# tritonmedia/downloader

Hardware: AMD Instinct MI355X
Metric: MB/s staged end-to-end (download->S3) + p50 job latency (higher is better)
Workload: dtype bytes

## Files before the change

downloader_amd/csrc/gpu_part_api.h:

```cpp
#pragma once

#include <stddef.h>
#include <stdint.h>

#define GPU_PART_API_ABI 2u
#define GPU_PART_COPIED 1
#define GPU_PART_DONE 2

typedef void (*gpu_part_notify_fn)(void* arg, uint64_t ticket, int phase);

struct GpuPartHashApi {
  uint32_t abi;
  void* ctx;
  int (*reg)(void* ctx, void* p, size_t n);
  void (*unreg)(void* ctx, void* p);
  uint64_t (*submit)(void* ctx, const uint8_t* data, int64_t len, int64_t piece_len);
  int (*wait)(void* ctx, uint64_t ticket, int phase, uint8_t* out, size_t out_len, char* err,
              size_t errlen);
  void (*set_notify)(void* ctx, gpu_part_notify_fn fn, void* arg);
};
```

downloader_amd/csrc/gpu_sha1.hip:

```cpp
#include <hip/hip_runtime.h>
#include <pybind11/pybind11.h>
#include <pybind11/stl.h>

#include <algorithm>
#include <atomic>
#include <chrono>
#include <cerrno>
#include <condition_variable>
#include <cstring>
#include <deque>
#include <fcntl.h>
#include <mutex>
#include <exception>
#include <stdexcept>
#include <string>
#include <pthread.h>
#include <thread>
#include <unistd.h>
#include <unordered_map>
#include <vector>

#include "gpu_part_api.h"
#include "part_dispatch.h"

// ... 959 lines not shown
      bool live = false;
    } pend[2];
    auto drain = [&](int s) {
      if (!pend[s].live) return;
      HIP_CHECK(hipStreamSynchronize(stream_[s]));
      uint8_t* hm = h_meta_ + (size_t)s * meta_stride_;
      if (out_digests) memcpy(out_digests + pend[s].first * 20, hm, (size_t)pend[s].cnt * 20);
      if (out_ok) memcpy(out_ok + pend[s].first, hm, (size_t)pend[s].cnt);
      pend[s].live = false;
    };
    int s = 0;
    for (int64_t first = 0; first < np; first += per, s ^= 1) {
      int64_t cnt = std::min(per, np - first);
      drain(s);
      fill(first, cnt, h_buf_[s]);
      int64_t off = first * piece_len;
      int64_t bytes = std::min(cnt * piece_len, total - off);
      int64_t last_len = bytes - (cnt - 1) * piece_len;
      uint8_t* dm = d_meta_ + (size_t)s * meta_stride_;
      uint8_t* hm = h_meta_ + (size_t)s * meta_stride_;
      HIP_CHECK(hipMemcpyAsync(d_buf_[s], h_buf_[s], (size_t)bytes, hipMemcpyHostToDevice, stream_[s]));
      const uint8_t* d_exp = nullptr;
      if (expected) {
        uint8_t* de = dm + per;
        HIP_CHECK(hipMemcpyAsync(de, expected + first * 20, (size_t)cnt * 20, hipMemcpyHostToDevice,
                                 stream_[s]));
        d_exp = de;
        launch(stream_[s], d_buf_[s], piece_len, last_len, (int)cnt, d_exp, dm, nullptr);
        HIP_CHECK(hipMemcpyAsync(hm, dm, (size_t)cnt, hipMemcpyDeviceToHost, stream_[s]));
      } else {
        launch(stream_[s], d_buf_[s], piece_len, last_len, (int)cnt, nullptr, nullptr, dm);
        HIP_CHECK(hipMemcpyAsync(hm, dm, (size_t)cnt * 20, hipMemcpyDeviceToHost, stream_[s]));
      }
      pend[s] = {first, cnt, true};
    }
    drain(0);
    drain(1);
  }

  void grow(int64_t bytes) {
    batch_bytes_ = 0;
    for (int s = 0; s < 2; ++s) {
      HIP_CHECK(hipStreamSynchronize(stream_[s]));
      HIP_CHECK(hipHostFree(h_buf_[s]));
      h_buf_[s] = nullptr;
      HIP_CHECK(hipFree(d_buf_[s]));
      d_buf_[s] = nullptr;
      HIP_CHECK(hipHostMalloc((void**)&h_buf_[s], (size_t)bytes, hipHostMallocDefault));
      HIP_CHECK(hipMalloc((void**)&d_buf_[s], (size_t)bytes));
    }
    batch_bytes_ = bytes;
  }

  void ensure_meta(int64_t per) {
    size_t need = (size_t)per * 21;
    if (need <= meta_stride_) return;
    if (d_meta_) HIP_CHECK(hipFree(d_meta_));
    d_meta_ = nullptr;
    if (h_meta_) HIP_CHECK(hipHostFree(h_meta_));
    h_meta_ = nullptr;
    meta_stride_ = 0;
    HIP_CHECK(hipMalloc((void**)&d_meta_, need * 2));
    HIP_CHECK(hipHostMalloc((void**)&h_meta_, need * 2, hipHostMallocDefault));
    meta_stride_ = need;
  }

  int device_;
  int64_t batch_bytes_;
  int readers_;
  hipStream_t stream_[2] = {nullptr, nullptr};
  hipEvent_t done_[2] = {nullptr, nullptr};
  uint8_t* h_buf_[2] = {nullptr, nullptr};
  uint8_t* d_buf_[2] = {nullptr, nullptr};
  uint8_t* d_meta_ = nullptr;
  uint8_t* h_meta_ = nullptr;
  size_t meta_stride_ = 0;
};

class HipPartDevice {
 public:
  using Event = hipEvent_t;

  HipPartDevice(int device, int64_t slot_bytes, int slots, int streams, int max_lanes,
                int copy_streams)
      : device_(device), slot_bytes_(slot_bytes), max_lanes_(max_lanes) {
    int n = 0;
    HIP_CHECK(hipGetDeviceCount(&n));
    if (device < 0 || device >= n) throw std::runtime_error("no such HIP device");
    if (slots < 2 || slot_bytes < (1 << 20) || max_lanes < 64 || copy_streams < 1 ||
        copy_streams > 4)
      throw std::invalid_argument("PartHasher: bad geometry");
    HIP_CHECK(hipSetDevice(device_));
    try {
      create(slots, streams, copy_streams);
    } catch (...) {
      release();
      throw;
    }
  }
  ~HipPartDevice() { release(); }
  HipPartDevice(const HipPartDevice&) = delete;
  HipPartDevice& operator=(const HipPartDevice&) = delete;

  static bool split_default() {
    const char* e = getenv("STAGER_SHA1_KERNEL");
    return !(e && std::string(e) == "lanes");
  }

  static int hw_queues() {
    const char* e = getenv("GPU_MAX_HW_QUEUES");
    const int n = e ? atoi(e) : 0;
    return n > 0 ? n : 4;
  }

  bool split() const { return split_; }
  int copy_streams() const { return (int)copies_.size(); }
  int compute_streams() const { return (int)streams_.size(); }
  int slots() const { return (int)slots_.size(); }
  void bind_thread() { HIP_CHECK(hipSetDevice(device_)); }
  int64_t* lane_table(int s) { return slots_[(size_t)s].h_lane; }

  Event copy(int s, int64_t off, const uint8_t* host, int64_t len, int cs) {
    hipStream_t st = copies_[(size_t)cs];
    HIP_CHECK(hipMemcpyAsync(slots_[(size_t)s].d_data + off, host, (size_t)len,
                             hipMemcpyHostToDevice, st));
    Event e = take_event();
    HIP_CHECK(hipEventRecord(e, st));
    return e;
  }
  bool copied(Event e) { return query(e); }
  void recycle(Event e) {
    if (e) free_events_.push_back(e);
  }
  void close_copies(int s) {
    Slot& sl = slots_[(size_t)s];
    for (size_t k = 0; k < copies_.size(); ++k) HIP_CHECK(hipEventRecord(sl.copied[k], copies_[k]));
  }
  int64_t launch_lanes() const { return launch_lanes_; }
  void launch(int stream, const int* slots, const int* lanes, int nslots, int total,
              bool align16) {
    if (total <= 0 || total > launch_lanes_) throw std::runtime_error("PartHasher: bad launch");
    Run& r = runs_[(size_t)stream];
    hipStream_t st = streams_[(size_t)stream];
    int64_t* ho = r.h_tab;
    int64_t* hl = r.h_tab + total;
    int i = 0;
    for (int k = 0; k < nslots; ++k) {
      Slot& sl = slots_[(size_t)slots[k]];
      for (size_t c = 0; c < copies_.size(); ++c) HIP_CHECK(hipStreamWaitEvent(st, sl.copied[c], 0));
      const int64_t base = (int64_t)(sl.d_data - arena_);
      for (int l = 0; l < lanes[k]; ++l, ++i) {
        ho[i] = base + sl.h_lane[l];
        hl[i] = sl.h_lane[max_lanes_ + l];
      }
    }
    if (i != total) throw std::runtime_error("PartHasher: lane count mismatch");
    HIP_CHECK(hipMemcpyAsync(r.d_tab, r.h_tab, (size_t)total * 2 * sizeof(int64_t),
                             hipMemcpyHostToDevice, st));
    const int64_t* dp = r.d_tab;
    const int64_t* dl = r.d_tab + total;
    const int block = 64, grid = (total + block - 1) / block;
    if (align16 && split_)
      hipLaunchKernelGGL(sha1_lanes_split, dim3(grid), dim3(kSplitThreads), 0, st, arena_, dp,
                         dl, total, r.d_dig);
    else if (align16)
      hipLaunchKernelGGL(sha1_lanes<16>, dim3(grid), dim3(block), 0, st, arena_, dp, dl, total,
                         r.d_dig);
    else
      hipLaunchKernelGGL(sha1_lanes<1>, dim3(grid), dim3(block), 0, st, arena_, dp, dl, total,
                         r.d_dig);
    HIP_CHECK(hipGetLastError());
    HIP_CHECK(hipMemcpyAsync(r.h_dig, r.d_dig, (size_t)total * 20, hipMemcpyDeviceToHost, st));
    HIP_CHECK(hipEventRecord(r.done, st));
  }
  bool finished(int stream) { return query(runs_[(size_t)stream].done); }
  const uint8_t* digests(int stream) { return runs_[(size_t)stream].h_dig; }
  void drain_copies() noexcept {
    for (auto c : copies_) hipStreamSynchronize(c);
  }
  int reg(void* p, size_t n) {
    if (hipSetDevice(device_) != hipSuccess) return -1;
    return hipHostRegister(p, n, hipHostRegisterDefault) == hipSuccess ? 0 : -1;
  }
  void unreg(void* p) {
    hipSetDevice(device_);
    hipHostUnregister(p);
  }

 private:
  struct Slot {
    uint8_t* d_data = nullptr;
    int64_t* h_lane = nullptr;
    hipEvent_t copied[4] = {nullptr, nullptr, nullptr, nullptr};
  };
  struct Run {
    int64_t* h_tab = nullptr;
    int64_t* d_tab = nullptr;
    uint8_t* d_dig = nullptr;
    uint8_t* h_dig = nullptr;
    hipEvent_t done = nullptr;
  };

  static bool query(hipEvent_t e) {
    hipError_t q = hipEventQuery(e);
    if (q == hipErrorNotReady) return false;
    HIP_CHECK(q);
    return true;
  }

  void create(int slots, int streams, int copy_streams) {
    copies_.resize((size_t)copy_streams);
    for (auto& c : copies_) HIP_CHECK(hipStreamCreateWithFlags(&c, hipStreamNonBlocking));
    const int hwq = hw_queues();
    const int compute = streams > 0 ? std::min(streams, 4) : std::max(1, hwq - copy_streams);
    streams_.resize((size_t)compute);
    for (auto& st : streams_) HIP_CHECK(hipStreamCreateWithFlags(&st, hipStreamNonBlocking));
    slots_.resize((size_t)slots);
    HIP_CHECK(hipMalloc((void**)&arena_, (size_t)slot_bytes_ * (size_t)slots + kArenaPad));
    for (size_t k = 0; k < slots_.size(); ++k) {
      Slot& sl = slots_[k];
      sl.d_data = arena_ + (size_t)slot_bytes_ * k;
      HIP_CHECK(hipHostMalloc((void**)&sl.h_lane, (size_t)max_lanes_ * 2 * sizeof(int64_t),
                              hipHostMallocDefault));
      for (auto& e : sl.copied) HIP_CHECK(hipEventCreateWithFlags(&e, hipEventDisableTiming));
    }
    launch_lanes_ = (int64_t)max_lanes_ * (int64_t)slots;
    runs_.resize((size_t)compute);
    for (auto& r : runs_) {
      HIP_CHECK(hipHostMalloc((void**)&r.h_tab, (size_t)launch_lanes_ * 2 * sizeof(int64_t),
                              hipHostMallocDefault));
      HIP_CHECK(hipMalloc((void**)&r.d_tab, (size_t)launch_lanes_ * 2 * sizeof(int64_t)));
      HIP_CHECK(hipMalloc((void**)&r.d_dig, (size_t)launch_lanes_ * 20));
      HIP_CHECK(hipHostMalloc((void**)&r.h_dig, (size_t)launch_lanes_ * 20, hipHostMallocDefault));
      HIP_CHECK(hipEventCreateWithFlags(&r.done, hipEventDisableTiming));
    }
  }

  void release() {
    hipSetDevice(device_);
    for (auto c : copies_)
      if (c) hipStreamSynchronize(c);
    for (auto st : streams_)
      if (st) {
        hipStreamSynchronize(st);
        hipStreamDestroy(st);
      }
    for (auto c : copies_)
      if (c) hipStreamDestroy(c);
    if (arena_) hipFree(arena_);
    arena_ = nullptr;
    for (auto& sl : slots_) {
      if (sl.h_lane) hipHostFree(sl.h_lane);
      for (auto e : sl.copied)
        if (e) hipEventDestroy(e);
    }
    for (auto& r : runs_) {
      if (r.h_tab) hipHostFree(r.h_tab);
      if (r.d_tab) hipFree(r.d_tab);
      if (r.d_dig) hipFree(r.d_dig);
      if (r.h_dig) hipHostFree(r.h_dig);
      if (r.done) hipEventDestroy(r.done);
    }
    for (hipEvent_t e : free_events_) hipEventDestroy(e);
    copies_.clear();
    streams_.clear();
    slots_.clear();
    runs_.clear();
    free_events_.clear();
  }

  hipEvent_t take_event() {
    if (!free_events_.empty()) {
      hipEvent_t e = free_events_.back();
      free_events_.pop_back();
      return e;
    }
    hipEvent_t e;
    HIP_CHECK(hipEventCreateWithFlags(&e, hipEventDisableTiming));
    return e;
  }

  int device_;
  int64_t slot_bytes_;
  int max_lanes_;
  bool split_ = split_default();
  int64_t launch_lanes_ = 0;
  uint8_t* arena_ = nullptr;
  std::vector<hipStream_t> copies_;
  std::vector<hipStream_t> streams_;
  std::vector<Slot> slots_;
  std::vector<Run> runs_;
  std::vector<hipEvent_t> free_events_;
};

using PartHasher = stager::PartDispatcher<HipPartDevice>;

py::dict part_stats(PartHasher& h) {
  const stager::PartDispatchStats s = h.stats();
  py::dict d;
  d["submitted"] = s.submitted;
  d["launches"] = s.launches;
  d["lanes"] = s.lanes;
  d["max_batch_lanes"] = s.max_batch_lanes;
  d["multi_slot_launches"] = s.multi_slot_launches;
  d["max_launch_slots"] = s.max_launch_slots;
  d["broken"] = s.broken;
  d["pending"] = s.pending;
  d["registered"] = s.registered;
  d["unregistered"] = s.unregistered;
  d["register_s"] = s.register_s;
  d["copy_streams"] = s.copy_streams;
  d["compute_streams"] = s.compute_streams;
  d["kernel"] = h.device().split() ? "sha1_lanes_split" : "sha1_lanes";
  return d;
}

int device_count() {
  int n = 0;
  if (hipGetDeviceCount(&n) != hipSuccess) return 0;
  return n;
}

}

PYBIND11_MODULE(_gpuhash, m) {
  m.doc() = "gfx950 batched SHA-1 piece verification (one lane per piece)";
  m.def("device_count", &device_count);
  m.def(
      "mem_info",
      [](int device) {
        size_t free_b = 0, total_b = 0;
        HIP_CHECK(hipSetDevice(device));
        HIP_CHECK(hipMemGetInfo(&free_b, &total_b));
        return py::make_tuple(free_b, total_b);
      },
      py::arg("device") = 0, "(free, total) bytes of device memory (hipMemGetInfo)");
  m.def("arch", [] {
    hipDeviceProp_t p;
    HIP_CHECK(hipGetDeviceProperties(&p, 0));
    return std::string(p.gcnArchName);
  });
  py::class_<GpuVerifier>(m, "GpuVerifier")
      .def(py::init([](int device, int64_t batch_bytes, int readers) {
             py::gil_scoped_release rel;
             return new GpuVerifier(device, batch_bytes, readers);
           }),
           py::arg("device") = 0, py::arg("batch_bytes") = (int64_t)256 << 20,
           py::arg("reader_threads") = 8)
      .def(
          "hash_buffer",
          [](GpuVerifier& g, const py::buffer& b, int64_t piece_len) {
            py::buffer_info info = b.request();
            int64_t n = (int64_t)info.size * (int64_t)info.itemsize;
            if (piece_len <= 0) throw std::invalid_argument("piece_len must be > 0");
            std::string out;
            {
              py::gil_scoped_release rel;
              out = g.hash_buffer((const uint8_t*)info.ptr, n, piece_len);
            }
            return py::bytes(out);
          },
          py::arg("data"), py::arg("piece_len"))
      .def(
          "verify_files",
          [](GpuVerifier& g, const std::vector<std::pair<std::string, int64_t>>& files,
             int64_t piece_len, const py::bytes& hashes) {
            std::string hs = hashes;
            if (piece_len <= 0) throw std::invalid_argument("piece_len must be > 0");
            std::vector<uint8_t> ok;
            {
              py::gil_scoped_release rel;
              ok = g.verify_files(files, piece_len, hs);
            }
            return py::bytes((const char*)ok.data(), ok.size());
          },
          py::arg("files"), py::arg("piece_len"), py::arg("hashes"))
      .def(
          "verify_files_streamed",
          [](GpuVerifier& g, const std::vector<std::pair<std::string, int64_t>>& files,
             int64_t piece_len, const py::bytes& hashes, int64_t chunk,
             const std::vector<int>& which) {
            std::string hs = hashes;
            if (piece_len <= 0) throw std::invalid_argument("piece_len must be > 0");
            std::vector<uint8_t> ok;
            std::vector<double> timing;
            {
              py::gil_scoped_release rel;
              ok = g.verify_files_streamed(files, piece_len, hs, chunk, &timing, which);
            }
            return py::make_tuple(py::bytes((const char*)ok.data(), ok.size()),
                                  py::make_tuple(timing[0], timing[1]));
          },
          py::arg("files"), py::arg("piece_len"), py::arg("hashes"), py::arg("chunk") = 65536,
          py::arg("which") = std::vector<int>{},
          "Chunk-streamed SHA-1 verification: returns (ok bytes, (host_fill_s, host_wait_s)); "
          "with `which`, one ok byte per listed piece in list order.")
      .def(
          "kernel_bench",
          [](GpuVerifier& g, int64_t piece_len, int n_pieces, int iters) {
            if (piece_len <= 0 || piece_len % 16 || n_pieces <= 0 || iters <= 0)
              throw std::invalid_argument("piece_len must be a positive multiple of 16");
            std::vector<double> r;
            {
              py::gil_scoped_release rel;
              r = g.kernel_bench(piece_len, n_pieces, iters);
            }
            return py::make_tuple(r[0], r[1]);
          },
          py::arg("piece_len"), py::arg("n_pieces"), py::arg("iters") = 5,
          "(ms_bitop3, ms_plain): kernel time per launch, device-resident data")
      .def(
          "kernel_bench_prefetch",
          [](GpuVerifier& g, int64_t piece_len, int n_pieces, int iters) {
            if (piece_len <= 0 || piece_len % 16 || n_pieces <= 0 || iters <= 0)
              throw std::invalid_argument("piece_len must be a positive multiple of 16");
            std::vector<double> r;
            {
              py::gil_scoped_release rel;
              r = g.kernel_bench_prefetch(piece_len, n_pieces, iters);
            }
            return py::make_tuple(r[0], r[1]);
          },
          py::arg("piece_len"), py::arg("n_pieces"), py::arg("iters") = 5,
          "(ms_prefetch, ms_no_prefetch): kernel time per launch, device-resident data")
      .def(
          "kernel_bench_concurrent",
          [](GpuVerifier& g, int64_t piece_len, int n0, int n1, int iters, int mode) {
            if (piece_len < 256 || piece_len % 16 || n0 <= 0 || n1 < 0 || iters <= 0 ||
                mode < 0 || mode > 2)
              throw std::invalid_argument("piece_len must be a multiple of 16, >= 256");
            std::vector<double> r;
            {
              py::gil_scoped_release rel;
              r = g.kernel_bench_concurrent(piece_len, n0, n1, iters, mode);
            }
            return py::make_tuple(r[0], r[1], r[2]);
          },
          py::arg("piece_len"), py::arg("n0"), py::arg("n1"), py::arg("iters") = 3,
          py::arg("mode") = 0,
          "(ms alone, ms on stream 0, ms on stream 1): sha1_lanes_split launches of n0 and n1 "
          "lanes side by side (mode 0), n0 beside 48 x 64 MiB H2D copies (1), after 40 ms idle "
          "(2)")
      .def(
          "kernel_bench_split",
          [](GpuVerifier& g, int64_t piece_len, int n_pieces, int iters, bool dup) {
            if (piece_len < 256 || piece_len % 16 || n_pieces <= 0 || iters <= 0)
              throw std::invalid_argument("piece_len must be a multiple of 16, >= 256");
            std::vector<double> r;
            {
              py::gil_scoped_release rel;
              r = g.kernel_bench_split(piece_len, n_pieces, iters, dup);
            }
            return py::make_tuple(r[0], r[1], r[2] != 0.0);
          },
          py::arg("piece_len"), py::arg("n_pieces"), py::arg("iters") = 3, py::arg("dup") = true,
          "(ms_split, ms_lanes, digests_equal): the PartHasher's two kernels on one lane table "
          "(dup=False: the split kernel with its idle lanes left idle)")
      .def_property_readonly("batch_bytes", &GpuVerifier::batch_bytes);
  py::class_<PartHasher>(m, "PartHasher")
      .def(py::init([](int device, int64_t slot_bytes, int slots, int streams, int max_lanes,
                       int copy_streams) {
             py::gil_scoped_release rel;
             return new PartHasher(slot_bytes, max_lanes, device, slot_bytes, slots, streams,
                                   max_lanes, copy_streams);
           }),
           py::arg("device") = 0, py::arg("slot_bytes") = (int64_t)1 << 30, py::arg("slots") = 8,
           py::arg("streams") = 0, py::arg("max_lanes") = 16384, py::arg("copy_streams") = 2)
      .def(
          "api",
          [](PartHasher& h) {
            return py::capsule((void*)h.api(), "downloader_amd.gpu_part_api");
          },
          "PyCapsule of the C ABI (gpu_part_api.h) for _native.set_gpu_part_hasher; the "
          "PartHasher must outlive every user of the capsule (ops.hashing keeps it for good)")
      .def(
          "hash",
          [](PartHasher& h, const py::buffer& b, int64_t piece_len) {
            py::buffer_info info = b.request();
            const int64_t n = (int64_t)info.size * (int64_t)info.itemsize;
            const int64_t np = piece_len > 0 ? (n + piece_len - 1) / piece_len : 0;
            std::string out((size_t)np * 20, '\0');
            char err[256] = {0};
            int rc;
            {
              py::gil_scoped_release rel;
              void* p = info.ptr;
              bool r = h.reg(p, (size_t)n) == 0;
              uint64_t t = h.submit((const uint8_t*)p, n, piece_len);
              rc = t ? h.wait(t, GPU_PART_DONE, (uint8_t*)out.data(), out.size(), err, sizeof err)
                     : -1;
              if (r) h.unreg(p);
            }
            if (rc != 0) throw std::runtime_error(err[0] ? err : "PartHasher refused the part");
            return py::bytes(out);
          },
          py::arg("data"), py::arg("piece_len"))
      .def("stats", &part_stats);
}
```

downloader_amd/csrc/module.cpp:

```cpp
#include <pybind11/pybind11.h>
#include <pybind11/stl.h>

#include <atomic>
#include <cstdlib>
#include <netinet/in.h>
#include <netinet/tcp.h>
#include <sys/socket.h>

#include "native.h"

namespace py = pybind11;
using namespace stager;

namespace {

struct BufView {
  const uint8_t* p;
  size_t n;
  py::buffer_info info;
};

BufView view(const py::buffer& b) {
  py::buffer_info info = b.request();
  if (info.ndim > 1 && info.strides.back() != info.itemsize)
    throw std::invalid_argument("buffer must be C-contiguous");
  size_t n = (size_t)info.size * (size_t)info.itemsize;
  return BufView{(const uint8_t*)info.ptr, n, std::move(info)};
}

py::dict head_to_dict(const ResponseHead& h) {
  py::dict d;
  d["status"] = h.status;
  d["reason"] = h.reason;
  py::list hs;
  for (auto& kv : h.headers) hs.append(py::make_tuple(kv.first, kv.second));
  d["headers"] = hs;
  d["content_length"] = h.content_length;
  d["chunked"] = h.chunked;
  d["keep_alive"] = h.keep_alive;
  return d;
}

}

void forget_ticket(uint64_t id) {
  if (id) gpu_part_forget(id);
}

static bool head_matches(const std::string& head, const std::string& pat) {
  size_t at = 0, i = 0;
  while (i <= pat.size()) {
    size_t star = pat.find('*', i);
    if (star == std::string::npos) star = pat.size();
    std::string piece = pat.substr(i, star - i);
    if (!piece.empty()) {
      size_t f = head.find(piece, at);
      if (f == std::string::npos) return false;
      at = f + piece.size();
    }
    i = star + 1;
  }
  return true;
}

static bool fault_bad_crc(const std::string& put_head) {
  static std::string pat;
  static std::atomic<int64_t> left{[] {
    const char* e = getenv("STAGER_FAULT_BAD_CRC");
    if (!e || !*e) return (int64_t)0;
    std::string v(e);
    size_t c = v.rfind(':');
    int64_t n = 1;
    if (c != std::string::npos && c + 1 < v.size() &&
        v.find_first_not_of("0123456789", c + 1) == std::string::npos) {
      n = atoll(v.c_str() + c + 1);
      v.resize(c);
    }
    pat = v;
    return n;
  }()};
  if (left.load(std::memory_order_relaxed) <= 0 || !head_matches(put_head, pat)) return false;
  return left.fetch_sub(1) > 0;
}

struct PieceSplit {
  int64_t skip, full_len, piece_len;
};

py::dict relay(HttpConn& src, const py::bytes& get_head, HttpConn& dst, const py::bytes& put_head,
               int64_t length, Progress* prog, int64_t max_body, const PieceSplit* split,
               bool crc, bool gpu = false) {
  std::string gh = get_head, ph = put_head;
  ResponseHead g, p;
  std::string gerr, pbody, digests, head, tail, crc_b64;
  int64_t moved = 0;
  uint64_t ticket = 0;
  {
    py::gil_scoped_release rel;
    try {
      src.send_request(gh, nullptr, 0);
      g = src.read_head();
      bool ok = (g.status == 200 || g.status == 206) && !g.chunked && g.content_length == length;
      if (!ok) {
        if (!g.chunked && g.content_length >= 0 && g.content_length <= (1 << 20))
          gerr = src.read_body(g, 1 << 20);
        else
          src.mark_unusable();
      } else {
        int cork = 1;
        setsockopt(dst.fd(), IPPROTO_TCP, TCP_CORK, &cork, sizeof(cork));
        dst.send_raw(ph);
        uint32_t c = 0;
        if (crc && length > 0) {
          char hx[32];
          snprintf(hx, sizeof hx, "%llx\r\n", (unsigned long long)length);
          dst.send_raw(hx);
        }
        moved = split ? src.relay_body_hashed(dst, length, split->skip, split->full_len,
                                              split->piece_len, prog, &digests, &head, &tail,
                                              crc ? &c : nullptr, gpu ? &ticket : nullptr)
                      : src.relay_body_to(dst, length, prog, crc ? &c : nullptr);
        if (crc) {
          if (fault_bad_crc(ph)) c ^= 1u;
          crc_b64 = crc32c_base64(c);
          dst.send_raw(std::string(length > 0 ? "\r\n" : "") + "0\r\nx-amz-checksum-crc32c:" +
                       crc_b64 + "\r\n\r\n");
        }
        cork = 0;
        setsockopt(dst.fd(), IPPROTO_TCP, TCP_CORK, &cork, sizeof(cork));
        p = dst.read_head();
        pbody = dst.read_body(p, max_body);
      }
    } catch (...) {
      forget_ticket(ticket);
      throw;
    }
    if (ticket && !(p.status >= 200 && p.status < 300)) {
      forget_ticket(ticket);
      ticket = 0;
    }
  }
  py::dict d;
  d["get"] = head_to_dict(g);
  d["get_body"] = py::bytes(gerr);
  d["put"] = p.status ? (py::object)head_to_dict(p) : py::none();
  d["put_body"] = py::bytes(pbody);
  d["moved"] = moved;
  d["crc32c"] = crc_b64;
  if (split) {
    d["gpu_ticket"] = ticket;
    d["digests"] = py::bytes(digests);
    d["head"] = py::bytes(head);
    d["tail"] = py::bytes(tail);
  }
  return d;
}

PYBIND11_MODULE(_native, m) {
  m.doc() = "stager host-native byte paths: hashing (OpenSSL EVP, threaded) and zero-copy HTTP";

  m.def("digest_size", &digest_size);
  m.def("crc32c_impl", []() { return std::string(crc32c_impl()); },
        "the CRC32C implementation this CPU runs (avx512-vpclmulqdq / sse4.2-3way)");
  m.def("sha1_mb_supported", &sha1_mb_supported,
        "True when the host runs the AVX-512 16-lane multi-buffer SHA-1 (csrc/sha1_mb.cpp)");
  m.def("effective_cpus", &effective_cpus,
        "CPUs usable by this process: affinity mask capped by the cgroup v2 cpu.max quota");
  m.def(
      "set_gpu_part_hasher",
      [](const py::object& capsule, int min_pieces) {
        if (capsule.is_none()) {
          set_gpu_part_hasher(nullptr, min_pieces);
          return;
        }
        void* p = PyCapsule_GetPointer(capsule.ptr(), "downloader_amd.gpu_part_api");
        if (!p) throw py::error_already_set();
        set_gpu_part_hasher(p, min_pieces);
      },
      py::arg("api"), py::arg("min_pieces") = 8,
      "Route the hashed relay's parts (>= min_pieces whole pieces) to the GPU hasher whose C "
      "ABI capsule is `api` (_gpuhash.PartHasher.api()); None: host multi-buffer SHA-1");
  m.def(
      "gpu_part_wait",
      [](uint64_t id) {
        std::string d;
        {
          py::gil_scoped_release rel;
          d = gpu_part_wait(id);
        }
        return py::bytes(d);
      },
      py::arg("id"), "Block until part `id` (the relay's gpu_ticket) is hashed: its digests");
  m.def(
      "gpu_part_forget",
      [](uint64_t id) {
        py::gil_scoped_release rel;
        gpu_part_forget(id);
      },
      py::arg("id"),
      "Nobody will ask for part `id`: returns once its buffer is back in the pool; the result "
      "is dropped when it arrives");
  m.def("gpu_part_eventfd", &gpu_part_eventfd,
        "eventfd that turns readable when gpu_part_poll has news");
  m.def(
      "gpu_part_poll",
      []() {
        std::vector<GpuPartEvent> ev;
        {
          py::gil_scoped_release rel;
          ev = gpu_part_poll();
        }
        py::list out;
        for (auto& e : ev)
          out.append(py::make_tuple(e.id, e.kind, py::bytes(e.data)));
        return out;
      },
      "Drain completions: [(id, kind, data)] with kind 1 = copied (the part's buffer is back in "
      "the pool), 2 = done (data = 20 B digests per piece), 3 = failed (data = error message)");
  py::class_<CpuPartHasher>(m, "CpuPartHasher")
      .def(py::init<double, int, int>(), py::arg("delay_s") = 0.005,
           py::arg("fail_copy_every") = 0, py::arg("fail_done_every") = 0,
           "gpu_part_api.h on a host thread (tests of the asynchronous relay-hashing path); "
           "fail_*_every: every Nth job's copy / hash fails")
      .def("api", [](CpuPartHasher& h) {
        return py::capsule((void*)h.api(), "downloader_amd.gpu_part_api");
      })
      .def_property_readonly("registered", &CpuPartHasher::registered);
  m.def("gpu_part_stats", []() {
    GpuPartStats s = gpu_part_stats();
    py::dict d;
    d["submitted"] = s.submitted;
    d["host_fallbacks"] = s.host_fallbacks;
    d["refused"] = s.refused;
    d["pending"] = s.pending;
    return d;
  });
  m.def("relay_pool_trim", &relay_pool_trim, py::arg("keep_bytes") = 0,
        "Unmap idle hashed-relay part buffers beyond keep_bytes; returns the bytes freed");
  m.def("relay_pool_set_budget", &relay_pool_set_budget, py::arg("bytes"),
        "Bound leased + idle part buffers (0 = no bound): idle ones are unmapped to make room");
  m.def("relay_pool_reset_peak", &relay_pool_reset_peak,
        "Restart the pool's high-water mark (peak_bytes) and its over_budget count");
  m.def("relay_pool_set_max_idle", &relay_pool_set_max_idle, py::arg("n"),
        "Keep at most n idle part buffers (the rest are unmapped on release)");
  py::class_<SwarmWire>(m, "SwarmWire",
                        "Native peer-wire receive path of one torrent session (peerwire.cpp)")
      .def(py::init<int, int>(), py::arg("verify_threads") = 2, py::arg("io_threads") = 4)
      .def("set_storage",
           [](SwarmWire& w, int64_t piece_length, int64_t total, const py::bytes& hashes,
              const std::vector<std::pair<int, int64_t>>& files) {
             w.set_storage(piece_length, total, std::string(hashes), files);
           },
           py::arg("piece_length"), py::arg("total"), py::arg("hashes"), py::arg("files"))
      .def("begin_piece", &SwarmWire::begin_piece, py::arg("idx"))
      .def("drop_piece", &SwarmWire::drop_piece, py::arg("idx"))
      .def("set_pipeline", &SwarmWire::set_pipeline, py::arg("depth"))
      .def("set_conn_pipeline", &SwarmWire::set_conn_pipeline, py::arg("conn_id"),
           py::arg("depth"), "requests in flight on one connection (its bandwidth-delay product)")
      .def("assign", &SwarmWire::assign, py::arg("conn_id"), py::arg("idx"),
           "Own piece idx on the connection: the wire requests its blocks (returns the "
           "connection's blocks still to request)")
      .def("todo", &SwarmWire::todo, py::arg("conn_id"))
      .def("release",
           [](SwarmWire& w, uint64_t id) {
             py::list out;
             for (auto& r : w.release(id)) out.append(py::make_tuple(r.first, py::bytes(r.second)));
             return out;
           },
           py::arg("conn_id"),
           "[(idx, states)] of the pieces the connection owned, now ordinary (2 received, "
           "1 requested and unanswered, 0 neither)")
      .def("release_piece",
           [](SwarmWire& w, uint32_t idx) -> py::object {
             uint64_t owner = 0;
             std::string st;
             if (!w.release_piece(idx, &owner, &st)) return py::none();
             return py::make_tuple(owner, py::bytes(st));
           },
           py::arg("idx"), "(owner, states) of an owned piece made ordinary, or None")
      .def("rx_idle", &SwarmWire::rx_idle, py::arg("conn_id"))
      .def("take_block",
           [](SwarmWire& w, uint32_t idx, uint32_t begin, const py::buffer& b) {
             py::buffer_info i = b.request();
             return w.take_block(idx, begin, (const uint8_t*)i.ptr,
                                 (uint32_t)(i.size * i.itemsize));
           },
           py::arg("idx"), py::arg("begin"), py::arg("data"),
           "A block received on a Python-framed connection: 0 not taken, 1 taken, 2 taken "
           "and the piece complete")
      .def("set_have",
           [](SwarmWire& w, const py::bytes& bits) { w.set_have(std::string(bits)); },
           py::arg("bits"))
      .def("set_have_piece", &SwarmWire::set_have_piece, py::arg("idx"))
      .def("set_serving", &SwarmWire::set_serving, py::arg("conn_id"), py::arg("on"))
      .def("set_backlog_cap", &SwarmWire::set_backlog_cap, py::arg("bytes"))
      .def("backlogged", &SwarmWire::backlogged,
           "True while complete, unreported pieces hold the cap or more (start no new piece)")
      .def("set_host_tail", &SwarmWire::set_host_tail, py::arg("on"),
           "GPU mode: hash the pieces completing from now on on the host (the download's end)")
      .def("rx_total", &SwarmWire::rx_total, "bytes received on every connection so far")
      .def("gpu_latency", &SwarmWire::gpu_latency,
           "GPU mode: submission -> digest time of the device's pieces (EWMA, s; 0 = none yet)")
      .def("set_gpu", &SwarmWire::set_gpu, py::arg("on"), py::arg("max_inflight") = 64,
           "Verify complete pieces on the installed GPU part hasher (set_gpu_part_hasher), at "
           "most max_inflight at once (the rest on the host)")
      .def("attach",
           [](SwarmWire& w, int fd, uint64_t id, const py::bytes& prefix) {
             w.attach(fd, id, std::string(prefix));
           },
           py::arg("fd"), py::arg("conn_id"), py::arg("prefix") = py::bytes(),
           "Hand a connected socket over (the fd is owned from here on, closed by detach)")
      .def("send",
           [](SwarmWire& w, uint64_t id, const py::bytes& data) {
             std::string s(data);
             return w.send(id, std::move(s));
           },
           py::arg("conn_id"), py::arg("data"))
      .def("sendv",
           [](SwarmWire& w, uint64_t id, const py::list& parts) {
// ... 388 lines not shown
```

downloader_amd/csrc/native.h:

```cpp
#pragma once

#include <atomic>
#include <condition_variable>
#include <cstdint>
#include <deque>
#include <memory>
#include <mutex>
#include <string>
#include <thread>
#include <unordered_map>
#include <utility>
#include <vector>

typedef struct evp_md_ctx_st EVP_MD_CTX;
typedef struct evp_md_st EVP_MD;
typedef struct ssl_st SSL;
typedef struct ssl_ctx_st SSL_CTX;

namespace stager {

const EVP_MD* md_for(const std::string& algo);
size_t digest_size(const std::string& algo);
int effective_cpus();
int resolve_threads(int threads, size_t work_items);
// ... 26 lines not shown

bool sha1_mb_supported();
void sha1_mb(const uint8_t* const* msgs, const size_t* lens, size_t n, uint8_t* out);
void sha1x16_init(uint32_t st[5][16]);
void sha1_mb16_blocks(uint32_t state[5][16], const uint8_t* const ptr[16], size_t nblocks,
                      uint16_t active);
void sha1x16_finish(uint32_t st[5][16], const uint8_t* const tails[16], size_t tail_len,
                    uint64_t total_len, uint16_t active, uint8_t* out);

struct Storage {
  struct Entry {
    std::string path;
    int64_t length;
    int64_t offset;
    int fd;
  };
  explicit Storage(const std::vector<std::pair<std::string, int64_t>>& files);
  ~Storage();
  void open_all(bool missing_ok);
  void close_all();
  bool read(int64_t off, int64_t len, uint8_t* buf) const;
  std::vector<Entry> entries;
  int64_t total = 0;
};

std::vector<uint8_t> verify_pieces(const std::vector<std::pair<std::string, int64_t>>& files,
                                   int64_t piece_len, const std::string& hashes,
                                   const std::vector<int64_t>& which, int threads);
std::string hash_storage_pieces(const std::vector<std::pair<std::string, int64_t>>& files,
                                int64_t piece_len, const std::string& algo, int threads);
std::vector<std::string> hash_file_ranges(const std::string& path,
                                          const std::vector<std::pair<int64_t, int64_t>>& ranges,
                                          const std::string& algo, int threads);

class TlsContext {
 public:
  TlsContext(bool verify, const std::string& ca_file);
  ~TlsContext();
  TlsContext(const TlsContext&) = delete;
  TlsContext& operator=(const TlsContext&) = delete;
  SSL_CTX* ctx() const { return ctx_; }
  bool verify() const { return verify_; }

 private:
  SSL_CTX* ctx_ = nullptr;
  bool verify_;
};
SSL* tls_handshake(TlsContext& ctx, int fd, const std::string& name);
std::string tls_error(SSL* s, int r, const std::string& what);

constexpr int64_t kMaxBufferedPart = (int64_t)64 << 20;

struct PipeStats {
  uint64_t created, short_pipes;
  size_t in_use, in_use_bytes, idle, idle_bytes;
};
PipeStats pipe_stats();
struct RelayCounters {
  uint64_t relays[4], bytes[4], cpu_ns[4];
  uint64_t splice_in_calls, splice_out_calls;
  uint64_t dup_calls, dup_bytes;
  uint64_t crc_ns, crc_bytes;
  uint64_t sha1_ns;
  uint64_t nt_bytes;
};
RelayCounters relay_counters();
void set_pipe_sizes(size_t main, size_t tee);
void set_pipes_refused(bool on);
void set_relay_dup(const std::string& mode);
std::string relay_dup_mode();

struct RelayPoolStats {
  size_t idle_buffers, idle_bytes, in_use, max_idle;
  uint64_t created;
  size_t in_use_bytes, budget, peak_bytes;
  uint64_t evicted, over_budget;
};
void set_gpu_part_hasher(const void* api, int min_pieces);
const void* gpu_part_hasher_current();
void swarm_piece_pool_forget(const void* api);
void swarm_piece_pool_limit(size_t bytes);
struct GpuPartStats {
  uint64_t submitted, host_fallbacks, refused, pending;
};
GpuPartStats gpu_part_stats();
std::string gpu_part_wait(uint64_t id);
void gpu_part_forget(uint64_t id);
int gpu_part_eventfd();
struct GpuPartEvent {
  uint64_t id;
  int kind;
  std::string data;
};
std::vector<GpuPartEvent> gpu_part_poll();
class CpuPartHasher {
 public:
  explicit CpuPartHasher(double delay_s, int fail_copy_every = 0, int fail_done_every = 0);
  ~CpuPartHasher();
  const void* api() const;
  uint64_t registered() const;

 private:
  struct Impl;
  std::unique_ptr<Impl> impl_;
};
struct WireEvent {
  uint64_t conn;
  int kind;
  std::string data;
};
struct SwarmWireStats {
  uint64_t begun = 0, blocks = 0, block_bytes = 0, blocks_ignored = 0, verified = 0,
           hash_fails = 0, rx_bytes = 0, recvs = 0;
  uint64_t verify_batches = 0, sha_ns = 0, write_ns = 0;
  uint64_t served_bytes = 0;
  uint64_t assigned = 0, requests = 0;
  uint64_t gpu_pieces = 0, gpu_refused = 0, gpu_errors = 0;
  uint64_t gpu_overflow = 0;
  int64_t gpu_latency_ns_sum = 0, gpu_latency_ns_max = 0;
  int64_t backlog_bytes = 0;
  size_t pool_in_use = 0, pool_idle = 0, pool_idle_bytes = 0;
  uint64_t pool_allocs = 0, pool_frees = 0, pool_locks = 0;
  size_t active_pieces = 0;
  size_t io_threads = 0;
  uint64_t serve_floods = 0;
  uint64_t serve_cancels = 0;
};
class SwarmWire {
 public:
  static constexpr int kEvMsg = 1, kEvBlocks = 2, kEvClosed = 3, kEvPiece = 4, kEvNeed = 5;
  explicit SwarmWire(int verify_threads = 2, int io_threads = 4);
  ~SwarmWire();
  void set_storage(int64_t piece_length, int64_t total, const std::string& hashes,
                   const std::vector<std::pair<int, int64_t>>& files);
  void begin_piece(uint32_t idx);
  void drop_piece(uint32_t idx);
  void set_pipeline(uint32_t depth);
  void set_conn_pipeline(uint64_t conn, uint32_t depth);
  size_t assign(uint64_t conn, uint32_t idx);
  size_t todo(uint64_t conn);
  std::vector<std::pair<uint32_t, std::string>> release(uint64_t conn);
  bool release_piece(uint32_t idx, uint64_t* owner, std::string* states);
  double rx_idle(uint64_t conn);
  void set_have(const std::string& bits);
  void set_have_piece(uint32_t idx);
  void set_serving(uint64_t id, bool on);
  void set_gpu(bool on, int max_inflight = 64);
  void set_host_tail(bool on);
  double gpu_latency() const { return gpu_lat_ewma_ns_.load() / 1e9; }
  uint64_t rx_total() const { return rx_bytes_.load(std::memory_order_relaxed); }
  void set_backlog_cap(int64_t bytes);
  bool backlogged();
  void attach(int fd, uint64_t id, const std::string& prefix);
  size_t send(uint64_t id, std::string data);
  size_t pending_out(uint64_t id);
  uint64_t conn_rx(uint64_t id);
  void detach(uint64_t id);
  int eventfd() const { return efd_; }
  std::vector<WireEvent> poll();
  SwarmWireStats stats();
  void close();
  int take_block(uint32_t idx, uint32_t begin, const uint8_t* p, uint32_t len);

 private:
  struct Piece;
  struct Conn;
  struct OutItem;
  struct IoLoop;
// ... 162 lines not shown
```

downloader_amd/csrc/part_dispatch.h:

```cpp
#pragma once

#include <algorithm>
#include <chrono>
#include <condition_variable>
#include <cstring>
#include <deque>
#include <exception>
#include <mutex>
#include <pthread.h>
#include <stdexcept>
#include <string>
#include <thread>
#include <unordered_map>
#include <utility>
#include <vector>

#include "gpu_part_api.h"

namespace stager {

struct PartDispatchStats {
  uint64_t submitted = 0, launches = 0, lanes = 0, max_batch_lanes = 0;
  uint64_t multi_slot_launches = 0, max_launch_slots = 0;
  uint64_t registered = 0, unregistered = 0;
  double register_s = 0;
  bool broken = false;
  size_t pending = 0;
  int copy_streams = 0, compute_streams = 0;
};

template <class Dev>
class PartDispatcher {
 public:
  template <class... A>
  PartDispatcher(int64_t slot_bytes, int max_lanes, A&&... dev_args)
      : dev_(std::forward<A>(dev_args)...), slot_bytes_(slot_bytes), max_lanes_(max_lanes) {
    slots_.resize((size_t)dev_.slots());
    running_.resize((size_t)dev_.compute_streams());
    api_.abi = GPU_PART_API_ABI;
    api_.ctx = this;
    api_.reg = [](void* c, void* p, size_t n) { return ((PartDispatcher*)c)->reg(p, n); };
    api_.unreg = [](void* c, void* p) { ((PartDispatcher*)c)->unreg(p); };
    api_.submit = [](void* c, const uint8_t* d, int64_t len, int64_t pl) {
      return ((PartDispatcher*)c)->submit(d, len, pl);
    };
    api_.wait = [](void* c, uint64_t t, int ph, uint8_t* out, size_t ol, char* err, size_t el) {
      return ((PartDispatcher*)c)->wait(t, ph, out, ol, err, el);
    };
    api_.set_notify = [](void* c, gpu_part_notify_fn fn, void* arg) {
      PartDispatcher* h = (PartDispatcher*)c;
      std::lock_guard<std::mutex> g(h->mu_);
      h->notify_ = fn;
      h->notify_arg_ = arg;
    };
    thread_ = std::thread([this] { run(); });
    pthread_setname_np(thread_.native_handle(), "gpu-part-disp");
  }

  ~PartDispatcher() {
    {
      std::lock_guard<std::mutex> g(mu_);
      stop_ = true;
    }
    cv_.notify_all();
    if (thread_.joinable()) thread_.join();
  }

  PartDispatcher(const PartDispatcher&) = delete;
  PartDispatcher& operator=(const PartDispatcher&) = delete;

  const GpuPartHashApi* api() const { return &api_; }
  Dev& device() { return dev_; }

  int reg(void* p, size_t n) {
    const auto t0 = std::chrono::steady_clock::now();
    const bool ok = dev_.reg(p, n) == 0;
    const double dt = std::chrono::duration<double>(std::chrono::steady_clock::now() - t0).count();
    std::lock_guard<std::mutex> g(mu_);
    stats_.registered++;
    stats_.register_s += dt;
    return ok ? 0 : -1;
  }
  void unreg(void* p) {
    dev_.unreg(p);
    std::lock_guard<std::mutex> g(mu_);
    stats_.unregistered++;
  }

  uint64_t submit(const uint8_t* data, int64_t len, int64_t piece_len) {
    if (len <= 0 || piece_len <= 0) return 0;
    const int64_t np = (len + piece_len - 1) / piece_len;
    if (np > max_lanes_ || len > slot_bytes_) return 0;
    std::lock_guard<std::mutex> g(mu_);
    if (broken_ || stop_) return 0;
    uint64_t t = ++seq_;
    Job& j = jobs_[t];
    j.host = data;
    j.len = len;
    j.piece_len = piece_len;
    j.np = (int)np;
    queue_.push_back(t);
    stats_.submitted++;
    cv_.notify_all();
    return t;
  }

  int wait(uint64_t t, int phase, uint8_t* out, size_t out_len, char* err, size_t errlen) {
    std::unique_lock<std::mutex> lk(mu_);
    auto it = jobs_.find(t);
    if (it == jobs_.end()) return fail(err, errlen, "unknown ticket");
    Job* j = &it->second;
    wcv_.wait(lk, [&] {
      return !j->err.empty() || j->done || (phase == GPU_PART_COPIED && j->copied);
    });
    if (!j->err.empty()) {
      std::string e = j->err;
      if (phase == GPU_PART_DONE || j->done || broken_) jobs_.erase(t);
      return fail(err, errlen, e.c_str());
    }
    if (phase == GPU_PART_DONE) {
      if (out_len < j->digests.size()) return fail(err, errlen, "digest buffer too small");
      memcpy(out, j->digests.data(), j->digests.size());
      jobs_.erase(t);
    }
    return 0;
  }

  PartDispatchStats stats() {
    std::lock_guard<std::mutex> g(mu_);
    PartDispatchStats s = stats_;
    s.broken = broken_;
    s.pending = jobs_.size();
    s.copy_streams = dev_.copy_streams();
    s.compute_streams = dev_.compute_streams();
    return s;
  }

 private:
  using Event = typename Dev::Event;
  struct Job {
    const uint8_t* host = nullptr;
    int64_t len = 0, piece_len = 0;
    int np = 0;
    int slot = -1, lane0 = 0;
    Event copy_ev{};
    bool copied = false, done = false;
    std::string err, digests;
  };
  struct Slot {
    int64_t used = 0;
    int lanes = 0;
    bool align16 = true;
    std::vector<uint64_t> jobs;
    int state = 0;
    std::chrono::steady_clock::time_point opened;
  };

  static int fail(char* err, size_t errlen, const char* msg) {
    if (err && errlen) {
      strncpy(err, msg, errlen - 1);
      err[errlen - 1] = 0;
    }
    return -1;
  }

  void tell(std::vector<uint64_t>& owed, int phase) {
    if (owed.empty()) return;
    std::vector<uint64_t> tickets;
    tickets.swap(owed);
    gpu_part_notify_fn fn;
    void* arg;
    {
      std::lock_guard<std::mutex> g(mu_);
      fn = notify_;
      arg = notify_arg_;
    }
    if (fn)
      for (uint64_t t : tickets) fn(arg, t, phase);
  }

  Job& job(uint64_t t) {
    std::lock_guard<std::mutex> g(mu_);
    return jobs_.at(t);
  }

  void run() {
    std::vector<uint64_t> owed_copied, owed_done;
    std::deque<uint64_t> copying;
    try {
      dev_.bind_thread();
      int filling = -1;
      for (;;) {
        std::deque<uint64_t> fresh;
        {
          std::unique_lock<std::mutex> lk(mu_);
          const bool idle = queue_.empty() && copying.empty() && !any_running() &&
                            !any_closed() && !(filling >= 0 && slots_[(size_t)filling].lanes > 0);
          if (idle) cv_.wait(lk, [&] { return stop_ || !queue_.empty(); });
          if (stop_ && idle && queue_.empty()) return;
          fresh.swap(queue_);
        }
        bool progressed = false;
        while (!fresh.empty()) {
          const uint64_t t = fresh.front();
          Job* j = &job(t);
          if (filling >= 0) {
            Slot& f = slots_[(size_t)filling];
            const int64_t off = (f.used + 255) & ~(int64_t)255;
            if (off + j->len > slot_bytes_ || f.lanes + j->np > max_lanes_) {
              f.state = 2;
              dev_.close_copies(filling);
              filling = -1;
            }
          }
          if (filling < 0) {
            filling = free_slot();
            if (filling < 0) break;
            Slot& f = slots_[(size_t)filling];
            f.state = 1;
            f.used = 0;
            f.lanes = 0;
            f.align16 = true;
            f.jobs.clear();
            f.opened = std::chrono::steady_clock::now();
          }
          Slot& f = slots_[(size_t)filling];
          const int64_t off = (f.used + 255) & ~(int64_t)255;
          const int cs = (int)(next_copy_++ % (size_t)dev_.copy_streams());
          Event ev = dev_.copy(filling, off, j->host, j->len, cs);
          int64_t* lt = dev_.lane_table(filling);
          for (int k = 0; k < j->np; ++k) {
            const int64_t po = (int64_t)k * j->piece_len;
            lt[f.lanes + k] = off + po;
            lt[max_lanes_ + f.lanes + k] = std::min(j->piece_len, j->len - po);
          }
          {
            std::lock_guard<std::mutex> g(mu_);
            j->copy_ev = ev;
            j->slot = filling;
            j->lane0 = f.lanes;
          }
          if (j->piece_len % 16) f.align16 = false;
          f.lanes += j->np;
          f.used = off + j->len;
          f.jobs.push_back(t);
          copying.push_back(t);
          fresh.pop_front();
          progressed = true;
        }
        const bool slot_bound = !fresh.empty();
        if (slot_bound) {
          std::lock_guard<std::mutex> g(mu_);
          for (auto it = fresh.rbegin(); it != fresh.rend(); ++it) queue_.push_front(*it);
        }
        for (auto it = copying.begin(); it != copying.end();) {
          Job* j = &job(*it);
          if (!dev_.copied(j->copy_ev)) {
            ++it;
            continue;
          }
          Event ev;
          {
            std::lock_guard<std::mutex> g(mu_);
            j->copied = true;
            ev = j->copy_ev;
            j->copy_ev = Event{};
            owed_copied.push_back(*it);
          }
          dev_.recycle(ev);
          wcv_.notify_all();
          it = copying.erase(it);
          progressed = true;
        }
        tell(owed_copied, GPU_PART_COPIED);
        for (size_t s = 0; s < running_.size(); ++s) {
          std::vector<int>& group = running_[s];
          if (group.empty()) continue;
          if (!dev_.finished((int)s)) continue;
          const uint8_t* dig = dev_.digests((int)s);
          std::vector<Event> late;
          {
            std::lock_guard<std::mutex> g(mu_);
            size_t base = 0;
            for (int si : group) {
              Slot& sl = slots_[(size_t)si];
              for (uint64_t t : sl.jobs) {
                Job& j = jobs_.at(t);
                j.digests.assign((const char*)dig + (base + (size_t)j.lane0) * 20, (size_t)j.np * 20);
                j.done = true;
                if (!j.copied) {
                  j.copied = true;
                  late.push_back(j.copy_ev);
                  j.copy_ev = Event{};
                  auto c = std::find(copying.begin(), copying.end(), t);
                  if (c != copying.end()) copying.erase(c);
                  owed_copied.push_back(t);
                }
                owed_done.push_back(t);
              }
              base += (size_t)sl.lanes;
            }
          }
          for (Event e : late) dev_.recycle(e);
          wcv_.notify_all();
          for (int si : group) {
            slots_[(size_t)si].state = 0;
            slots_[(size_t)si].jobs.clear();
          }
          group.clear();
          progressed = true;
        }
        tell(owed_copied, GPU_PART_COPIED);
        for (size_t s = 0; s < running_.size(); ++s) {
          if (!running_[s].empty()) continue;
          std::vector<int> group, lanes;
          int total = 0;
          bool a16 = true;
          for (int pick : closed_by_age()) {
            const Slot& sl = slots_[(size_t)pick];
            if (total + sl.lanes > dev_.launch_lanes()) break;
            group.push_back(pick);
            lanes.push_back(sl.lanes);
            total += sl.lanes;
            a16 = a16 && sl.align16;
          }
          if (filling >= 0 && slots_[(size_t)filling].lanes > 0 &&
              total + slots_[(size_t)filling].lanes <= dev_.launch_lanes()) {
            Slot& f = slots_[(size_t)filling];
            dev_.close_copies(filling);
            group.push_back(filling);
            lanes.push_back(f.lanes);
            total += f.lanes;
            a16 = a16 && f.align16;
            filling = -1;
          }
          if (group.empty()) break;
          dev_.launch((int)s, group.data(), lanes.data(), (int)group.size(), total, a16);
          for (int si : group) slots_[(size_t)si].state = 3;
          running_[s] = group;
          std::lock_guard<std::mutex> g(mu_);
          stats_.launches++;
          stats_.lanes += (uint64_t)total;
          stats_.max_batch_lanes = std::max<uint64_t>(stats_.max_batch_lanes, (uint64_t)total);
          stats_.max_launch_slots = std::max<uint64_t>(stats_.max_launch_slots, group.size());
          if (group.size() > 1) stats_.multi_slot_launches++;
          progressed = true;
        }
        tell(owed_done, GPU_PART_DONE);
        if (!progressed) {
          std::unique_lock<std::mutex> lk(mu_);
          cv_.wait_until(lk, std::chrono::system_clock::now() + std::chrono::microseconds(200),
                         [&] { return stop_ || (!slot_bound && !queue_.empty()); });
        }
      }
    } catch (const std::exception& e) {
      dev_.drain_copies();
      tell(owed_copied, GPU_PART_COPIED);
      tell(owed_done, GPU_PART_DONE);
      std::vector<uint64_t> failed_copy, failed_hash;
      {
        std::lock_guard<std::mutex> g(mu_);
        broken_ = true;
        for (auto& kv : jobs_)
          if (!kv.second.done) {
            kv.second.err = std::string("GPU part hasher: ") + e.what();
            (kv.second.copied ? failed_hash : failed_copy).push_back(kv.first);
          }
        queue_.clear();
        wcv_.notify_all();
      }
      tell(failed_copy, GPU_PART_COPIED);
      tell(failed_hash, GPU_PART_DONE);
    }
  }

  bool any_running() const {
    for (auto& g : running_)
      if (!g.empty()) return true;
    return false;
  }
  bool any_closed() const {
    for (auto& sl : slots_)
      if (sl.state == 2) return true;
    return false;
  }
  int free_slot() const {
    for (size_t i = 0; i < slots_.size(); ++i)
      if (slots_[i].state == 0) return (int)i;
    return -1;
  }
  std::vector<int> closed_by_age() const {
    std::vector<int> out;
    for (size_t i = 0; i < slots_.size(); ++i)
      if (slots_[i].state == 2) out.push_back((int)i);
    std::sort(out.begin(), out.end(),
              [&](int a, int b) { return slots_[(size_t)a].opened < slots_[(size_t)b].opened; });
    return out;
  }

  Dev dev_;
  int64_t slot_bytes_;
  int max_lanes_;
  size_t next_copy_ = 0;
  std::vector<std::vector<int>> running_;
  std::vector<Slot> slots_;
  std::mutex mu_;
  std::condition_variable cv_, wcv_;
  std::deque<uint64_t> queue_;
  std::unordered_map<uint64_t, Job> jobs_;
  uint64_t seq_ = 0;
  bool stop_ = false, broken_ = false;
  PartDispatchStats stats_;
  GpuPartHashApi api_{};
  gpu_part_notify_fn notify_ = nullptr;
  void* notify_arg_ = nullptr;
  std::thread thread_;
};

}
```

downloader_amd/csrc/part_fake_device.h:

```cpp
#pragma once

#include <atomic>
#include <chrono>
#include <condition_variable>
#include <cstring>
#include <deque>
#include <functional>
#include <memory>
#include <mutex>
#include <random>
#include <stdexcept>
#include <string>
#include <thread>
#include <vector>

#include "native.h"

namespace stager {

struct FakeDeviceKnobs {
  int copy_us_max = 200;
  int kernel_us_max = 1500;
  double lag = 0.3;
  int fail_launch_at = 0;
  int fail_query_at = 0;
  uint32_t seed = 1;
};

class FakePartDevice {
 public:
  using Event = std::shared_ptr<std::atomic<int>>;

  FakePartDevice(int64_t slot_bytes, int slots, int compute_streams, int copy_streams,
                 int max_lanes, FakeDeviceKnobs k)
      : max_lanes_(max_lanes), k_(k), rng_(k.seed) {
    slots_.resize((size_t)slots);
    for (auto& s : slots_) {
      s.mem.assign((size_t)slot_bytes, 0);
      s.lanes.assign((size_t)max_lanes * 2, 0);
      s.markers.resize((size_t)copy_streams);
    }
    runs_.resize((size_t)compute_streams);
    for (auto& r : runs_) r.done = std::make_shared<std::atomic<int>>(0);
    for (int i = 0; i < copy_streams; ++i) copies_.emplace_back(new Queue(k.seed * 7 + i));
    for (int i = 0; i < compute_streams; ++i) computes_.emplace_back(new Queue(k.seed * 13 + i));
  }
  ~FakePartDevice() {
    for (auto& q : copies_) q->stop();
    for (auto& q : computes_) q->stop();
  }
  FakePartDevice(const FakePartDevice&) = delete;
  FakePartDevice& operator=(const FakePartDevice&) = delete;

  int copy_streams() const { return (int)copies_.size(); }
  int compute_streams() const { return (int)computes_.size(); }
  int slots() const { return (int)slots_.size(); }
  void bind_thread() {}
  int64_t* lane_table(int s) { return slots_[(size_t)s].lanes.data(); }

  Event copy(int s, int64_t off, const uint8_t* host, int64_t len, int cs) {
    Event e = std::make_shared<std::atomic<int>>(0);
    uint8_t* dst = slots_[(size_t)s].mem.data() + off;
    const int us = k_.copy_us_max;
    Queue* q = copies_[(size_t)cs].get();
    q->push([dst, host, len, e, us, q] {
      q->nap(us);
      memcpy(dst, host, (size_t)len);
      e->store(1, std::memory_order_release);
    });
    return e;
  }
  bool copied(const Event& e) {
    tick();
    if (!e->load(std::memory_order_acquire)) return false;
    return !chance(k_.lag);
  }
  void recycle(const Event&) {}
  void close_copies(int s) {
    Slot& sl = slots_[(size_t)s];
    for (size_t k = 0; k < copies_.size(); ++k) {
      Event m = std::make_shared<std::atomic<int>>(0);
      sl.markers[k] = m;
      copies_[k]->push([m] { m->store(1, std::memory_order_release); });
    }
  }
  int64_t launch_lanes() const { return (int64_t)max_lanes_ * (int64_t)slots_.size(); }
  void launch(int stream, const int* slots, const int* lanes, int nslots, int total,
              bool ) {
    if (k_.fail_launch_at && ++launches_ == k_.fail_launch_at)
      throw std::runtime_error("injected device fault (launch)");
    Run* run = &runs_[(size_t)stream];
    run->done->store(0, std::memory_order_relaxed);
    std::vector<std::pair<Slot*, int>> group;
    std::vector<Event> markers;
    for (int k = 0; k < nslots; ++k) {
      Slot* sl = &slots_[(size_t)slots[k]];
      group.push_back({sl, lanes[k]});
      markers.insert(markers.end(), sl->markers.begin(), sl->markers.end());
    }
    const int us = k_.kernel_us_max, ml = max_lanes_;
    Queue* q = computes_[(size_t)stream].get();
    run->dig.assign((size_t)total * 20, 0);
    q->push([run, group, markers, us, ml, q] {
      for (auto& m : markers)
        while (m && !m->load(std::memory_order_acquire)) std::this_thread::yield();
      q->nap(us);
      size_t i = 0;
      for (auto& g : group) {
        Slot* sl = g.first;
        for (int k = 0; k < g.second; ++k, ++i) {
          const int64_t off = sl->lanes[(size_t)k], len = sl->lanes[(size_t)(ml + k)];
          const std::string d = digest("sha1", sl->mem.data() + off, (size_t)len);
          memcpy(run->dig.data() + i * 20, d.data(), 20);
        }
      }
      run->done->store(1, std::memory_order_release);
    });
  }
  bool finished(int stream) {
    tick();
    return runs_[(size_t)stream].done->load(std::memory_order_acquire) != 0;
  }
  const uint8_t* digests(int stream) { return runs_[(size_t)stream].dig.data(); }
  void drain_copies() noexcept {
    for (auto& q : copies_) q->drain();
  }
  int reg(void*, size_t) { return 0; }
  void unreg(void*) {}

 private:
  struct Queue {
    std::mutex mu;
    std::condition_variable cv;
    std::deque<std::function<void()>> tasks;
    bool stopping = false, busy = false;
    std::mt19937 rng;
    std::thread th;
    explicit Queue(uint32_t seed) : rng(seed) {
      th = std::thread([this] {
        std::unique_lock<std::mutex> lk(mu);
        for (;;) {
          cv.wait(lk, [&] { return stopping || !tasks.empty(); });
          if (tasks.empty()) return;
          auto f = std::move(tasks.front());
          tasks.pop_front();
          busy = true;
          lk.unlock();
          f();
          lk.lock();
          busy = false;
          cv.notify_all();
        }
      });
    }
    void push(std::function<void()> f) {
      std::lock_guard<std::mutex> g(mu);
      tasks.push_back(std::move(f));
      cv.notify_all();
    }
    void nap(int us_max) {
      const int us = us_max > 0 ? (int)(rng() % (uint32_t)us_max) : 0;
      if (us) std::this_thread::sleep_for(std::chrono::microseconds(us));
    }
    void drain() {
      std::unique_lock<std::mutex> lk(mu);
      cv.wait(lk, [&] { return tasks.empty() && !busy; });
    }
    void stop() {
      {
        std::lock_guard<std::mutex> g(mu);
        stopping = true;
      }
      cv.notify_all();
      if (th.joinable()) th.join();
    }
  };
  struct Slot {
    std::vector<uint8_t> mem;
    std::vector<int64_t> lanes;
    std::vector<Event> markers;
  };
  struct Run {
    std::vector<uint8_t> dig;
    Event done;
  };

  void tick() {
    if (k_.fail_query_at && ++queries_ == k_.fail_query_at)
      throw std::runtime_error("injected device fault (query)");
  }
  bool chance(double p) {
    return p > 0 && std::uniform_real_distribution<double>(0, 1)(rng_) < p;
  }

  int max_lanes_;
  FakeDeviceKnobs k_;
  std::mt19937 rng_;
  int launches_ = 0, queries_ = 0;
  std::vector<Slot> slots_;
  std::vector<Run> runs_;
  std::vector<std::unique_ptr<Queue>> copies_, computes_;
};

}
```

downloader_amd/csrc/selftest.cpp:

```cpp
#include <arpa/inet.h>
#include <fcntl.h>
#include <netinet/in.h>
#include <signal.h>
#include <sys/socket.h>
#include <unistd.h>

#include <openssl/err.h>
#include <openssl/evp.h>
#include <openssl/pem.h>
#include <openssl/ssl.h>
#include <openssl/x509v3.h>

#include <poll.h>

#include <algorithm>
#include <chrono>
#include <condition_variable>
#include <cstdio>
#include <cstdlib>
#include <cstring>
#include <functional>
#include <map>
#include <memory>
#include <mutex>
// ... 660 lines not shown
        const uint32_t idx = rd32(e.data.data());
        if (e.data[4] == 1) {
          verified[idx]++;
          done++;
        } else {
          bad++;
          w.begin_piece(idx);
          w.assign(1, idx);
        }
        if (!released && done >= npieces / 2) {
          released = true;
          records_before = block_records;
          for (auto& r : w.release(2)) {
            CHECK(r.second.size() == (size_t)((std::min<int64_t>(plen, total - (int64_t)r.first * plen) + 16383) / 16384));
            w.assign(1, r.first);
          }
        }
      }
    }
  }
  CHECK(done == npieces);
  for (int i = 0; i < npieces; ++i) CHECK(verified[i] == 1);
  SwarmWireStats st = w.stats();
  CHECK(bad == 1 && st.hash_fails == 1 && st.verified == (uint64_t)npieces);
  CHECK(released && records_before == 0);
  CHECK(needs > 0);
  CHECK(st.blocks_ignored >= 1);
  w.close();
  for (auto& t : seeders) t.join();
  std::vector<uint8_t> back((size_t)total);
  CHECK(pread(f1, back.data(), (size_t)total, 0) == total);
  CHECK(back == data);
  for (int fd : theirs) close(fd);
  close(f1);
  unlink(p1);
  fprintf(stderr, "wire (owned): %d pieces, %d requests, %d NEED events, %llu blocks refused\n",
          done, requests.load(), needs, (unsigned long long)st.blocks_ignored);
}

static void multislot_section() {
  Watchdog wd("multi-slot launches", 60);
  FakeDeviceKnobs k;
  k.kernel_us_max = 30000;
  k.copy_us_max = 100;
  k.lag = 0.3;
  k.seed = 7;
  auto h = fake_hasher(k);
  const GpuPartHashApi* api = h->api();
  const int64_t piece = 16 << 10;
  const int parts = 160, pieces = 8;
  auto data = rnd((size_t)parts * pieces * piece, 91);
  std::vector<uint64_t> tickets;
  for (int i = 0; i < parts; ++i) {
    const uint8_t* p = data.data() + (size_t)i * pieces * piece;
    uint64_t t = 0;
    while (!(t = api->submit(api->ctx, p, pieces * piece, piece)))
      std::this_thread::sleep_for(std::chrono::microseconds(50));
    tickets.push_back(t);
  }
  bool ok = true;
  for (int i = 0; i < parts; ++i) {
    uint8_t dig[pieces * 20];
    char err[256] = {0};
    if (api->wait(api->ctx, tickets[(size_t)i], GPU_PART_DONE, dig, sizeof dig, err, sizeof err) != 0) {
      fprintf(stderr, "multi-slot: part %d failed: %s\n", i, err);
      ok = false;
      continue;
    }
    for (int q = 0; q < pieces; ++q) {
      const uint8_t* pc = data.data() + ((size_t)i * pieces + q) * piece;
      if (digest("sha1", pc, (size_t)piece) != std::string((const char*)dig + q * 20, 20)) ok = false;
    }
  }
  const PartDispatchStats st = h->stats();
  fprintf(stderr, "multi-slot: %llu launches, %llu spanning >= 2 slots, up to %llu slots / %llu lanes\n",
          (unsigned long long)st.launches, (unsigned long long)st.multi_slot_launches,
          (unsigned long long)st.max_launch_slots, (unsigned long long)st.max_batch_lanes);
  CHECK(ok);
  CHECK(st.multi_slot_launches > 0 && st.max_launch_slots >= 2);
  CHECK(st.max_batch_lanes > 256);
  CHECK(st.lanes == (uint64_t)parts * pieces && st.pending == 0);
}

static void stress_sections() {
  multislot_section();
  {
    Watchdog wd("part stress", 90);
    PartStress cfg;
    GpuPartStats before = gpu_part_stats();
    PartStressResult r = part_stress(cfg);
    GpuPartStats after = gpu_part_stats();
    fprintf(stderr, "part stress: %d good, %d forgotten, %d via poll, %d failed, %d hashers\n",
            r.good, r.forgotten, r.polled, r.failed, r.hashers);
    CHECK(r.digests_ok && r.failed == 0);
    CHECK(r.good + r.forgotten == cfg.threads * cfg.parts);
    CHECK(r.forgotten > 0 && r.hashers > 2);
    CHECK(after.submitted - before.submitted + after.refused - before.refused ==
          (uint64_t)(cfg.threads * cfg.parts));
    CHECK(after.submitted - before.submitted > (uint64_t)(cfg.threads * cfg.parts) / 2);
    CHECK(after.pending == 0);
  }
  {
    Watchdog wd("part stress with device faults", 90);
    PartStress cfg;
    cfg.threads = 16;
    cfg.parts = 24;
    cfg.replace_every_ms = 20;
    cfg.first.fail_launch_at = 3;
    cfg.knobs.fail_launch_at = 4;
    cfg.knobs.fail_query_at = 400;
    GpuPartStats before = gpu_part_stats();
    PartStressResult r = part_stress(cfg);
    GpuPartStats after = gpu_part_stats();
    fprintf(stderr, "part stress (faults): %d good, %d forgotten, %d failed, %d host fallbacks\n",
            r.good, r.forgotten, r.failed, (int)(after.host_fallbacks - before.host_fallbacks));
    CHECK(r.digests_ok);
    CHECK(r.good + r.forgotten + r.failed == cfg.threads * cfg.parts);
    CHECK(r.failed + (int)(after.host_fallbacks - before.host_fallbacks) > 0);
    CHECK(after.pending == 0);
  }
}

int main() {
  signal(SIGPIPE, SIG_IGN);
  if (getenv("SELFTEST_ONLY") && strcmp(getenv("SELFTEST_ONLY"), "wire") == 0) {
    wire_section(false);
    wire_section(true);
    wire_owned_section();
    printf(g_fail ? "selftest: failures\n" : "selftest ok\n");
    return g_fail ? 1 : 0;
  }
  if (getenv("SELFTEST_ONLY") && strcmp(getenv("SELFTEST_ONLY"), "stress") == 0) {
    stress_sections();
    printf(g_fail ? "selftest: failures\n" : "selftest ok\n");
    return g_fail ? 1 : 0;
  }
  const uint8_t* abc = (const uint8_t*)"abc";
  CHECK(hex(digest("sha1", abc, 3)) == "a9993e364706816aba3e25717850c26c9cd0d89d");
  CHECK(hex(digest("md5", abc, 3)) == "900150983cd24fb0d6963f7d28e17f72");
  CHECK(hex(digest("sha256", abc, 3)) ==
        "ba7816bf8f01cfea414140de5dae2223b00361a396177a9cb410ff61f20015ad");

  auto data = rnd(8 << 20, 1);
  std::string p1 = hash_pieces("sha1", data.data(), data.size(), 65536, 1);
  std::string p8 = hash_pieces("sha1", data.data(), data.size(), 65536, 8);
  CHECK(p1 == p8);

  auto a = rnd(3000001, 2), b = rnd(777777, 3);
  std::string fa = tmpfile_with(a, "a"), fb = tmpfile_with(b, "b");
  std::vector<std::pair<std::string, int64_t>> files = {{fa, (int64_t)a.size()}, {fb, (int64_t)b.size()}};
  std::string hashes = hash_storage_pieces(files, 262144, "sha1", 8);
  auto ok = verify_pieces(files, 262144, hashes, {}, 8);
  bool all = true;
  for (auto v : ok) all = all && v;
  CHECK(all);
  {
    int fd = open(fb.c_str(), O_WRONLY);
    uint8_t x = b[5] ^ 0xFF;
    pwrite(fd, &x, 1, 5);
    close(fd);
  }
  ok = verify_pieces(files, 262144, hashes, {}, 8);
  int bad = 0;
  for (auto v : ok) bad += !v;
  CHECK(bad == 1);

  auto body = rnd(1 << 20, 4);
// ... 318 lines not shown
```

downloader_amd/csrc/transfer.cpp:

```cpp
#include "native.h"
#include "gpu_part_api.h"

#include <algorithm>
#include <atomic>
#include <chrono>
#include <condition_variable>
#include <deque>
#include <thread>
#include <arpa/inet.h>
#include <cerrno>
#include <cstdlib>
#include <cstring>
#include <fcntl.h>
#include <netdb.h>
#include <netinet/in.h>
#include <netinet/tcp.h>
#include <poll.h>
#include <mutex>
#include <new>
#include <stdexcept>
#include <sys/mman.h>
#include <sys/sendfile.h>
#include <sys/socket.h>
#include <sys/types.h>
// ... 1292 lines not shown
    {
      std::lock_guard<std::mutex> g(mu_);
      for (size_t i = 0; i < idle_.size();) {
        if (idle_[i]->reg_api && idle_[i]->reg_api != keep) {
          idle_bytes_ -= idle_[i]->cap;
          drop.push_back(std::move(idle_[i]));
          idle_.erase(idle_.begin() + (ptrdiff_t)i);
        } else {
          ++i;
        }
      }
    }
  }
  size_t trim(size_t keep_bytes) {
    std::vector<std::unique_ptr<PartBuffer>> drop;
    size_t freed = 0;
    {
      std::lock_guard<std::mutex> g(mu_);
      while (!idle_.empty() && idle_bytes_ > keep_bytes) {
        idle_bytes_ -= idle_.back()->cap;
        freed += idle_.back()->cap;
        drop.push_back(std::move(idle_.back()));
        idle_.pop_back();
      }
    }
    return freed;
  }
  void set_max_idle(size_t n) {
    std::lock_guard<std::mutex> g(mu_);
    max_idle_ = n;
  }
  void set_budget(size_t bytes) {
    std::vector<std::unique_ptr<PartBuffer>> drop;
    std::lock_guard<std::mutex> g(mu_);
    budget_ = bytes;
    while (bytes && !idle_.empty() && in_use_bytes_ + idle_bytes_ > budget_) {
      idle_bytes_ -= idle_.back()->cap;
      drop.push_back(std::move(idle_.back()));
      idle_.pop_back();
      evicted_++;
    }
  }
  void reset_peak() {
    std::lock_guard<std::mutex> g(mu_);
    peak_ = in_use_bytes_ + idle_bytes_;
    over_budget_ = 0;
  }
  RelayPoolStats stats() {
    std::lock_guard<std::mutex> g(mu_);
    return RelayPoolStats{idle_.size(), idle_bytes_, in_use_, max_idle_, created_.load(),
                          in_use_bytes_, budget_, peak_, evicted_, over_budget_};
  }

 private:
  void lease(size_t bytes) {
    in_use_ += 1;
    in_use_bytes_ += bytes;
    if (budget_ && in_use_bytes_ > budget_) over_budget_++;
    peak_ = std::max(peak_, in_use_bytes_ + idle_bytes_);
  }
  std::mutex mu_;
  std::vector<std::unique_ptr<PartBuffer>> idle_;
  size_t idle_bytes_ = 0, in_use_ = 0, max_idle_ = 16;
  size_t in_use_bytes_ = 0, budget_ = 0, peak_ = 0;
  uint64_t evicted_ = 0, over_budget_ = 0;
  std::atomic<uint64_t> created_{0};
};

PartPool& part_pool() {
  static PartPool* p = new PartPool();
  return *p;
}

struct PartLease {
  std::unique_ptr<PartBuffer> b;
  explicit PartLease(size_t n) : b(part_pool().acquire(n)) {}
  ~PartLease() {
    if (b) part_pool().release(std::move(b));
  }
};

std::atomic<int> g_gpu_min_pieces{8};
std::atomic<uint64_t> g_gpu_submitted{0}, g_gpu_fallbacks{0}, g_gpu_refused{0};

struct GpuPending {
  std::unique_ptr<PartBuffer> buf;
  const GpuPartHashApi* api = nullptr;
  uint64_t ticket = 0;
  int64_t skip = 0, full_len = 0, piece_len = 0;
  bool copied = false, finished = false, failed = false;
  bool forgotten = false, copied_reported = false;
  bool waited = false;
  std::string result;
};
std::mutex g_gpu_mu;
std::condition_variable g_gpu_cv;
std::unordered_map<uint64_t, GpuPending> g_gpu_parts;
std::map<std::pair<const GpuPartHashApi*, uint64_t>, uint64_t> g_gpu_ids;
std::deque<uint64_t> g_gpu_news;
uint64_t g_gpu_next_id = 0;

int gpu_efd() {
  static int fd = eventfd(0, EFD_NONBLOCK | EFD_CLOEXEC);
  return fd;
}

void gpu_signal(uint64_t id) {
  g_gpu_news.push_back(id);
  g_gpu_cv.notify_all();
  const uint64_t one = 1;
  if (gpu_efd() >= 0) {
    ssize_t w = write(gpu_efd(), &one, sizeof one);
    (void)w;
  }
}

void host_digests_impl(const uint8_t* p, int64_t full_len, int64_t piece_len, std::string* out);
void host_digests(const uint8_t* p, int64_t full_len, int64_t piece_len, std::string* out) {
  const uint64_t t0 = mono_ns();
  host_digests_impl(p, full_len, piece_len, out);
  t_tally.sha1_ns += mono_ns() - t0;
}
void host_digests_impl(const uint8_t* p, int64_t full_len, int64_t piece_len, std::string* out) {
  const int64_t np = (full_len + piece_len - 1) / piece_len;
  std::vector<const uint8_t*> ptrs((size_t)np);
  std::vector<size_t> lens((size_t)np);
  for (int64_t i = 0; i < np; ++i) {
    ptrs[(size_t)i] = p + i * piece_len;
    lens[(size_t)i] = (size_t)std::min<int64_t>(piece_len, full_len - i * piece_len);
  }
  out->resize((size_t)np * 20);
  sha1_mb(ptrs.data(), lens.data(), (size_t)np, (uint8_t*)&(*out)[0]);
}

void gpu_copied(const GpuPartHashApi* a, uint64_t ticket, uint64_t id) {
  char err[256] = {0};
  const int rc = a->wait(a->ctx, ticket, GPU_PART_COPIED, nullptr, 0, err, sizeof err);
  std::unique_ptr<PartBuffer> buf;
  int64_t skip = 0, full = 0, plen = 0;
  {
    std::lock_guard<std::mutex> g(g_gpu_mu);
    auto it = g_gpu_parts.find(id);
    if (it == g_gpu_parts.end() || it->second.copied || !it->second.buf) return;
    buf = std::move(it->second.buf);
    skip = it->second.skip;
    full = it->second.full_len;
    plen = it->second.piece_len;
  }
  std::string digests;
  if (rc != 0) {
    host_digests(buf->data + skip, full, plen, &digests);
    g_gpu_fallbacks++;
  }
  part_pool().release(std::move(buf));
  std::lock_guard<std::mutex> g(g_gpu_mu);
  auto it = g_gpu_parts.find(id);
  if (it == g_gpu_parts.end()) return;
  GpuPending& p = it->second;
  p.copied = true;
  if (rc != 0) {
    p.finished = true;
    p.result.swap(digests);
    g_gpu_ids.erase({a, ticket});
  }
  if (p.forgotten && p.finished)
    g_gpu_parts.erase(it);
  else if (!p.forgotten)
    gpu_signal(id);
  g_gpu_cv.notify_all();
}

void gpu_done(const GpuPartHashApi* a, uint64_t ticket, uint64_t id) {
  int64_t np = 0;
  {
    std::lock_guard<std::mutex> g(g_gpu_mu);
    auto it = g_gpu_parts.find(id);
    if (it == g_gpu_parts.end() || it->second.finished) return;
    np = (it->second.full_len + it->second.piece_len - 1) / it->second.piece_len;
  }
  std::string out((size_t)np * 20, '\0');
  char err[256] = {0};
  const int rc = a->wait(a->ctx, ticket, GPU_PART_DONE, (uint8_t*)&out[0], out.size(), err,
                         sizeof err);
  std::lock_guard<std::mutex> g(g_gpu_mu);
  g_gpu_ids.erase({a, ticket});
  auto it = g_gpu_parts.find(id);
  if (it == g_gpu_parts.end()) return;
  GpuPending& p = it->second;
  p.finished = true;
  p.failed = rc != 0;
  p.result = rc ? std::string("GPU piece hashing failed: ") + err : out;
  if (p.forgotten) {
    g_gpu_parts.erase(it);
    g_gpu_cv.notify_all();
  } else {
    gpu_signal(id);
  }
}

void gpu_notify(void* arg, uint64_t ticket, int phase) {
  const GpuPartHashApi* a = (const GpuPartHashApi*)arg;
  uint64_t id;
  bool copied;
  {
    std::lock_guard<std::mutex> g(g_gpu_mu);
    auto it = g_gpu_ids.find({a, ticket});
    if (it == g_gpu_ids.end()) return;
    id = it->second;
    auto p = g_gpu_parts.find(id);
    if (p == g_gpu_parts.end()) return;
    copied = p->second.copied;
  }
  if (!copied) gpu_copied(a, ticket, id);
  if (phase == GPU_PART_DONE) gpu_done(a, ticket, id);
}
}

const void* gpu_part_hasher_current() { return g_gpu_api.load(); }

void set_gpu_part_hasher(const void* api, int min_pieces) {
  const GpuPartHashApi* a = (const GpuPartHashApi*)api;
  if (a && a->abi != GPU_PART_API_ABI) throw std::invalid_argument("gpu_part_api ABI mismatch");
  if (a) a->set_notify(a->ctx, &gpu_notify, (void*)a);
  g_gpu_min_pieces.store(std::max(1, min_pieces));
  const GpuPartHashApi* old = g_gpu_api.exchange(a);
  part_pool().drop_foreign(a);
  if (old && old != a) swarm_piece_pool_forget(old);
}

namespace {
struct CpuJob {
  const uint8_t* host;
  int64_t len, piece_len;
  std::string copy, digests;
  bool copied = false, done = false;
  bool fail_copy = false, fail_done = false;
  bool abandoned = false;
};
}

struct CpuPartHasher::Impl {
  std::mutex mu;
  std::condition_variable cv, wcv;
  std::unordered_map<uint64_t, CpuJob> jobs;
  std::deque<uint64_t> queue;
// ... 59 lines not shown
  m->api.reg = [](void* c, void*, size_t) {
    Impl* i = (Impl*)c;
    std::lock_guard<std::mutex> g(i->mu);
    i->registered++;
    return 0;
  };
  m->api.unreg = [](void*, void*) {};
  m->api.submit = [](void* c, const uint8_t* d, int64_t len, int64_t pl) -> uint64_t {
    Impl* i = (Impl*)c;
    std::lock_guard<std::mutex> g(i->mu);
    if (i->stop || len <= 0 || pl <= 0) return 0;
    uint64_t t = ++i->seq;
    CpuJob& j = i->jobs[t];
    j.host = d;
    j.len = len;
    j.piece_len = pl;
    j.fail_copy = i->fail_copy_every > 0 && t % (uint64_t)i->fail_copy_every == 0;
    j.fail_done = i->fail_done_every > 0 && t % (uint64_t)i->fail_done_every == 0;
    i->queue.push_back(t);
    i->cv.notify_all();
    return t;
  };
  m->api.wait = [](void* c, uint64_t t, int phase, uint8_t* out, size_t ol, char* err,
                   size_t el) -> int {
    Impl* i = (Impl*)c;
    std::unique_lock<std::mutex> lk(i->mu);
    auto it = i->jobs.find(t);
    if (it == i->jobs.end()) {
      snprintf(err, el, "unknown ticket");
      return -1;
    }
    CpuJob* j = &it->second;
    i->wcv.wait(lk, [&] { return phase == GPU_PART_COPIED ? j->copied : j->done; });
    if ((phase == GPU_PART_COPIED && j->fail_copy) || (phase == GPU_PART_DONE && j->fail_done)) {
      snprintf(err, el, "injected device failure (%s)", phase == GPU_PART_COPIED ? "copy" : "hash");
      if (phase == GPU_PART_DONE)
        i->jobs.erase(t);
      else
        j->abandoned = true;
      return -1;
    }
    if (phase == GPU_PART_DONE) {
      if (ol < j->digests.size()) {
        snprintf(err, el, "digest buffer too small");
        return -1;
      }
      memcpy(out, j->digests.data(), j->digests.size());
      i->jobs.erase(t);
    }
    return 0;
  };
  m->api.set_notify = [](void* c, gpu_part_notify_fn fn, void* arg) {
    Impl* i = (Impl*)c;
    std::lock_guard<std::mutex> g(i->mu);
    i->notify = fn;
    i->notify_arg = arg;
  };
  m->th = std::thread([m] { m->run(); });
}

CpuPartHasher::~CpuPartHasher() {
  {
    std::lock_guard<std::mutex> g(impl_->mu);
    impl_->stop = true;
  }
  impl_->cv.notify_all();
  impl_->th.join();
}

const void* CpuPartHasher::api() const { return &impl_->api; }

uint64_t CpuPartHasher::registered() const {
  std::lock_guard<std::mutex> g(impl_->mu);
  return impl_->registered;
}

GpuPartStats gpu_part_stats() {
  size_t pending;
  {
    std::lock_guard<std::mutex> g(g_gpu_mu);
    pending = g_gpu_parts.size();
  }
  return GpuPartStats{g_gpu_submitted.load(), g_gpu_fallbacks.load(), g_gpu_refused.load(),
                      pending};
}

std::string gpu_part_wait(uint64_t id) {
  std::unique_lock<std::mutex> lk(g_gpu_mu);
  auto w = g_gpu_parts.find(id);
  if (w == g_gpu_parts.end()) throw IoError("gpu_part_wait: unknown part");
  w->second.waited = true;
  g_gpu_cv.wait(lk, [&] {
    auto f = g_gpu_parts.find(id);
    return f == g_gpu_parts.end() || f->second.finished;
  });
  auto it = g_gpu_parts.find(id);
  if (it == g_gpu_parts.end()) throw IoError("gpu_part_wait: part already collected");
  GpuPending p = std::move(it->second);
  g_gpu_parts.erase(it);
  if (p.failed) throw IoError(p.result);
  return p.result;
}

void gpu_part_forget(uint64_t id) {
  std::unique_lock<std::mutex> lk(g_gpu_mu);
  auto it = g_gpu_parts.find(id);
  if (it == g_gpu_parts.end()) return;
  it->second.forgotten = true;
  g_gpu_cv.wait(lk, [&] {
    auto f = g_gpu_parts.find(id);
    return f == g_gpu_parts.end() || f->second.copied;
  });
  it = g_gpu_parts.find(id);
  if (it != g_gpu_parts.end() && it->second.finished) g_gpu_parts.erase(it);
}

int gpu_part_eventfd() { return gpu_efd(); }

std::vector<GpuPartEvent> gpu_part_poll() {
  uint64_t cnt;
  ssize_t r = read(gpu_efd(), &cnt, sizeof cnt);
  (void)r;
  std::vector<GpuPartEvent> out;
  std::lock_guard<std::mutex> g(g_gpu_mu);
  while (!g_gpu_news.empty()) {
    const uint64_t id = g_gpu_news.front();
    g_gpu_news.pop_front();
    auto it = g_gpu_parts.find(id);
    if (it == g_gpu_parts.end() || it->second.forgotten || it->second.waited) continue;
    GpuPending& p = it->second;
    if (p.copied && !p.copied_reported) {
      p.copied_reported = true;
      out.push_back(GpuPartEvent{id, 1, std::string()});
    }
    if (p.finished) {
      out.push_back(GpuPartEvent{id, p.failed ? 3 : 2, std::move(p.result)});
      g_gpu_parts.erase(it);
    }
  }
  return out;
}

void set_relay_dup(const std::string& mode) {
  if (mode != "peek" && mode != "tee") throw std::invalid_argument("relay dup mode: peek or tee");
  g_relay_peek.store(mode == "peek" ? 1 : 0);
}
std::string relay_dup_mode() { return relay_peek_on() ? "peek" : "tee"; }

size_t relay_pool_trim(size_t keep_bytes) { return part_pool().trim(keep_bytes); }
PipeStats pipe_stats() { return pipe_pool().stats(); }

RelayCounters relay_counters() {
  RelayCounters c{};
  for (int i = 0; i < 4; ++i) {
    c.relays[i] = g_rc.relays[i].load();
    c.bytes[i] = g_rc.bytes[i].load();
    c.cpu_ns[i] = g_rc.cpu_ns[i].load();
  }
  c.splice_in_calls = g_rc.splice_in.load();
  c.splice_out_calls = g_rc.splice_out.load();
  c.dup_calls = g_rc.dup_calls.load();
  c.dup_bytes = g_rc.dup_bytes.load();
  c.crc_ns = g_rc.crc_ns.load();
  c.crc_bytes = g_rc.crc_bytes.load();
  c.sha1_ns = g_rc.sha1_ns.load();
  c.nt_bytes = g_rc.nt_bytes.load();
  return c;
}
void set_pipes_refused(bool on) { g_pipes_refused.store(on); }
void set_pipe_sizes(size_t main, size_t tee) {
  if (main) g_pipe_main.store(main);
  if (tee) g_pipe_tee.store(tee);
  pipe_pool().drop_idle();
}
void relay_pool_set_max_idle(size_t n) { part_pool().set_max_idle(n); }
void relay_pool_set_budget(size_t bytes) { part_pool().set_budget(bytes); }
void relay_pool_reset_peak() { part_pool().reset_peak(); }
RelayPoolStats relay_pool_stats() { return part_pool().stats(); }

static int part_nt_mode() {
  static const int m = [] {
    const char* e = getenv("STAGER_PART_NT");
    return e ? std::max(0, std::min(2, atoi(e))) : 1;
  }();
  return m;
}

__attribute__((target("avx2"))) static void stream_copy_avx2(uint8_t* d, const uint8_t* s,
                                                              size_t n) {
  size_t head = std::min(n, (size_t)(-(uintptr_t)d & 31));
  memcpy(d, s, head);
  d += head, s += head, n -= head;
  for (; n >= 128; n -= 128, d += 128, s += 128) {
    const __m256i a = _mm256_loadu_si256((const __m256i*)s);
    const __m256i b = _mm256_loadu_si256((const __m256i*)(s + 32));
    const __m256i c = _mm256_loadu_si256((const __m256i*)(s + 64));
    const __m256i e = _mm256_loadu_si256((const __m256i*)(s + 96));
    _mm256_stream_si256((__m256i*)d, a);
    _mm256_stream_si256((__m256i*)(d + 32), b);
    _mm256_stream_si256((__m256i*)(d + 64), c);
    _mm256_stream_si256((__m256i*)(d + 96), e);
  }
  for (; n >= 32; n -= 32, d += 32, s += 32)
    _mm256_stream_si256((__m256i*)d, _mm256_loadu_si256((const __m256i*)s));
  memcpy(d, s, n);
  _mm_sfence();
}

static void stream_copy(uint8_t* d, const uint8_t* s, size_t n) {
  static const bool avx2 = __builtin_cpu_supports("avx2");
  if (avx2)
    stream_copy_avx2(d, s, n);
  else
    memcpy(d, s, n);
}

int64_t HttpConn::relay_body_hashed_mb(HttpConn& dst, int64_t n, int64_t skip,
                                       int64_t full_len, int64_t piece_len, Progress* prog,
                                       std::string* digests, std::string* head,
                                       std::string* tail, uint32_t* crc,
                                       uint64_t* gpu_ticket) {
  PartLease lease((size_t)n);
  uint8_t* b = lease.b->data;
  int64_t pos = 0;
  const int64_t np = (full_len + piece_len - 1) / piece_len;
  const GpuPartHashApi* api = gpu_ticket ? g_gpu_api.load() : nullptr;
  const int nt = part_nt_mode();
  if (!ssl_ && !dst.ssl_ && relay_tee_on() &&
      (nt == 2 || (nt == 1 && api && np >= g_gpu_min_pieces.load()))) {
    thread_local std::vector<uint8_t> sbuf(peek_stage_bytes());
    relay_dup(
        dst, n, 0, prog,
        [&](size_t& len) {
          len = std::min({len, sbuf.size(), (size_t)(n - pos)});
          return sbuf.data();
        },
        [&](const uint8_t* p, size_t k) {
          if (crc) {
            uint64_t t0 = mono_ns();
            *crc = stager::crc32c(p, k, *crc);
            t_tally.crc_ns += mono_ns() - t0;
          }
          stream_copy(b + pos, p, k);
          pos += (int64_t)k;
        });
    g_rc.nt_bytes.fetch_add((uint64_t)pos, std::memory_order_relaxed);
  } else if (!ssl_ && !dst.ssl_ && relay_tee_on()) {
    relay_dup(
        dst, n, 0, prog,
        [&](size_t& len) {
          len = std::min<size_t>(len, (size_t)(n - pos));
          return b + pos;
        },
        [&](const uint8_t* p, size_t k) {
          if (crc) {
            uint64_t t0 = mono_ns();
            *crc = stager::crc32c(p, k, *crc);
            t_tally.crc_ns += mono_ns() - t0;
          }
          pos += (int64_t)k;
        });
  }
  while (pos < n) {
    if (prog && prog->cancelled.load(std::memory_order_relaxed)) {
      reusable_ = false;
      dst.reusable_ = false;
      throw IoError("cancelled");
    }
    const int64_t want = std::min<int64_t>(n - pos, 1 << 20);
    int64_t k = take_buffered(b + pos, want);
    if (k == 0) {
      size_t r;
      try {
        r = recv_some(b + pos, (size_t)want);
      } catch (...) {
        dst.reusable_ = false;
        throw;
      }
      if (r == 0) {
        reusable_ = false;
        dst.reusable_ = false;
        throw IoError("source closed mid-body");
      }
      k = (int64_t)r;
    }
    if (crc) *crc = stager::crc32c(b + pos, (size_t)k, *crc);
    try {
      dst.send_all(b + pos, (size_t)k);
    } catch (...) {
      reusable_ = false;
      throw;
    }
    pos += k;
    if (prog) prog->bytes.fetch_add(k, std::memory_order_relaxed);
  }
  head->assign((const char*)b, (size_t)skip);
  tail->assign((const char*)b + skip + full_len, (size_t)(n - skip - full_len));
  if (api && np >= g_gpu_min_pieces.load()) {
    PartBuffer* pb = lease.b.get();
    if (!pb->reg_api && api->reg(api->ctx, pb->data, pb->cap) == 0)
      pb->reg_api = api;
    if (pb->reg_api == api) {
      std::lock_guard<std::mutex> g(g_gpu_mu);
      const uint64_t t = api->submit(api->ctx, b + skip, full_len, piece_len);
// ... 33 lines not shown
```

downloader_amd/net/http.py:

```python
from __future__ import annotations

import asyncio
import os
import threading
import time
from concurrent.futures import ThreadPoolExecutor
from dataclasses import dataclass, field
from typing import Callable, Dict, List, Optional, Sequence, Set, Tuple, Union
from urllib.parse import quote, urljoin, urlsplit

from .proxy import Proxy, ProxyConfig
from ..utils.log import get_logger, redact_text, redact_url

log = get_logger("http.py")

Headers = Sequence[Tuple[str, str]]

REDIRECTS = (301, 302, 303, 307, 308)
MAX_REDIRECTS = 10


class HttpError(Exception):
    def __init__(self, msg: str, status: int = 0, body: bytes = b""):
        super().__init__(msg)
# ... 339 lines not shown
            host, port, path, headers = _via_proxy(proxy, url, headers)
        nprog = None
        if progress is not None:
            if progress.native is None:
                progress.native = self._n.Progress()
            nprog = progress.native
        loop = asyncio.get_running_loop()
        slot = self._new_slot()
        fut = loop.run_in_executor(self._exec, self._do, method, host, port, host_hdr, path,
                                   headers, body, sink, nprog, expect_body, slot, tls, tunnel)
        try:
            return await asyncio.shield(fut)
        except asyncio.CancelledError:
            self._abort_slot(slot)
            await _drain(fut)
            raise
        finally:
            self._end_slot(slot)

    def _new_slot(self) -> int:
        with self._lock:
            self._seq = getattr(self, "_seq", 0) + 1
            self._inflight.add(self._seq)
            return self._seq

    def _end_slot(self, slot: int) -> None:
        with self._lock:
            self._inflight.discard(slot)
            self._slots.pop(slot, None)
            self._aborted.discard(slot)

    def _relay(self, src_url: str, src_headers: Headers, dst_url: str, dst_headers: Headers,
               length: int, nprog, slot: int = 0, split: Optional[Tuple[int, int, int]] = None,
               src_proxy: Optional[Proxy] = None, checksum: bool = False, gpu: bool = False
               ) -> Tuple[Response, Optional[Response], int, Optional[dict]]:
        ss, sh, sp, spath = split_host(src_url)
        ds, dh, dp, dpath = split_host(dst_url)
        if not (self.handles(src_url, src_proxy is not None) and self.handles(dst_url)):
            raise TransportError(f"relay {ss}:// -> {ds}://"
                                 + (" through a proxy" if src_proxy is not None else "")
                                 + ": not supported by the native transport")
        stls, dtls = ss == "https", ds == "https"
        src_host_hdr = _host_hdr(sh, sp, stls)
        tunnel = src_proxy if stls else None
        if src_proxy is not None and not stls:
            sh, sp, spath, src_headers = _via_proxy(src_proxy, src_url, src_headers)
        get_head = _build_head("GET", src_host_hdr, spath, src_headers, None)
        put_head = _build_head("PUT", _host_hdr(dh, dp, dtls), dpath, dst_headers,
                               aws_chunked_length(length) if checksum else length)
        src, _ = self._acquire(sh, sp, stls, tunnel)
        self._track(slot, src)
        try:
            dst, _ = self._acquire(dh, dp, dtls)
        except BaseException:
            self._untrack(slot, src)
            self._release(src)
            raise
        self._track(slot, dst)
        try:
            if split is None:
                d = src.relay_to(get_head, dst, put_head, length, nprog, crc=checksum)
            else:
                d = src.relay_hashed_to(get_head, dst, put_head, length, *split, nprog,
                                        crc=checksum, gpu=gpu)
        except RuntimeError as e:
            self._untrack(slot, src)
            self._untrack(slot, dst)
            src.close()
            dst.close()
            raise TransportError(f"relay {spath} -> {dpath}: {e}") from e
        self._untrack(slot, src)
        self._untrack(slot, dst)
        self._release(src)
        self._release(dst)
        g = d["get"]
        get = Response(g["status"], list(g["headers"]), d["get_body"], 0, g.get("reason", ""))
        put = None
        if d["put"] is not None:
            p = d["put"]
            put = Response(p["status"], list(p["headers"]), d["put_body"], 0, p.get("reason", ""))
            put.sent_crc32c = d.get("crc32c", "")
        hashed = {k: d[k] for k in ("digests", "head", "tail", "gpu_ticket")} \
            if split is not None else None
        return get, put, d["moved"], hashed

    async def relay(self, src_url: str, src_headers: Headers, dst_url: str, dst_headers: Headers,
                    length: int, progress: Optional[Progress] = None,
                    split: Optional[Tuple[int, int, int]] = None,
                    src_proxy: Optional[ProxyConfig] = None, checksum: bool = False,
                    gpu: bool = False
                    ) -> Tuple[Response, Optional[Response], int, Optional[dict]]:
        nprog = None
        if progress is not None:
            if progress.native is None:
                progress.native = self._n.Progress()
            nprog = progress.native
        loop = asyncio.get_running_loop()
        for _ in range(MAX_REDIRECTS + 1):
            slot = self._new_slot()
            px = src_proxy.for_url(src_url) if src_proxy is not None else None
            fut = loop.run_in_executor(self._exec, self._relay, src_url, src_headers, dst_url,
                                       dst_headers, length, nprog, slot, split, px, checksum,
                                       gpu)
            try:
                out = await asyncio.shield(fut)
            except asyncio.CancelledError as ce:
                self._abort_slot(slot)
                await _drain(fut)
                held = await self._forget_ticket(fut)
                if held is not None:
                    ce.held_until = held
                raise
            finally:
                self._end_slot(slot)
            get, put = out[0], out[1]
            get.url = src_url
            nxt = redirect_target(src_url, get) if put is None else None
            if nxt is None:
                return out
            if not self.handles(nxt, src_proxy is not None and
                                src_proxy.for_url(nxt) is not None):
                raise TransportError(f"relay source {redact_url(src_url)} redirects to "
                                     f"{redact_url(nxt)}: not "
                                     f"supported by the socket relay", get.status)
            src_headers = redirect_headers(src_url, nxt, src_headers)
            src_url = nxt
        raise TransportError(f"relay source: more than {MAX_REDIRECTS} redirects", 310)

    FORGET_WAIT_S = 5.0

    async def _forget_ticket(self, fut: "asyncio.Future") -> Optional["asyncio.Future"]:
        if not fut.done() or fut.cancelled() or fut.exception() is not None:
            return None
        hashed = fut.result()[3]
        gid = hashed.get("gpu_ticket") if hashed else 0
        if not gid:
            return None
        loop = asyncio.get_running_loop()
        over = loop.create_future()

        def settle() -> None:
            if not over.done():
                over.set_result(None)

        def forget() -> None:
            try:
                self._n.gpu_part_forget(gid)
            finally:
                try:
                    loop.call_soon_threadsafe(settle)
                except RuntimeError:
                    pass
        threading.Thread(target=forget, name="gpu-part-forget", daemon=True).start()
        try:
            await asyncio.wait_for(asyncio.shield(over), self.FORGET_WAIT_S)
        except asyncio.TimeoutError:
            log.warn("gpu part forget still blocked: its budget stays held until it returns",
                        ticket=gid, waited_s=self.FORGET_WAIT_S)
            return over
        except asyncio.CancelledError:
            pass
        return None

    async def close(self) -> None:
        with self._lock:
            conns = [c for v in self._pool.values() for c, _ in v]
# ... 174 lines not shown
```

downloader_amd/ops/build.py:

```python
from __future__ import annotations

import os
import shutil
import subprocess
import sys
import sysconfig
from pathlib import Path
from typing import List, Sequence

PKG = Path(__file__).resolve().parents[1]
CSRC = PKG / "csrc"
OPS = PKG / "ops"
BIN = PKG / "bin"
EXT = sysconfig.get_config_var("EXT_SUFFIX") or ".so"
ROCM = Path(os.environ.get("ROCM_PATH", "/opt/rocm"))
ARCH = os.environ.get("PYTORCH_ROCM_ARCH", "gfx950")


def _pybind_includes() -> List[str]:
    import pybind11
    return [f"-I{pybind11.get_include()}", f"-I{sysconfig.get_paths()['include']}"]


def _stale(out: Path, srcs: Sequence[Path]) -> bool:
    if not out.exists():
        return True
    t = out.stat().st_mtime
    return any(s.stat().st_mtime > t for s in srcs)


def _run(cmd: List[str], verbose: bool) -> None:
    assert cmd[-2] == "-o", cmd
    out = cmd[-1]
    tmp = f"{out}.tmp.{os.getpid()}"
    cmd = cmd[:-1] + [tmp]
    if verbose:
        print("+", " ".join(cmd[:-1] + [out]), flush=True)
    r = subprocess.run(cmd, capture_output=True, text=True)
    if r.returncode != 0:
        try:
            os.unlink(tmp)
        except OSError:
            pass
        sys.stderr.write(r.stdout + r.stderr)
        raise RuntimeError(f"build failed: {' '.join(cmd[:3])} ... (exit {r.returncode})")
    os.replace(tmp, out)


def build_native(force: bool = False, verbose: bool = True) -> Path:
    srcs = [CSRC / "module.cpp", CSRC / "hashing.cpp", CSRC / "sha1_mb.cpp", CSRC / "transfer.cpp",
            CSRC / "tls.cpp", CSRC / "peerwire.cpp"]
    out = OPS / f"_native{EXT}"
    if force or _stale(out, srcs + [CSRC / "native.h", CSRC / "crc32c.h",
                                    CSRC / "gpu_part_api.h"]):
        cxx = os.environ.get("CXX", "g++")
        cmd = [cxx, "-O3", "-std=c++17", "-shared", "-fPIC", "-fvisibility=hidden",
               "-march=x86-64-v3", "-Wall", "-Wno-unused-result",
               *_pybind_includes(), *[str(s) for s in srcs], "-lssl", "-lcrypto", "-lpthread",
               "-o", str(out)]
        _run(cmd, verbose)
    return out


def build_gpuhash(force: bool = False, verbose: bool = True) -> Path:
    srcs = [CSRC / "gpu_sha1.hip"]
    out = OPS / f"_gpuhash{EXT}"
    if force or _stale(out, srcs + [CSRC / "gpu_part_api.h", CSRC / "part_dispatch.h"]):
        hipcc = str(ROCM / "bin" / "hipcc")
        cmd = [hipcc, f"--offload-arch={ARCH}", "-O3", "-std=c++17", "-shared", "-fPIC",
               "-fvisibility=hidden", *_pybind_includes(), str(srcs[0]), "-o", str(out)]
        _run(cmd, verbose)
    return out


def build_blobd(force: bool = False, verbose: bool = True) -> Path:
    srcs = [CSRC / "blobd.cpp"]
    BIN.mkdir(exist_ok=True)
    out = BIN / "blobd"
    if force or _stale(out, srcs + [CSRC / "crc32c.h"]):
        cxx = os.environ.get("CXX", "g++")
        cmd = [cxx, "-O3", "-std=c++17", "-march=x86-64-v3", "-Wall", str(srcs[0]),
               "-lssl", "-lcrypto", "-lpthread", "-o", str(out)]
        _run(cmd, verbose)
    return out


def build_swarmd(force: bool = False, verbose: bool = True) -> Path:
    srcs = [CSRC / "swarmd.cpp"]
    BIN.mkdir(exist_ok=True)
    out = BIN / "swarmd"
    if force or _stale(out, srcs):
        cxx = os.environ.get("CXX", "g++")
        cmd = [cxx, "-O2", "-std=c++17", "-Wall", str(srcs[0]), "-lpthread", "-o", str(out)]
        _run(cmd, verbose)
    return out


def build_relaybench(force: bool = False, verbose: bool = True) -> Path:
    srcs = [CSRC / "relaybench.cpp"]
    BIN.mkdir(exist_ok=True)
    out = BIN / "relaybench"
    if force or _stale(out, srcs + [CSRC / "crc32c.h"]):
        cxx = os.environ.get("CXX", "g++")
        cmd = [cxx, "-O3", "-std=c++17", "-march=x86-64-v3", "-Wall", str(srcs[0]),
               "-lpthread", "-o", str(out)]
        _run(cmd, verbose)
    return out


SANITIZERS = {"asan": ["-fsanitize=address,undefined", "-fno-omit-frame-pointer"],
              "tsan": ["-fsanitize=thread"]}


def build_selftest(kind: str, force: bool = False, verbose: bool = True) -> Path:
    srcs = [CSRC / "selftest.cpp", CSRC / "hashing.cpp", CSRC / "sha1_mb.cpp", CSRC / "transfer.cpp",
            CSRC / "tls.cpp", CSRC / "peerwire.cpp"]
    BIN.mkdir(exist_ok=True)
    out = BIN / f"selftest_{kind}"
    if force or _stale(out, srcs + [CSRC / "native.h", CSRC / "crc32c.h",
                                    CSRC / "gpu_part_api.h", CSRC / "part_dispatch.h"]):
        cxx = os.environ.get("CXX", "g++")
        cmd = [cxx, "-O1", "-g", "-std=c++17", "-msse4.2", *SANITIZERS[kind],
               *[str(s) for s in srcs],
               "-lssl", "-lcrypto", "-lpthread", "-o", str(out)]
        _run(cmd, verbose)
    return out


def build_all(force: bool = False, verbose: bool = True, gpu: bool = True) -> None:
    build_native(force, verbose)
    if (CSRC / "blobd.cpp").exists():
        build_blobd(force, verbose)
    if (CSRC / "relaybench.cpp").exists():
        build_relaybench(force, verbose)
    if (CSRC / "swarmd.cpp").exists():
        build_swarmd(force, verbose)
    if gpu and (CSRC / "gpu_sha1.hip").exists():
        if not (ROCM / "bin" / "hipcc").exists():
            raise RuntimeError("hipcc not found; cannot build the gfx950 kernels")
        build_gpuhash(force, verbose)


def clean() -> None:
    for p in OPS.glob("_*.so"):
        p.unlink()
    if BIN.exists():
        shutil.rmtree(BIN)


if __name__ == "__main__":
    build_all(force="--force" in sys.argv)
```

downloader_amd/ops/hashing.py:

```python
from __future__ import annotations

import collections
import os
import threading
import weakref
from typing import List, Optional, Sequence, Tuple

from . import gpu_available, gpuhash, native

FileList = Sequence[Tuple[str, int]]

GPU_MIN_BYTES = 256 << 20
GPU_MIN_PIECES = 256


def digest(algo: str, data) -> bytes:
    return native().digest(algo, data)


def sha1(data) -> bytes:
    return native().digest("sha1", data)


def sha256_hex(data) -> str:
    return native().digest("sha256", data).hex()


def md5(data) -> bytes:
    return native().digest("md5", data)


def crc32c(data, crc: int = 0) -> int:
    return native().crc32c(data, crc)


def crc32c_b64(data) -> str:
    n = native()
    return n.crc32c_base64(n.crc32c(data))


def crc32c_fd_b64(fd: int, offset: int, length: int) -> str:
    n = native()
    return n.crc32c_base64(n.crc32c_fd(fd, offset, length))


def new(algo: str):
    return native().Hasher(algo)


def hash_pieces(data, piece_len: int, algo: str = "sha1", threads: int = 0,
                backend: str = "cpu") -> bytes:
    if backend == "gpu":
        if algo != "sha1":
            raise ValueError("GPU backend implements SHA-1 only")
        return _verifier().hash_buffer(data, piece_len)
    return native().hash_pieces(algo, data, piece_len, threads)


def hash_storage_pieces(files: FileList, piece_len: int, algo: str = "sha1",
                        threads: int = 0) -> bytes:
    return native().hash_storage_pieces(list(files), piece_len, algo, threads)


def hash_file_ranges(path: str, ranges: Sequence[Tuple[int, int]], algo: str,
                     threads: int = 0) -> List[bytes]:
    return list(native().hash_file_ranges(path, list(ranges), algo, threads))


_gpu_lock = threading.Lock()
_gpu_verifier = None
GPU_COLD_MIN_BYTES = 32 << 30


def gpu_device() -> int:
    if os.environ.get("STAGER_GPU_DEVICE"):
        return int(os.environ["STAGER_GPU_DEVICE"])
    idx = int(os.environ.get("STAGER_WORKER_INDEX", os.environ.get("LOCAL_RANK", "0")) or 0)
    try:
        n = gpuhash().device_count()
    except Exception:
        n = 1
    return idx % max(1, n)


def _verifier():
    global _gpu_verifier
    with _gpu_lock:
        if _gpu_verifier is None:
            _gpu_verifier = gpuhash().GpuVerifier(gpu_device(), 256 << 20, 8)
        return _gpu_verifier


def prewarm_gpu() -> bool:
    if not gpu_available():
        return False
    _verifier()
    return True


_part_hasher = None
_part_hasher_failed = False
_retired_hashers: list = []

PART_SLOT_BYTES = 1 << 30
PART_SLOTS = 16


def gpu_relay_hashing(min_pieces: int = 8, slots: int = PART_SLOTS,
                      slot_bytes: int = PART_SLOT_BYTES, copy_streams: int = 2,
                      compute_streams: int = 0) -> bool:
    global _part_hasher, _part_hasher_failed
    with _gpu_lock:
        if _part_hasher is not None:
            return True
        if _part_hasher_failed or not gpu_available():
            return False
        try:
            ph = gpuhash().PartHasher(gpu_device(), int(slot_bytes), int(slots),
                                      int(compute_streams), 16384, int(copy_streams))
            native().set_gpu_part_hasher(ph.api(), min_pieces)
        except Exception:
            _part_hasher_failed = True
            raise
        _part_hasher = ph
        return True


def use_part_hasher(hasher, min_pieces: int = 8) -> None:
    global _part_hasher
    with _gpu_lock:
        native().set_gpu_part_hasher(hasher.api() if hasher is not None else None, min_pieces)
        if _part_hasher is not None and _part_hasher is not hasher:
            _retired_hashers.append(_part_hasher)
        _part_hasher = hasher


class GpuPart:

    def __init__(self, loop: "asyncio.AbstractEventLoop"):
        self.loop = loop
        self.copied = loop.create_future()
        self.done = loop.create_future()
        self.done.add_done_callback(_retrieve)

    def _deliver(self, kind: int, data: bytes) -> None:
        if not self.copied.done():
            self.copied.set_result(None)
        if self.done.done():
            return
        if kind == 2:
            self.done.set_result(data)
        elif kind == 3:
            self.done.set_exception(RuntimeError(data.decode(errors="replace")))


def _retrieve(fut) -> None:
    if not fut.cancelled():
        fut.exception()


EARLY_MAX = 4096


class _GpuParts:

    def __init__(self):
        self._lock = threading.Lock()
        self._parts: dict = {}
        self._early: dict = {}
        self._evicted: "collections.OrderedDict" = collections.OrderedDict()
        self._loops: "weakref.WeakSet" = weakref.WeakSet()

    def track(self, gid: int) -> GpuPart:
        import asyncio
        loop = asyncio.get_running_loop()
        self._watch(loop)
        part = GpuPart(loop)
        with self._lock:
            lost = self._evicted.pop(gid, None) is not None
            if not lost:
                self._parts[gid] = part
            early = self._early.pop(gid, [])
        if lost:
            part._deliver(3, b"GPU part completion lost before it was tracked")
            return part
        for kind, data in early:
            self._dispatch(gid, part, kind, data)
        self.drain()
        return part

    def _watch(self, loop) -> None:
        if loop in self._loops:
            return
        loop.add_reader(native().gpu_part_eventfd(), self.drain)
        self._loops.add(loop)

    def _dispatch(self, gid: int, part: GpuPart, kind: int, data: bytes) -> None:
        if kind != 1:
            with self._lock:
                self._parts.pop(gid, None)
        import asyncio
        try:
# ... 181 lines not shown
```

downloader_amd/service/worker.py:

```python
from __future__ import annotations

import asyncio
import time
from collections import deque
from dataclasses import dataclass, field
from typing import Any, Deque, Dict, List, Optional, Tuple

from ..broker.base import Broker, Delivery, make_broker
from ..models import api, keys
from ..net.http import TransportSet, make_transports
from ..s3.client import S3Client, S3Error
from ..stages import build_stages
from ..stages.base import EventEmitter, Job, Services, Stage
from ..stages.jobdir import get_reaper
from ..utils import limits
from ..utils.config import Config
from ..utils.log import Logger, get_logger, redact_text
from ..utils.metrics import Metrics
from ..utils.trace import Tracer, init_tracer
from .telemetry import Telemetry


@dataclass
class ActiveJob:
# ... 6 lines not shown
@dataclass
class JobResult:
    job_id: str
    outcome: str
    seconds: float
    bytes: int = 0
    error: str = ""
    stats: dict = field(default_factory=dict)


RESULTS_MAX = 10_000


def _attempt(headers: Dict[str, Any]) -> int:
    try:
        return max(0, min(1 << 20, int(headers.get("x-attempt", 0) or 0)))
    except (TypeError, ValueError, OverflowError):
        return 0


class Worker:
    def __init__(self, cfg: Config, broker: Optional[Broker] = None,
                 s3: Optional[S3Client] = None, transports: Optional[TransportSet] = None,
                 telemetry: Optional[Telemetry] = None, metrics: Optional[Metrics] = None,
                 tracer: Optional[Tracer] = None, logger: Optional[Logger] = None):
        self.cfg = cfg
        self.log = logger or get_logger("main")
        self.metrics = metrics or Metrics()
        self.broker = broker or make_broker(cfg, self.metrics)
        self.transports = transports or make_transports(
            native=cfg.s3.native_transport or cfg.download.http_native,
            max_workers=max(16, cfg.concurrency * 2 *
                            (cfg.s3.max_inflight_parts + cfg.download.http_streams)),
            connect_timeout=cfg.s3.connect_timeout_s, io_timeout=cfg.s3.request_timeout_s,
            ssl_verify=cfg.tls.verify, ca_file=cfg.tls.ca_file, native_tls=cfg.tls.native)
        self.s3 = s3 or S3Client.from_config(cfg.s3, self.transports)
        self.metrics.watch_runtime(self.transports)
        self.telemetry = telemetry or Telemetry.from_config(cfg, self.broker, self.log,
                                                            self.metrics)
        self.tracer = tracer or init_tracer("downloader", cfg.trace.enabled, cfg.trace.path)
        self.services = Services(cfg, self.telemetry, self.s3, self.transports, self.metrics,
                                 self.tracer, self.log)
        self.stages: List[Tuple[str, Stage]] = []
        self.active: Dict[int, ActiveJob] = {}
        self.results: Deque[JobResult] = deque(maxlen=RESULTS_MAX)
        self._consumer: Optional[str] = None
        self._inflight: set = set()
        self._stopping = False
        self._health = None
        self._seq = 0
        self.on_result = None

    async def init(self) -> None:
        await self.broker.connect()
        await self.telemetry.connect()
        for q in (self.cfg.broker.download_queue, self.cfg.broker.convert_queue,
                  self.cfg.broker.dead_letter_queue):
            await self.broker.declare(q)
        if not self.stages:
            self.stages = await build_stages(self.cfg.stages, self.cfg, self.services)
        get_reaper(self.services).sweep()
        d = self.cfg.download
        self.pipe_bytes = limits.apply_pipe_size(d.pipe_kb, d.pipe_sharers)
        if d.gpu_prewarm and d.stream_verify_backend == "gpu" and d.stream_gpu_pending > 0:
            await self._prewarm_part_hasher()
        if d.gpu_prewarm and d.verify_backend != "cpu":
            from ..ops import hashing
            if d.verify_backend == "auto" and not hashing.auto_may_use_gpu():
                return
            prewarm_gpu = hashing.prewarm_gpu
            try:
                warm = await asyncio.get_running_loop().run_in_executor(None, prewarm_gpu)
                self.log.info({"gpu_verifier": warm}, "gpu verifier prewarm")
            except Exception as e:
                self.log.warn({"err": str(e)}, "gpu verifier prewarm failed")

    async def _prewarm_part_hasher(self) -> None:
        from ..ops import gpu_available, hashing
        d = self.cfg.download
        loop = asyncio.get_running_loop()
        try:
            if not await loop.run_in_executor(None, gpu_available):
                return
            ok = await loop.run_in_executor(
                None, lambda: hashing.gpu_relay_hashing(
                    d.stream_gpu_min_pieces, d.stream_gpu_slots, d.stream_gpu_slot_mb << 20,
                    copy_streams=d.stream_gpu_copy_streams,
                    compute_streams=d.stream_gpu_compute_streams))
            self.log.info({"gpu_part_hasher": ok}, "gpu relay hashing prewarm")
        except Exception as e:
            self.log.warn({"err": str(e)}, "gpu relay hashing prewarm failed")

    async def start(self, health: bool = True) -> None:
        await self.init()
        self._consumer = await self.broker.consume(self.cfg.broker.download_queue,
                                                   self._on_delivery, self.cfg.broker.prefetch)
        if health and self.cfg.health.enabled:
            from .health import HealthServer
            self._health = HealthServer(self, self.cfg.health)
            await self._health.start()
        if self.cfg.metrics.enabled and self.cfg.metrics.port:
            self.metrics.expose(self.cfg.metrics.port)
        self.log.info("successfully connected to queue and started server")

    async def stop(self, drain_timeout: float = 30.0) -> int:
        self._stopping = True
        had_active = bool(self.active)
        if self._consumer is not None:
            try:
                await self.broker.cancel(self._consumer)
            except Exception:
                pass
            self._consumer = None
        if self._inflight:
            await asyncio.wait(list(self._inflight), timeout=drain_timeout)
        if self._health is not None:
            await self._health.stop()
        for _, st in self.stages:
            await st.close()
        await asyncio.get_running_loop().run_in_executor(None, get_reaper(self.services).close,
                                                         drain_timeout)
        await self.telemetry.close(timeout=2 * self.cfg.telemetry.publish_timeout_s)
        try:
            await self.broker.close()
        except Exception:
            pass
        await self.s3.close()
        await self.transports.close()
        self.tracer.close()
        return 1 if had_active and self.active else 0

    async def _on_delivery(self, d: Delivery) -> None:
        t = asyncio.current_task()
        self._inflight.add(t)
        try:
            await self.process(d)
        finally:
            self._inflight.discard(t)

    async def process(self, d: Delivery) -> JobResult:
        t0 = time.perf_counter()
        try:
            msg = api.decode(api.Download, d.body)
        except Exception as e:
            self.log.error("undecodable message dropped to dead-letter", err=str(e))
            await self._dead_letter(d, f"decode: {e}")
            return self._finish(None, JobResult("", "dead", time.perf_counter() - t0, error=str(e)))
        media = msg.media
        job_id, creator = media.id, media.creatorId
        attempt = _attempt(d.headers)
        child = self.log.child(jobId=job_id, fileId=creator)
        self._seq += 1
        slot = self._seq
        self.active[slot] = ActiveJob(job_id, creator)
        self.metrics.inflight.inc()
        await self.telemetry.emit_status(job_id, api.STATUS_DOWNLOADING)
        emitter = EventEmitter()
        job = Job(msg=msg, media=media, logger=child, emitter=emitter, attempt=attempt,
                  headers=dict(d.headers))
        outcome, err = "staged", ""
        try:
            with self.tracer.span("job", traceparent=d.headers.get("traceparent"),
                                  job_id=job_id, attempt=attempt) as span:
                staged = await self._already_staged(job_id, child)
                if not staged:
                    child.info("starting main processor after successful stage init")
# ... 174 lines not shown
```

downloader_amd/torrent/stream.py:

```python
from __future__ import annotations

import asyncio
import hashlib
import os
import time
import weakref
from dataclasses import dataclass, field
from typing import Dict, List, Optional, Set, Tuple

from ..models import keys
from ..stages.base import media_type
from ..net.http import TransportError
from ..utils.aio import gather_strict
from ..utils import membudget
from ..utils.log import redact_url
from .metainfo import Metainfo
from .session import TorrentError, webseed_url


@dataclass(eq=False)
class _Target:
    path: str
    key: str
    index: int
# ... 96 lines not shown
        except Exception:
            pass
    if idle_s <= 0:
        _trim_relay_buffers()
    else:
        _trim_handle = asyncio.get_running_loop().call_later(idle_s, _trim_relay_buffers)


def piece_split(meta: Metainfo, start: int, length: int) -> Tuple[int, int]:
    plen, end = meta.piece_length, start + length
    ps = -(-start // plen) * plen
    pe = end if end == meta.total_length else (end // plen) * plen
    if pe <= ps:
        return min(ps - start, length), 0
    return ps - start, pe - ps


class StreamStager:
    def __init__(self, meta: Metainfo, job, cfg, sv, selected: List[str], root: str,
                 webseeds: List[str], parallel: int = 16, max_failures: int = 5):
        self.meta = meta
        self.job = job
        self.sv = sv
        self.s3 = sv.s3
        self.bucket = cfg.s3.bucket
        self.webseeds = list(webseeds)
        self.plen = meta.piece_length
        self.parallel = max(1, parallel)
        self.max_failures = max(1, max_failures)
        self.cfg = cfg
        self.trim_idle_s = float(getattr(getattr(cfg, "download", None),
                                         "relay_pool_idle_trim_s", 0.0) or 0.0)
        self.budget_bytes = membudget.relay_budget_bytes(getattr(cfg, "download", None))
        self._budget: Optional[membudget.PartBudget] = None
        index = {os.path.abspath(p): i for i, (p, _) in enumerate(meta.local_files(root))}
        self.selected = [os.path.abspath(f) for f in selected]
        self.sizes = {f: meta.files[index[f]].length for f in self.selected}
        owner: Dict[str, str] = {}
        for f in self.selected:
            owner[keys.object_key(job.id, f)] = f
        self.targets: List[_Target] = []
        self.units: List[_Unit] = []
        for key, f in owner.items():
            fe = meta.files[index[f]]
            t = _Target(f, key, index[f], fe.offset, fe.length,
                        fe.length <= self.s3.multipart_threshold)
            self.targets.append(t)
            if t.size == 0:
                continue
            parts = [(0, 0, t.size)] if t.single else \
                self.s3.plan_parts(t.size, fe.offset, meta.piece_length)
            for num, off, ln in parts:
                skip, full = piece_split(meta, t.offset + off, ln)
                self.units.append(_Unit(len(self.units), t.offset + off, ln, t, num, off,
                                        skip, full))
        self.frags: Dict[int, Dict[int, bytes]] = {}
        self.suppliers: Dict[int, Set[int]] = {}
        self._plan_gaps()
        self.verified: Set[int] = set()
        self._checking: Set[int] = set()
        self.frag_ver: Dict[int, int] = {}
        self.piece_fails: Dict[int, int] = {}
        self.total = sum(t.size for t in self.targets)
        self.fetched_bytes = 0
        self.done_bytes = 0
        self.hash_fails = 0
        self.error: Optional[BaseException] = None
        self._outstanding = 0
        self._finished = asyncio.Event()
        self.stats = {"relay_s": 0.0, "gap_bytes": 0, "units": 0}
        self.timeline: Dict[str, float] = {}
        self._t0 = time.monotonic()
        self._gpu_slots: Optional[asyncio.Semaphore] = None
        self.gpu_pending = 0
        self._continuations: Set[asyncio.Task] = set()
        d = getattr(cfg, "download", None)
        gpu_pending = int(getattr(d, "stream_gpu_pending", 0) or 0)
        self.verify_mode = getattr(d, "stream_verify_backend", "cpu") if gpu_pending > 0 else "cpu"
        self._min_pieces = int(getattr(d, "stream_gpu_min_pieces", 8) or 8)
        self._gpu_dev_slots = int(getattr(d, "stream_gpu_slots", 16) or 16)
        self._gpu_copy_streams = int(getattr(d, "stream_gpu_copy_streams", 2) or 2)
        self._gpu_compute_streams = int(getattr(d, "stream_gpu_compute_streams", 0) or 0)
        self._gpu_slot_bytes = int(getattr(d, "stream_gpu_slot_mb", 1024) or 1024) << 20
        self.gpu_tail = int(getattr(d, "stream_gpu_tail", 0) or 0)
        self._n_parts = sum(1 for u in self.units if u.target is not None)
        from ..ops import hashing
        try:
            self._host_mb = hashing.host_multibuffer()
        except Exception:
            self._host_mb = False
        if self.verify_mode == "auto":
            self.gpu_pending = gpu_pending
            self.stats["verify"] = "auto"
        if self.verify_mode == "gpu":
            why = _gpu_relay_on(cfg)
            if why is None:
                self.gpu_pending = gpu_pending
                self.stats["verify"] = "gpu"
            else:
                self.stats["verify_fallback"] = why
                job.logger.warn("GPU piece hashing unavailable, hashing on the host", err=why)

    def _piece_range(self, p: int) -> Tuple[int, int]:
        return p * self.plen, p * self.plen + self.meta.piece_size(p)

    def _plan_gaps(self) -> None:
        covered: Dict[int, List[Tuple[int, int]]] = {}
        for u in self.units:
            for a, b in u.fragments():
                p = a // self.plen
                covered.setdefault(p, []).append((a, b))
                self.suppliers.setdefault(p, set()).add(u.uid)
        for p in sorted(covered):
            lo, hi = self._piece_range(p)
            pos = lo
            for a, b in sorted(covered[p]) + [(hi, hi)]:
                if a > pos:
                    g = _Unit(len(self.units), pos, a - pos)
                    self.units.append(g)
                    self.suppliers[p].add(g.uid)
                pos = max(pos, b)
            self.frags[p] = {}

    @property
    def progress(self) -> float:
        return 1.0 if self.total == 0 else min(1.0, self.done_bytes / self.total)

    def skipped_bytes(self) -> int:
        return self.meta.total_length - sum(u.length for u in self.units)

    async def run(self) -> List[dict]:
        global _active_stagers
        multi = [t for t in self.targets if not t.single and t.size]
        _active_stagers += 1
        if _trim_handle is not None:
            _trim_handle.cancel()
        self._budget = membudget.part_budget(self.budget_bytes)
        self._t0 = time.monotonic()
        self.stats["timeline"] = self.timeline
        try:
            from ..ops import native
            native().relay_pool_set_max_idle(POOL_IDLE_MAX)
        except Exception:
            pass
        if self.verify_mode == "auto" and self._gpu_wanted():
            start_gpu_init(self._min_pieces, self._gpu_dev_slots, self._gpu_copy_streams,
                           self._gpu_compute_streams, self._gpu_slot_bytes)
        try:
            for t in self.targets:
                if t.size == 0:
                    await self.s3.put_object(self.bucket, t.key, b"", self._ctype(t))
            async def create(t: _Target) -> None:
                t.upload_id = await self.s3.create_multipart_upload(
                    self.bucket, t.key, self._ctype(t),
                    checksum=self.s3.want_checksum(relay=True, hashed=True))
            await gather_strict(*(create(t) for t in multi), cancel=False)
            self._mark("created_s")
            queue: "asyncio.Queue[_Unit]" = asyncio.Queue()
            for u in self.units:
                queue.put_nowait(u)
            self._outstanding = len(self.units)
            if not self.units:
                self._finished.set()
            workers = [asyncio.ensure_future(self._worker(queue)) for _ in range(self.parallel)]
            try:
                await self._finished.wait()
                self._mark("settled_s")
            finally:
                for w in workers + list(self._continuations):
                    w.cancel()
                await asyncio.gather(*workers, *self._continuations, return_exceptions=True)
            if self.error is not None:
                raise self.error
            unverified = [p for p in self.frags if p not in self.verified]
            if unverified:
                raise TorrentError(f"pieces {unverified[:5]} never verified")
            async def complete(t: _Target) -> None:
                await self.s3.complete_multipart_upload(self.bucket, t.key, t.upload_id,
                                                        sorted(t.etags.items()))
                t.completed = True
            await gather_strict(*(complete(t) for t in multi), cancel=False)
            self._mark("completed_s")
        except BaseException:
            await asyncio.shield(self.abort())
            raise
        finally:
            _active_stagers -= 1
            self.stats["budget"] = self._budget.stats()
            if _active_stagers == 0:
                _schedule_trim(self.trim_idle_s,
                               self.parallel * membudget.buffer_bytes(self.s3.part_size))
        return [{"file": f, "key": keys.object_key(self.job.id, f), "size": self.sizes[f],
                 "virtual": True} for f in self.selected]

    async def _worker(self, queue: "asyncio.Queue[_Unit]") -> None:
        while True:
            u = await queue.get()
            u.state = "running"
            if u.target is not None and self._gpu_sem() is not None:
                await self._gpu_slots.acquire()
                try:
                    nb = await self._budget.acquire(u.length)
                except BaseException:
                    self._gpu_slots.release()
                    raise
                gpu = self._gpu_now() and queue.qsize() >= self.gpu_tail
                try:
                    res = await self._relay_part(u, gpu)
                except BaseException as e:
                    self._release_after(e, nb)
                    self._gpu_slots.release()
                    if not await self._unit_failed(u, e, queue):
                        return
                    continue
                gid = res[1].get("gpu_ticket")
                if gid:
                    from ..ops import hashing
                    try:
                        part = hashing.gpu_part_track(gid)
                    except BaseException as e:
                        await self._forget_part(gid)
                        self._budget.release(nb)
                        self._gpu_slots.release()
                        if not await self._unit_failed(u, e, queue):
                            return
                        continue
                    part.copied.add_done_callback(lambda _f, nb=nb: self._budget.release(nb))
                    t = asyncio.ensure_future(self._complete(u, res, part, queue))
                    self._continuations.add(t)
                    t.add_done_callback(self._continuations.discard)
                    continue
                self._budget.release(nb)
                self._gpu_slots.release()
                try:
                    requeue = await self._after_fetch(u, self._accept(u, *res,
                                                                       res[1]["digests"]))
                except BaseException as e:
                    if not await self._unit_failed(u, e, queue):
                        return
                    continue
            else:
                try:
                    requeue = await self._process(u)
                except BaseException as e:
                    if not await self._unit_failed(u, e, queue):
                        return
                    continue
            if self.error is not None:
                return
            self._settle(u, requeue, queue)

    def _mark(self, key: str, first: bool = False) -> None:
        t = round(time.monotonic() - self._t0, 4)
        if not first or key not in self.timeline:
            self.timeline[key] = t

    def _release_after(self, e: BaseException, nb: int) -> None:
        held = getattr(e, "held_until", None)
        if held is not None and not held.done():
            held.add_done_callback(lambda _f, nb=nb: self._budget.release(nb))
        else:
            self._budget.release(nb)

    async def _forget_part(self, gid: int) -> None:
        from ..ops import native
        try:
            await asyncio.get_running_loop().run_in_executor(None, native().gpu_part_forget, gid)
        except Exception:
            pass

    def _gpu_wanted(self) -> bool:
        return not self._host_mb or _active_stagers >= 2 or self._n_parts > self.gpu_tail

    def _gpu_sem(self) -> Optional[asyncio.Semaphore]:
        if self._gpu_slots is None and self.gpu_pending:
            from ..ops import hashing
            if hashing._part_hasher is not None:
                self._gpu_slots = _gpu_pending_sem(self.gpu_pending)
        return self._gpu_slots

    def _gpu_now(self) -> bool:
        if self.verify_mode == "gpu":
            return True
        if self._gpu_wanted():
            return True
        return False

    async def _unit_failed(self, u: _Unit, e: BaseException,
                           queue: "asyncio.Queue[_Unit]") -> bool:
        if not isinstance(e, (TransportError, OSError)):
            self._fail(e)
            return False
        u.attempts += 1
        if u.attempts >= self.max_failures:
            self._fail(TorrentError(f"webseed failed: {e}"))
            return False
        await asyncio.sleep(min(5.0, 0.1 * (2 ** u.attempts)))
        if self.error is not None:
            return False
        self._settle(u, [u], queue)
        return True

    async def _complete(self, u: _Unit, res, part, queue: "asyncio.Queue[_Unit]") -> None:
        etag, h = res
        try:
            try:
                digests = await part.done
            except RuntimeError as e:
                self.stats["gpu_failures"] = self.stats.get("gpu_failures", 0) + 1
                raise TransportError(f"part {u.num}: {e}") from e
# ... 203 lines not shown
```

downloader_amd/utils/config.py:

```python
from __future__ import annotations

import os
from pathlib import Path
from typing import Any, Dict, List, Literal, Mapping, Optional

import yaml
from pydantic import BaseModel, Field

MiB = 1024 * 1024


class InstanceConfig(BaseModel):
    download_path: str = "downloads"
    per_attempt_dirs: bool = True
    background_cleanup: bool = True


class S3Config(BaseModel):
    endpoint: str = "127.0.0.1:9000"
    access_key: str = "minioadmin"
    secret_key: str = "minioadmin"
    session_token: str = ""
    region: str = "us-east-1"
    secure: bool = False
    bucket: str = "triton-staging"
    part_size: int = 64 * MiB
    multipart_threshold: int = 64 * MiB
    max_inflight_parts: int = 8
    concurrent_files: int = 4
    unsigned_payload: bool = True
    content_type_by_extension: bool = True
    resume_uploads: bool = True
    native_transport: bool = True
    addressing: Literal["auto", "path", "virtual"] = "auto"
    split_tls_relays: bool = True
    checksum: Literal["auto", "always", "off"] = "always"
    connect_timeout_s: float = 10.0
    request_timeout_s: float = 300.0
    retries: int = 3
    relay_resume_min_bytes: int = 1 << 30
    sweep_stale_uploads: bool = True


class BrokerConfig(BaseModel):
    backend: Literal["amqp", "memory"] = "amqp"
    url: str = ""
    prefetch: int = 1
    max_retries: int = 2
    download_queue: str = "v1.download"
    convert_queue: str = "v1.convert"
    dead_letter_queue: str = "v1.download.dead"
    retry_backoff_s: float = 0.5
    retry_backoff_max_s: float = 30.0
    heartbeat_s: int = 30
    publish_retry_s: float = 120.0
    reconnect_delay_s: float = 1.0
    connect_retry_s: float = 60.0
    recover_delay_s: float = 1.0
    retry_delay: Literal["queue", "sleep"] = "queue"
    ca_file: str = ""
    cert_file: str = ""
    key_file: str = ""


class TelemetryConfig(BaseModel):
    enabled: bool = True
    status_queue: str = "v1.telemetry.status"
    progress_queue: str = "v1.telemetry.progress"
    publish_timeout_s: float = 1.0
    retry_max_s: float = 5.0
    buffer_max: int = 10_000


class DownloadConfig(BaseModel):
    torrent_metadata_timeout_s: float = 240.0
    torrent_stall_timeout_s: float = 240.0
    progress_interval_s: float = 30.0
    allow_file_urls: bool = False
    http_streams: int = 4
    http_min_split: int = 32 * MiB
    http_timeout_s: float = 300.0
    http_min_rate: float = 0.0
    http_native: bool = True
    http_proxy: str = "env"
    stream_http: bool = True
    eager_upload: bool = True
    torrent_stream: Literal["auto", "always", "off"] = "auto"
    torrent_stream_parallel: int = 32
    relay_memory_mb: int = 0
    relay_memory_fraction: float = 0.25
    relay_pool_idle_trim_s: float = 60.0
    pipe_kb: int = 0
    pipe_sharers: int = 4
    bucket_concurrency: int = 4
    bucket_secure: bool = True
    stream_bucket: bool = True
    bucket_server_copy: bool = True
    stream_file: bool = True
    verify_backend: Literal["cpu", "gpu", "auto"] = "auto"
    stream_verify_backend: Literal["cpu", "gpu", "auto"] = "auto"
    stream_gpu_pending: int = 160
    stream_gpu_slots: int = 16
    stream_gpu_slot_mb: int = 1024
    stream_gpu_copy_streams: int = 2
    stream_gpu_compute_streams: int = 0
    stream_gpu_min_pieces: int = 8
    stream_gpu_tail: int = 32
    verify_threads: int = 0
    gpu_prewarm: bool = True
    torrent_listen_port: int = 0
    torrent_max_peers: int = 32
    torrent_enable_dht: bool = True
    torrent_dht_bootstrap: List[str] = Field(default_factory=list)
    torrent_default_trackers: List[str] = Field(default_factory=list)
    torrent_enable_trackers: bool = True
    torrent_enable_webseeds: bool = True
    torrent_request_pipeline: int = 16
    torrent_native_wire: bool = True
    torrent_wire_requests: bool = True
    swarm_verify_backend: str = "auto"
    swarm_gpu_min_gb: float = 1.5
    swarm_verify_threads: int = 4
    swarm_wire_io_threads: int = 4
    swarm_pool_mb: int = 0
    swarm_gpu_inflight: int = 1024
    swarm_gpu_tail_mb: int = -1
    swarm_gpu_tail_x: float = 3.0
    swarm_gpu_tail_max: float = 0.85
    swarm_backlog_mb: int = 0
    webseed_streams: int = 4
    webseed_chunk: int = 64 * MiB
    webseed_verify_depth: int = 2
    webseed_verify_depth_gpu: int = 32
    min_free_bytes: int = 0
    cleanup_on_stall: bool = True
    emit_errored_on_stall: bool = False


class ProcessConfig(BaseModel):
    media_exts: List[str] = Field(default_factory=lambda: [".mp4", ".mkv", ".mov", ".webm"])
    case_insensitive_exts: bool = False
    legacy_full_path_extras: bool = False
    legacy_any_depth_sole_dir: bool = False


class HealthConfig(BaseModel):
    enabled: bool = True
    host: str = "0.0.0.0"
    port: int = 3401
    legacy_idle_500: bool = True


class MetricsConfig(BaseModel):
    enabled: bool = True
    port: int = 0


class TraceConfig(BaseModel):
    enabled: bool = False
    path: str = ""


class TlsConfig(BaseModel):
    verify: bool = True
    ca_file: str = ""
    native: bool = True


class Config(BaseModel):
    name: str = "downloader"
    mode: Literal["tuned", "reference"] = "tuned"
    concurrency: int = 4
    instance: InstanceConfig = Field(default_factory=InstanceConfig)
    s3: S3Config = Field(default_factory=S3Config)
    broker: BrokerConfig = Field(default_factory=BrokerConfig)
    telemetry: TelemetryConfig = Field(default_factory=TelemetryConfig)
    download: DownloadConfig = Field(default_factory=DownloadConfig)
    process: ProcessConfig = Field(default_factory=ProcessConfig)
    health: HealthConfig = Field(default_factory=HealthConfig)
    metrics: MetricsConfig = Field(default_factory=MetricsConfig)
    trace: TraceConfig = Field(default_factory=TraceConfig)
    tls: TlsConfig = Field(default_factory=TlsConfig)
    stages: List[str] = Field(default_factory=lambda: ["download", "process", "upload"])

    def apply_mode(self) -> "Config":
        if self.mode == "reference":
            self.concurrency = 1
            self.broker.prefetch = 1
# ... 92 lines not shown
```

Before: 55170.

## Stream relay chunks into a GPU inbox while downloading instead of after

Adds a device-side inbox of blocks and a stage_open/push/submit API so the hashed relay pushes each received chunk to the GPU asynchronously through a small pinned ring. Previously the whole part had to be buffered on the host before it was submitted and copied. The intent is to overlap the host-to-device copy with network receive, release the host memory budget as soon as the part is submitted, and cut per-part latency. In exchange it allocates an extra 2 GiB inbox on the device, adds device-to-device copies from inbox to slot, and brings in event-pool locking and a more complex failure path. Whether it is on depends on part_stream_enabled (STAGER_PART_STREAM).

```diff
diff --git a/downloader_amd/csrc/gpu_part_api.h b/downloader_amd/csrc/gpu_part_api.h
--- a/downloader_amd/csrc/gpu_part_api.h
+++ b/downloader_amd/csrc/gpu_part_api.h
@@ -3,7 +3,7 @@
 #include <stddef.h>
 #include <stdint.h>
 
-#define GPU_PART_API_ABI 2u
+#define GPU_PART_API_ABI 3u
 #define GPU_PART_COPIED 1
 #define GPU_PART_DONE 2
 
@@ -18,4 +18,10 @@
   int (*wait)(void* ctx, uint64_t ticket, int phase, uint8_t* out, size_t out_len, char* err,
               size_t errlen);
   void (*set_notify)(void* ctx, gpu_part_notify_fn fn, void* arg);
+  uint64_t (*stage_open)(void* ctx, int64_t len, int64_t piece_len);
+  uint64_t (*stage_push)(void* ctx, uint64_t handle, int64_t off, const uint8_t* host,
+                         int64_t len);
+  int (*stage_wait)(void* ctx, uint64_t token);
+  uint64_t (*stage_submit)(void* ctx, uint64_t handle);
+  void (*stage_abort)(void* ctx, uint64_t handle);
 };
diff --git a/downloader_amd/csrc/gpu_sha1.hip b/downloader_amd/csrc/gpu_sha1.hip
--- a/downloader_amd/csrc/gpu_sha1.hip
+++ b/downloader_amd/csrc/gpu_sha1.hip
@@ -1065,14 +1065,17 @@
   using Event = hipEvent_t;
 
   HipPartDevice(int device, int64_t slot_bytes, int slots, int streams, int max_lanes,
-                int copy_streams)
-      : device_(device), slot_bytes_(slot_bytes), max_lanes_(max_lanes) {
+                int copy_streams, int inbox_blocks = 0, int64_t inbox_block_bytes = 0)
+      : device_(device), slot_bytes_(slot_bytes), max_lanes_(max_lanes),
+        inbox_blocks_(inbox_blocks), block_bytes_(inbox_block_bytes) {
     int n = 0;
     HIP_CHECK(hipGetDeviceCount(&n));
     if (device < 0 || device >= n) throw std::runtime_error("no such HIP device");
     if (slots < 2 || slot_bytes < (1 << 20) || max_lanes < 64 || copy_streams < 1 ||
-        copy_streams > 4)
+        copy_streams > 4 || inbox_blocks < 0 || inbox_blocks > 1024 ||
+        (inbox_blocks > 0 && inbox_block_bytes < 4096))
       throw std::invalid_argument("PartHasher: bad geometry");
+    block_bytes_ = std::min(block_bytes_, slot_bytes_);
     HIP_CHECK(hipSetDevice(device_));
     try {
       create(slots, streams, copy_streams);
@@ -1111,6 +1114,50 @@
     HIP_CHECK(hipEventRecord(e, st));
     return e;
   }
+  int inbox_blocks() const { return inbox_blocks_; }
+  int64_t inbox_block_bytes() const { return block_bytes_; }
+  uint64_t stage_copy(int b, int64_t off, const uint8_t* host, int64_t len, int cs) noexcept {
+    if (b < 0 || b >= inbox_blocks_ || off < 0 || len <= 0 || off + len > block_bytes_) return 0;
+    if (!bind_caller()) return 0;
+    hipStream_t st = copies_[(size_t)cs];
+    hipEvent_t e = nullptr;
+    {
+      std::lock_guard<std::mutex> g(stage_mu_);
+      if (!stage_events_.empty()) {
+        e = stage_events_.back();
+        stage_events_.pop_back();
+      }
+    }
+    if (!e && hipEventCreateWithFlags(&e, hipEventDisableTiming) != hipSuccess) return 0;
+    if (hipMemcpyAsync(inbox_ + (size_t)b * (size_t)block_bytes_ + (size_t)off, host, (size_t)len,
+                       hipMemcpyHostToDevice, st) != hipSuccess ||
+        hipEventRecord(e, st) != hipSuccess) {
+      stage_put(e);
+      return 0;
+    }
+    return (uint64_t)(uintptr_t)e;
+  }
+  int stage_wait(uint64_t token) noexcept {
+    hipEvent_t e = (hipEvent_t)(uintptr_t)token;
+    if (!bind_caller()) return -1;
+    hipError_t q = hipEventQuery(e);
+    if (q == hipErrorNotReady) q = hipEventSynchronize(e);
+    stage_put(e);
+    return q == hipSuccess ? 0 : -1;
+  }
+  Event copy_block(int s, int64_t off, int b, int64_t len, int cs) {
+    hipStream_t st = copies_[(size_t)cs];
+    HIP_CHECK(hipMemcpyAsync(slots_[(size_t)s].d_data + off,
+                             inbox_ + (size_t)b * (size_t)block_bytes_, (size_t)len,
+                             hipMemcpyDeviceToDevice, st));
+    Event e = take_event();
+    HIP_CHECK(hipEventRecord(e, st));
+    return e;
+  }
+  void drain_stream(int cs) noexcept {
+    if (bind_caller()) hipStreamSynchronize(copies_[(size_t)cs]);
+  }
+
   bool copied(Event e) { return query(e); }
   void recycle(Event e) {
     if (e) free_events_.push_back(e);
@@ -1184,6 +1231,18 @@
     hipEvent_t done = nullptr;
   };
 
+  bool bind_caller() noexcept {
+    thread_local int bound = -1;
+    if (bound == device_) return true;
+    if (hipSetDevice(device_) != hipSuccess) return false;
+    bound = device_;
+    return true;
+  }
+  void stage_put(hipEvent_t e) noexcept {
+    std::lock_guard<std::mutex> g(stage_mu_);
+    stage_events_.push_back(e);
+  }
+
   static bool query(hipEvent_t e) {
     hipError_t q = hipEventQuery(e);
     if (q == hipErrorNotReady) return false;
@@ -1200,6 +1259,8 @@
     for (auto& st : streams_) HIP_CHECK(hipStreamCreateWithFlags(&st, hipStreamNonBlocking));
     slots_.resize((size_t)slots);
     HIP_CHECK(hipMalloc((void**)&arena_, (size_t)slot_bytes_ * (size_t)slots + kArenaPad));
+    if (inbox_blocks_ > 0)
+      HIP_CHECK(hipMalloc((void**)&inbox_, (size_t)block_bytes_ * (size_t)inbox_blocks_));
     for (size_t k = 0; k < slots_.size(); ++k) {
       Slot& sl = slots_[k];
       sl.d_data = arena_ + (size_t)slot_bytes_ * k;
@@ -1232,6 +1293,10 @@
       if (c) hipStreamDestroy(c);
     if (arena_) hipFree(arena_);
     arena_ = nullptr;
+    if (inbox_) hipFree(inbox_);
+    inbox_ = nullptr;
+    for (hipEvent_t e : stage_events_) hipEventDestroy(e);
+    stage_events_.clear();
     for (auto& sl : slots_) {
       if (sl.h_lane) hipHostFree(sl.h_lane);
       for (auto e : sl.copied)
@@ -1274,6 +1339,11 @@
   std::vector<Slot> slots_;
   std::vector<Run> runs_;
   std::vector<hipEvent_t> free_events_;
+  int inbox_blocks_ = 0;
+  int64_t block_bytes_ = 0;
+  uint8_t* inbox_ = nullptr;
+  std::mutex stage_mu_;
+  std::vector<hipEvent_t> stage_events_;
 };
 
 using PartHasher = stager::PartDispatcher<HipPartDevice>;
@@ -1294,6 +1364,11 @@
   d["register_s"] = s.register_s;
   d["copy_streams"] = s.copy_streams;
   d["compute_streams"] = s.compute_streams;
+  d["staged_parts"] = s.staged_parts;
+  d["staged_chunks"] = s.staged_chunks;
+  d["stage_refused"] = s.stage_refused;
+  d["inbox_blocks"] = s.inbox_blocks;
+  d["inbox_free"] = s.inbox_free;
   d["kernel"] = h.device().split() ? "sha1_lanes_split" : "sha1_lanes";
   return d;
 }
@@ -1442,13 +1517,14 @@
       .def_property_readonly("batch_bytes", &GpuVerifier::batch_bytes);
   py::class_<PartHasher>(m, "PartHasher")
       .def(py::init([](int device, int64_t slot_bytes, int slots, int streams, int max_lanes,
-                       int copy_streams) {
+                       int copy_streams, int inbox_blocks, int64_t inbox_block_bytes) {
              py::gil_scoped_release rel;
              return new PartHasher(slot_bytes, max_lanes, device, slot_bytes, slots, streams,
-                                   max_lanes, copy_streams);
+                                   max_lanes, copy_streams, inbox_blocks, inbox_block_bytes);
            }),
            py::arg("device") = 0, py::arg("slot_bytes") = (int64_t)1 << 30, py::arg("slots") = 8,
-           py::arg("streams") = 0, py::arg("max_lanes") = 16384, py::arg("copy_streams") = 2)
+           py::arg("streams") = 0, py::arg("max_lanes") = 16384, py::arg("copy_streams") = 2,
+           py::arg("inbox_blocks") = 32, py::arg("inbox_block_bytes") = (int64_t)64 << 20)
       .def(
           "api",
           [](PartHasher& h) {
@@ -1478,5 +1554,31 @@
             return py::bytes(out);
           },
           py::arg("data"), py::arg("piece_len"))
+      .def(
+          "hash_streamed",
+          [](PartHasher& h, const py::buffer& b, int64_t piece_len, int64_t chunk, int ring,
+             int64_t skip, int64_t tail) {
+            py::buffer_info info = b.request();
+            const int64_t n = (int64_t)info.size * (int64_t)info.itemsize;
+            const int64_t full = n - skip - tail;
+            if (piece_len <= 0 || chunk <= 0 || ring <= 0 || skip < 0 || tail < 0 || full <= 0)
+              throw std::invalid_argument("hash_streamed: bad sizes");
+            const int64_t np = (full + piece_len - 1) / piece_len;
+            std::string out((size_t)np * 20, '\0');
+            char err[256] = {0};
+            int rc = -1;
+            {
+              py::gil_scoped_release rel;
+              rc = stager::stream_part(h.api(), (const uint8_t*)info.ptr, n, skip, full, piece_len,
+                                       chunk, ring, (uint8_t*)out.data(), out.size(), err,
+                                       sizeof err);
+            }
+            if (rc != 0) throw std::runtime_error(err[0] ? err : "PartHasher refused the part");
+            return py::bytes(out);
+          },
+          py::arg("data"), py::arg("piece_len"), py::arg("chunk") = (int64_t)512 << 10,
+          py::arg("ring") = 4, py::arg("skip") = 0, py::arg("tail") = 0,
+          "Digests of the pieces in data[skip : len - tail], the body streamed through the "
+          "inbox chunk by chunk as the hashed relay does")
       .def("stats", &part_stats);
 }
diff --git a/downloader_amd/csrc/module.cpp b/downloader_amd/csrc/module.cpp
--- a/downloader_amd/csrc/module.cpp
+++ b/downloader_amd/csrc/module.cpp
@@ -8,9 +8,12 @@
 #include <sys/socket.h>
 
 #include "native.h"
+#include "part_dispatch.h"
+#include "part_fake_device.h"
 
 namespace py = pybind11;
 using namespace stager;
+using FakeHasher = PartDispatcher<FakePartDevice>;
 
 namespace {
 
@@ -149,6 +152,7 @@
   d["crc32c"] = crc_b64;
   if (split) {
     d["gpu_ticket"] = ticket;
+    d["streamed"] = ticket != 0 && gpu_part_streamed(ticket);
     d["digests"] = py::bytes(digests);
     d["head"] = py::bytes(head);
     d["tail"] = py::bytes(tail);
@@ -233,8 +237,127 @@
     d["host_fallbacks"] = s.host_fallbacks;
     d["refused"] = s.refused;
     d["pending"] = s.pending;
+    d["streamed"] = s.streamed;
+    d["stream_failed"] = s.stream_failed;
     return d;
   });
+  m.def("set_part_stream", &set_part_stream, py::arg("on"),
+        "STAGER_PART_STREAM at run time: 1 / 0, -1 reads the environment again");
+  m.def("part_stream_enabled", &part_stream_enabled);
+  py::class_<FakeHasher>(m, "FakePartHasher",
+                         "PartDispatcher (part_dispatch.h) on the host-thread fake device: the "
+                         "PartHasher's state machine, streamed parts included, without a GPU")
+      .def(py::init([](int64_t slot_bytes, int slots, int max_lanes, int inbox_blocks,
+                       int64_t inbox_block_bytes, int fail_launch_at, int fail_push_at,
+                       int kernel_us_max, uint32_t seed) {
+             FakeDeviceKnobs k;
+             k.fail_launch_at = fail_launch_at;
+             k.fail_push_at = fail_push_at;
+             k.kernel_us_max = kernel_us_max;
+             k.seed = seed;
+             return new FakeHasher(slot_bytes, max_lanes, slot_bytes, slots,  2,
+                                    2, max_lanes, k, inbox_blocks, inbox_block_bytes);
+           }),
+           py::arg("slot_bytes") = (int64_t)8 << 20, py::arg("slots") = 4,
+           py::arg("max_lanes") = 256, py::arg("inbox_blocks") = 4,
+           py::arg("inbox_block_bytes") = 0, py::arg("fail_launch_at") = 0,
+           py::arg("fail_push_at") = 0, py::arg("kernel_us_max") = 1500, py::arg("seed") = 1)
+      .def("api",
+           [](FakeHasher& h) { return py::capsule((void*)h.api(), "downloader_amd.gpu_part_api"); })
+      .def("set_stage_open_wait_us", &FakeHasher::set_stage_open_wait_us)
+      .def(
+          "hash",
+          [](FakeHasher& h, const py::bytes& data, int64_t piece_len) {
+            const std::string d = data;
+            const int64_t np = piece_len > 0 ? ((int64_t)d.size() + piece_len - 1) / piece_len : 0;
+            std::string out((size_t)np * 20, '\0');
+            char err[256] = {0};
+            int rc;
+            {
+              py::gil_scoped_release rel;
+              const uint64_t t = h.submit((const uint8_t*)d.data(), (int64_t)d.size(), piece_len);
+              rc = t ? h.wait(t, GPU_PART_DONE, (uint8_t*)&out[0], out.size(), err, sizeof err) : -1;
+            }
+            if (rc != 0) throw std::runtime_error(err[0] ? err : "refused");
+            return py::bytes(out);
+          },
+          py::arg("data"), py::arg("piece_len"))
+      .def(
+          "hash_streamed",
+          [](FakeHasher& h, const py::bytes& data, int64_t piece_len, int64_t chunk, int ring,
+             int64_t skip, int64_t tail) {
+            const std::string d = data;
+            const int64_t n = (int64_t)d.size(), full = n - skip - tail;
+            if (piece_len <= 0 || chunk <= 0 || ring <= 0 || skip < 0 || tail < 0 || full <= 0)
+              throw std::invalid_argument("hash_streamed: bad sizes");
+            const int64_t np = (full + piece_len - 1) / piece_len;
+            std::string out((size_t)np * 20, '\0');
+            char err[256] = {0};
+            int rc;
+            {
+              py::gil_scoped_release rel;
+              rc = stream_part(h.api(), (const uint8_t*)d.data(), n, skip, full, piece_len, chunk,
+                               ring, (uint8_t*)&out[0], out.size(), err, sizeof err);
+            }
+            if (rc != 0) throw std::runtime_error(err[0] ? err : "refused");
+            return py::bytes(out);
+          },
+          py::arg("data"), py::arg("piece_len"), py::arg("chunk") = 65536, py::arg("ring") = 4,
+          py::arg("skip") = 0, py::arg("tail") = 0)
+      .def("stage_open", [](FakeHasher& h, int64_t len, int64_t pl) {
+        py::gil_scoped_release rel;
+        return h.stage_open(len, pl);
+      })
+      .def("stage_push", [](FakeHasher& h, uint64_t handle, int64_t off, const py::bytes& data) {
+        const std::string d = data;
+        py::gil_scoped_release rel;
+        const uint64_t t = h.stage_push(handle, off, (const uint8_t*)d.data(), (int64_t)d.size());
+        return t != 0 && h.stage_wait(t) == 0;
+      })
+      .def("stage_submit", [](FakeHasher& h, uint64_t handle) {
+        py::gil_scoped_release rel;
+        return h.stage_submit(handle);
+      })
+      .def("stage_abort", [](FakeHasher& h, uint64_t handle) {
+        py::gil_scoped_release rel;
+        h.stage_abort(handle);
+      })
+      .def("submit_held",
+           [](FakeHasher& h, const py::bytes& data, int64_t piece_len) {
+             char* p;
+             Py_ssize_t n;
+             if (PyBytes_AsStringAndSize(data.ptr(), &p, &n) != 0) throw py::error_already_set();
+             return h.submit((const uint8_t*)p, (int64_t)n, piece_len);
+           })
+      .def("wait",
+           [](FakeHasher& h, uint64_t ticket, int phase, int np) -> py::object {
+             std::string out((size_t)np * 20, '\0');
+             char err[256] = {0};
+             int rc;
+             {
+               py::gil_scoped_release rel;
+               rc = h.wait(ticket, phase, (uint8_t*)&out[0], out.size(), err, sizeof err);
+             }
+             if (rc != 0) throw std::runtime_error(err[0] ? err : "wait failed");
+             return phase == GPU_PART_DONE ? (py::object)py::bytes(out) : py::none();
+           })
+      .def("stats", [](FakeHasher& h) {
+        const PartDispatchStats s = h.stats();
+        py::dict d;
+        d["submitted"] = s.submitted;
+        d["launches"] = s.launches;
+        d["lanes"] = s.lanes;
+        d["multi_slot_launches"] = s.multi_slot_launches;
+        d["max_launch_slots"] = s.max_launch_slots;
+        d["broken"] = s.broken;
+        d["pending"] = s.pending;
+        d["staged_parts"] = s.staged_parts;
+        d["staged_chunks"] = s.staged_chunks;
+        d["stage_refused"] = s.stage_refused;
+        d["inbox_blocks"] = s.inbox_blocks;
+        d["inbox_free"] = s.inbox_free;
+        return d;
+      });
   m.def("relay_pool_trim", &relay_pool_trim, py::arg("keep_bytes") = 0,
         "Unmap idle hashed-relay part buffers beyond keep_bytes; returns the bytes freed");
   m.def("relay_pool_set_budget", &relay_pool_set_budget, py::arg("bytes"),
diff --git a/downloader_amd/csrc/native.h b/downloader_amd/csrc/native.h
--- a/downloader_amd/csrc/native.h
+++ b/downloader_amd/csrc/native.h
@@ -132,8 +132,13 @@
 void swarm_piece_pool_limit(size_t bytes);
 struct GpuPartStats {
   uint64_t submitted, host_fallbacks, refused, pending;
+  uint64_t streamed;
+  uint64_t stream_failed;
 };
 GpuPartStats gpu_part_stats();
+bool gpu_part_streamed(uint64_t id);
+void set_part_stream(int on);
+bool part_stream_enabled();
 std::string gpu_part_wait(uint64_t id);
 void gpu_part_forget(uint64_t id);
 int gpu_part_eventfd();
diff --git a/downloader_amd/csrc/part_dispatch.h b/downloader_amd/csrc/part_dispatch.h
--- a/downloader_amd/csrc/part_dispatch.h
+++ b/downloader_amd/csrc/part_dispatch.h
@@ -1,8 +1,10 @@
 #pragma once
 
 #include <algorithm>
+#include <atomic>
 #include <chrono>
 #include <condition_variable>
+#include <cstdio>
 #include <cstring>
 #include <deque>
 #include <exception>
@@ -27,6 +29,9 @@
   bool broken = false;
   size_t pending = 0;
   int copy_streams = 0, compute_streams = 0;
+  uint64_t staged_parts = 0, staged_chunks = 0;
+  uint64_t stage_refused = 0;
+  int inbox_blocks = 0, inbox_free = 0;
 };
 
 template <class Dev>
@@ -37,6 +42,7 @@
       : dev_(std::forward<A>(dev_args)...), slot_bytes_(slot_bytes), max_lanes_(max_lanes) {
     slots_.resize((size_t)dev_.slots());
     running_.resize((size_t)dev_.compute_streams());
+    blocks_ = std::vector<Block>((size_t)dev_.inbox_blocks());
     api_.abi = GPU_PART_API_ABI;
     api_.ctx = this;
     api_.reg = [](void* c, void* p, size_t n) { return ((PartDispatcher*)c)->reg(p, n); };
@@ -53,6 +59,17 @@
       h->notify_ = fn;
       h->notify_arg_ = arg;
     };
+    if (!blocks_.empty()) {
+      api_.stage_open = [](void* c, int64_t len, int64_t pl) {
+        return ((PartDispatcher*)c)->stage_open(len, pl);
+      };
+      api_.stage_push = [](void* c, uint64_t h, int64_t off, const uint8_t* p, int64_t n) {
+        return ((PartDispatcher*)c)->stage_push(h, off, p, n);
+      };
+      api_.stage_wait = [](void* c, uint64_t t) { return ((PartDispatcher*)c)->stage_wait(t); };
+      api_.stage_submit = [](void* c, uint64_t h) { return ((PartDispatcher*)c)->stage_submit(h); };
+      api_.stage_abort = [](void* c, uint64_t h) { ((PartDispatcher*)c)->stage_abort(h); };
+    }
     thread_ = std::thread([this] { run(); });
     pthread_setname_np(thread_.native_handle(), "gpu-part-disp");
   }
@@ -105,6 +122,97 @@
     return t;
   }
 
+  uint64_t stage_open(int64_t len, int64_t piece_len) {
+    if (len <= 0 || piece_len <= 0 || blocks_.empty()) return 0;
+    const int64_t np = (len + piece_len - 1) / piece_len;
+    if (np > max_lanes_ || len > slot_bytes_ || len > dev_.inbox_block_bytes()) return 0;
+    std::unique_lock<std::mutex> lk(mu_);
+    int b = -1;
+    auto pick = [&] {
+      if (broken_ || stop_) return true;
+      for (size_t i = 0; i < blocks_.size(); ++i)
+        if (blocks_[i].state == 0) {
+          b = (int)i;
+          return true;
+        }
+      return false;
+    };
+    if (!pick())
+      scv_.wait_until(lk, std::chrono::system_clock::now() + std::chrono::microseconds(open_wait_us_),
+                      pick);
+    if (b < 0 || broken_ || stop_) {
+      stats_.stage_refused++;
+      return 0;
+    }
+    Block& bl = blocks_[(size_t)b];
+    bl.state = 1;
+    bl.len = len;
+    bl.piece_len = piece_len;
+    bl.cs = (int)(next_copy_stage_++ % (size_t)dev_.copy_streams());
+    const uint64_t h = ++stage_gen_ * kHandleStride + (uint64_t)b;
+    bl.handle.store(h, std::memory_order_release);
+    return h;
+  }
+
+  uint64_t stage_push(uint64_t h, int64_t off, const uint8_t* host, int64_t len) {
+    Block* bl = block_of(h);
+    if (!bl || len <= 0 || off < 0 || off + len > bl->len) return 0;
+    if (broken_flag_.load(std::memory_order_acquire)) return 0;
+    const uint64_t tok = dev_.stage_copy((int)(bl - blocks_.data()), off, host, len, bl->cs);
+    if (tok) {
+      staged_chunks_.fetch_add(1, std::memory_order_relaxed);
+    } else {
+      broken_flag_.store(true, std::memory_order_release);
+      {
+        std::lock_guard<std::mutex> g(mu_);
+        stage_fault_ = true;
+      }
+      cv_.notify_all();
+    }
+    return tok;
+  }
+
+  int stage_wait(uint64_t token) { return token ? dev_.stage_wait(token) : -1; }
+
+  uint64_t stage_submit(uint64_t h) {
+    Block* bl = block_of(h);
+    if (!bl) return 0;
+    std::unique_lock<std::mutex> lk(mu_);
+    if (bl->state != 1) return 0;
+    if (broken_ || stop_) {
+      lk.unlock();
+      release_open(bl);
+      return 0;
+    }
+    bl->state = 2;
+    uint64_t t = ++seq_;
+    Job& j = jobs_[t];
+    j.block = (int)(bl - blocks_.data());
+    j.len = bl->len;
+    j.piece_len = bl->piece_len;
+    j.np = (int)((bl->len + bl->piece_len - 1) / bl->piece_len);
+    queue_.push_back(t);
+    stats_.submitted++;
+    stats_.staged_parts++;
+    cv_.notify_all();
+    return t;
+  }
+
+  void stage_abort(uint64_t h) {
+    Block* bl = block_of(h);
+    if (!bl) return;
+    {
+      std::lock_guard<std::mutex> g(mu_);
+      if (bl->state != 1) return;
+    }
+    release_open(bl);
+  }
+
+  void set_stage_open_wait_us(int us) {
+    std::lock_guard<std::mutex> g(mu_);
+    open_wait_us_ = us;
+  }
+
   int wait(uint64_t t, int phase, uint8_t* out, size_t out_len, char* err, size_t errlen) {
     std::unique_lock<std::mutex> lk(mu_);
     auto it = jobs_.find(t);
@@ -133,12 +241,25 @@
     s.pending = jobs_.size();
     s.copy_streams = dev_.copy_streams();
     s.compute_streams = dev_.compute_streams();
+    s.staged_chunks = staged_chunks_.load(std::memory_order_relaxed);
+    s.inbox_blocks = (int)blocks_.size();
+    for (auto& b : blocks_) s.inbox_free += b.state == 0;
     return s;
   }
 
  private:
   using Event = typename Dev::Event;
+  static constexpr uint64_t kHandleStride = 4096;
+  struct Block {
+    int state = 0;
+    int64_t len = 0, piece_len = 0;
+    int cs = 0;
+    std::atomic<uint64_t> handle{0};
+    Block() = default;
+    Block(const Block&) {}
+  };
   struct Job {
+    int block = -1;
     const uint8_t* host = nullptr;
     int64_t len = 0, piece_len = 0;
     int np = 0;
@@ -184,6 +305,23 @@
     return jobs_.at(t);
   }
 
+  Block* block_of(uint64_t h) {
+    const size_t b = (size_t)(h % kHandleStride);
+    if (!h || b >= blocks_.size()) return nullptr;
+    return blocks_[b].handle.load(std::memory_order_acquire) == h ? &blocks_[b] : nullptr;
+  }
+  void free_block(int b) {
+    Block& bl = blocks_[(size_t)b];
+    bl.handle.store(0, std::memory_order_release);
+    bl.state = 0;
+    scv_.notify_all();
+  }
+  void release_open(Block* bl) {
+    dev_.drain_stream(bl->cs);
+    std::lock_guard<std::mutex> g(mu_);
+    free_block((int)(bl - blocks_.data()));
+  }
+
   void run() {
     std::vector<uint64_t> owed_copied, owed_done;
     std::deque<uint64_t> copying;
@@ -196,7 +334,8 @@
           std::unique_lock<std::mutex> lk(mu_);
           const bool idle = queue_.empty() && copying.empty() && !any_running() &&
                             !any_closed() && !(filling >= 0 && slots_[(size_t)filling].lanes > 0);
-          if (idle) cv_.wait(lk, [&] { return stop_ || !queue_.empty(); });
+          if (idle) cv_.wait(lk, [&] { return stop_ || stage_fault_ || !queue_.empty(); });
+          if (stage_fault_) throw std::runtime_error("a streamed chunk copy was refused");
           if (stop_ && idle && queue_.empty()) return;
           fresh.swap(queue_);
         }
@@ -227,7 +366,9 @@
           Slot& f = slots_[(size_t)filling];
           const int64_t off = (f.used + 255) & ~(int64_t)255;
           const int cs = (int)(next_copy_++ % (size_t)dev_.copy_streams());
-          Event ev = dev_.copy(filling, off, j->host, j->len, cs);
+          Event ev = j->block >= 0
+                         ? dev_.copy_block(filling, off, j->block, j->len, blocks_[(size_t)j->block].cs)
+                         : dev_.copy(filling, off, j->host, j->len, cs);
           int64_t* lt = dev_.lane_table(filling);
           for (int k = 0; k < j->np; ++k) {
             const int64_t po = (int64_t)k * j->piece_len;
@@ -265,6 +406,7 @@
             j->copied = true;
             ev = j->copy_ev;
             j->copy_ev = Event{};
+            if (j->block >= 0) free_block(j->block);
             owed_copied.push_back(*it);
           }
           dev_.recycle(ev);
@@ -290,6 +432,7 @@
                 j.done = true;
                 if (!j.copied) {
                   j.copied = true;
+                  if (j.block >= 0) free_block(j.block);
                   late.push_back(j.copy_ev);
                   j.copy_ev = Event{};
                   auto c = std::find(copying.begin(), copying.end(), t);
@@ -361,9 +504,11 @@
       {
         std::lock_guard<std::mutex> g(mu_);
         broken_ = true;
+        broken_flag_.store(true, std::memory_order_release);
         for (auto& kv : jobs_)
           if (!kv.second.done) {
             kv.second.err = std::string("GPU part hasher: ") + e.what();
+            if (kv.second.block >= 0 && !kv.second.copied) free_block(kv.second.block);
             (kv.second.copied ? failed_hash : failed_copy).push_back(kv.first);
           }
         queue_.clear();
@@ -402,10 +547,17 @@
   int64_t slot_bytes_;
   int max_lanes_;
   size_t next_copy_ = 0;
+  size_t next_copy_stage_ = 0;
+  uint64_t stage_gen_ = 0;
+  int open_wait_us_ = 2000;
+  bool stage_fault_ = false;
+  std::vector<Block> blocks_;
+  std::atomic<uint64_t> staged_chunks_{0};
+  std::atomic<bool> broken_flag_{false};
   std::vector<std::vector<int>> running_;
   std::vector<Slot> slots_;
   std::mutex mu_;
-  std::condition_variable cv_, wcv_;
+  std::condition_variable cv_, wcv_, scv_;
   std::deque<uint64_t> queue_;
   std::unordered_map<uint64_t, Job> jobs_;
   uint64_t seq_ = 0;
@@ -417,4 +569,48 @@
   std::thread thread_;
 };
 
+inline int stream_part(const GpuPartHashApi* a, const uint8_t* data, int64_t n, int64_t skip,
+                       int64_t full_len, int64_t piece_len, int64_t chunk, int ring,
+                       uint8_t* out, size_t out_len, char* err, size_t errlen) {
+  auto fail = [&](const char* m) {
+    if (err && errlen) snprintf(err, errlen, "%s", m);
+    return -1;
+  };
+  if (!a->stage_open) return fail("hasher has no streamed path");
+  if (skip < 0 || full_len <= 0 || skip + full_len > n) return fail("bad piece split");
+  const uint64_t h = a->stage_open(a->ctx, full_len, piece_len);
+  if (!h) return fail("stage_open refused");
+  std::vector<uint8_t> mem((size_t)chunk * (size_t)ring + 4096);
+  uint8_t* base = (uint8_t*)(((uintptr_t)mem.data() + 4095) & ~(uintptr_t)4095);
+  const bool locked = a->reg(a->ctx, base, (size_t)chunk * (size_t)ring) == 0;
+  std::vector<uint64_t> tok((size_t)ring, 0);
+  bool ok = true;
+  int i = 0;
+  for (int64_t off = 0; ok && off < n; off += chunk, i = (i + 1) % ring) {
+    if (tok[(size_t)i]) {
+      ok = a->stage_wait(a->ctx, tok[(size_t)i]) == 0;
+      tok[(size_t)i] = 0;
+      if (!ok) break;
+    }
+    const int64_t k = std::min(chunk, n - off);
+    uint8_t* p = base + (size_t)i * (size_t)chunk;
+    memcpy(p, data + off, (size_t)k);
+    const int64_t lo = std::max(off, skip), hi = std::min(off + k, skip + full_len);
+    if (lo >= hi) continue;
+    tok[(size_t)i] = a->stage_push(a->ctx, h, lo - skip, p + (lo - off), hi - lo);
+    ok = tok[(size_t)i] != 0;
+  }
+  for (uint64_t& t : tok)
+    if (t) ok = (a->stage_wait(a->ctx, t) == 0) && ok;
+  uint64_t ticket = 0;
+  if (ok)
+    ticket = a->stage_submit(a->ctx, h);
+  else
+    a->stage_abort(a->ctx, h);
+  if (locked) a->unreg(a->ctx, base);
+  if (!ok) return fail("streamed copy failed");
+  if (!ticket) return fail("stage_submit refused");
+  return a->wait(a->ctx, ticket, GPU_PART_DONE, out, out_len, err, errlen);
 }
+
+}
diff --git a/downloader_amd/csrc/part_fake_device.h b/downloader_amd/csrc/part_fake_device.h
--- a/downloader_amd/csrc/part_fake_device.h
+++ b/downloader_amd/csrc/part_fake_device.h
@@ -1,5 +1,6 @@
 #pragma once
 
+#include <algorithm>
 #include <atomic>
 #include <chrono>
 #include <condition_variable>
@@ -24,6 +25,7 @@
   double lag = 0.3;
   int fail_launch_at = 0;
   int fail_query_at = 0;
+  int fail_push_at = 0;
   uint32_t seed = 1;
 };
 
@@ -32,8 +34,12 @@
   using Event = std::shared_ptr<std::atomic<int>>;
 
   FakePartDevice(int64_t slot_bytes, int slots, int compute_streams, int copy_streams,
-                 int max_lanes, FakeDeviceKnobs k)
-      : max_lanes_(max_lanes), k_(k), rng_(k.seed) {
+                 int max_lanes, FakeDeviceKnobs k, int inbox_blocks = 4,
+                 int64_t inbox_block_bytes = 0)
+      : max_lanes_(max_lanes), k_(k), rng_(k.seed),
+        block_bytes_(inbox_block_bytes > 0 ? inbox_block_bytes : slot_bytes) {
+    inbox_.resize((size_t)inbox_blocks);
+    for (auto& b : inbox_) b.assign((size_t)block_bytes_, 0);
     slots_.resize((size_t)slots);
     for (auto& s : slots_) {
       s.mem.assign((size_t)slot_bytes, 0);
@@ -70,6 +76,31 @@
     });
     return e;
   }
+  int inbox_blocks() const { return (int)inbox_.size(); }
+  int64_t inbox_block_bytes() const { return block_bytes_; }
+  uint64_t stage_copy(int b, int64_t off, const uint8_t* host, int64_t len, int cs) noexcept {
+    if (k_.fail_push_at && ++pushes_ == k_.fail_push_at) return 0;
+    Event e = std::make_shared<std::atomic<int>>(0);
+    uint8_t* dst = inbox_[(size_t)b].data() + off;
+    Queue* q = copies_[(size_t)cs].get();
+    const int us = std::min(k_.copy_us_max, 50);
+    q->push([dst, host, len, e, us, q] {
+      q->nap(us);
+      memcpy(dst, host, (size_t)len);
+      e->store(1, std::memory_order_release);
+    });
+    return (uint64_t)(uintptr_t) new Event(std::move(e));
+  }
+  int stage_wait(uint64_t token) noexcept {
+    Event* e = (Event*)(uintptr_t)token;
+    while (!(*e)->load(std::memory_order_acquire)) std::this_thread::yield();
+    delete e;
+    return 0;
+  }
+  Event copy_block(int s, int64_t off, int b, int64_t len, int cs) {
+    return copy(s, off, inbox_[(size_t)b].data(), len, cs);
+  }
+  void drain_stream(int cs) noexcept { copies_[(size_t)cs]->drain(); }
   bool copied(const Event& e) {
     tick();
     if (!e->load(std::memory_order_acquire)) return false;
@@ -197,6 +228,9 @@
   FakeDeviceKnobs k_;
   std::mt19937 rng_;
   int launches_ = 0, queries_ = 0;
+  std::atomic<int> pushes_{0};
+  int64_t block_bytes_;
+  std::vector<std::vector<uint8_t>> inbox_;
   std::vector<Slot> slots_;
   std::vector<Run> runs_;
   std::vector<std::unique_ptr<Queue>> copies_, computes_;
diff --git a/downloader_amd/csrc/selftest.cpp b/downloader_amd/csrc/selftest.cpp
--- a/downloader_amd/csrc/selftest.cpp
+++ b/downloader_amd/csrc/selftest.cpp
@@ -766,7 +766,211 @@
   CHECK(st.lanes == (uint64_t)parts * pieces && st.pending == 0);
 }
 
+struct NotifyLog {
+  std::mutex mu;
+  std::vector<std::pair<uint64_t, int>> seen;
+};
+static void log_notify(void* arg, uint64_t ticket, int phase) {
+  NotifyLog* l = (NotifyLog*)arg;
+  std::lock_guard<std::mutex> g(l->mu);
+  l->seen.push_back({ticket, phase});
+}
+
+static void stream_section() {
+  Watchdog wd("streamed parts", 90);
+  {
+    FakeDeviceKnobs k;
+    k.seed = 11;
+    std::unique_ptr<FakeHasher> h(new FakeHasher(8 << 20, 256, 8 << 20, 4, 2, 2, 256, k));
+    const int64_t piece = 256 << 10;
+    const int shapes[][2] = {{1, 0}, {3, 0}, {16, 0}, {3, 100001}, {16, 1}};
+    const int64_t edges[] = {0, 1, 4095};
+    bool ok = true;
+    for (auto& s : shapes)
+      for (int64_t skip : edges)
+        for (int64_t tail : edges) {
+          const int64_t full = s[0] * piece - s[1], n = skip + full + tail;
+          auto body = rnd((size_t)n, (uint32_t)(s[0] * 31 + skip + tail));
+          std::string want = hash_pieces("sha1", body.data() + skip, (size_t)full, (size_t)piece, 1);
+          std::string got((size_t)s[0] * 20, '\0');
+          char err[256] = {0};
+          const int rc = stream_part(h->api(), body.data(), n, skip, full, piece, 64 << 10, 4,
+                                     (uint8_t*)&got[0], got.size(), err, sizeof err);
+          if (rc != 0 || got != want) {
+            fprintf(stderr, "streamed: %d pieces skip %lld tail %lld: %s\n", s[0], (long long)skip,
+                    (long long)tail, rc ? err : "digest mismatch");
+            ok = false;
+          }
+        }
+    CHECK(ok);
+    const PartDispatchStats st = h->stats();
+    CHECK(st.staged_parts == 45 && st.inbox_free == st.inbox_blocks && !st.broken);
+  }
+  {
+    FakeDeviceKnobs k;
+    k.kernel_us_max = 40000;
+    k.copy_us_max = 100;
+    k.seed = 5;
+    std::unique_ptr<FakeHasher> h(new FakeHasher(1 << 20, 64, 1 << 20, 4, 2, 2, 64, k, 4));
+    const GpuPartHashApi* api = h->api();
+    NotifyLog log;
+    api->set_notify(api->ctx, &log_notify, &log);
+    const int64_t piece = 16 << 10;
+    const int parts = 96, pieces = 8;
+    auto data = rnd((size_t)parts * pieces * piece, 23);
+    std::vector<uint64_t> tickets;
+    for (int i = 0; i < parts; ++i) {
+      const uint8_t* p = data.data() + (size_t)i * pieces * piece;
+      uint64_t t = 0;
+      if (i % 2) {
+        uint64_t hd = 0;
+        while (!(hd = api->stage_open(api->ctx, pieces * piece, piece))) {}
+        for (int64_t off = 0; off < pieces * piece; off += 24 << 10) {
+          const int64_t len = std::min<int64_t>(24 << 10, pieces * piece - off);
+          const uint64_t tok = api->stage_push(api->ctx, hd, off, p + off, len);
+          CHECK(tok != 0 && api->stage_wait(api->ctx, tok) == 0);
+        }
+        t = api->stage_submit(api->ctx, hd);
+      } else {
+        while (!(t = api->submit(api->ctx, p, pieces * piece, piece)))
+          std::this_thread::sleep_for(std::chrono::microseconds(50));
+      }
+      CHECK(t != 0);
+      tickets.push_back(t);
+    }
+    bool ok = true;
+    for (int i = 0; i < parts; ++i) {
+      uint8_t dig[pieces * 20];
+      char err[256] = {0};
+      if (api->wait(api->ctx, tickets[(size_t)i], GPU_PART_DONE, dig, sizeof dig, err, sizeof err) != 0) {
+        ok = false;
+        continue;
+      }
+      for (int q = 0; q < pieces; ++q) {
+        const uint8_t* pc = data.data() + ((size_t)i * pieces + q) * piece;
+        if (digest("sha1", pc, (size_t)piece) != std::string((const char*)dig + q * 20, 20)) ok = false;
+      }
+    }
+    CHECK(ok);
+    const PartDispatchStats st = h->stats();
+    CHECK(st.staged_parts == parts / 2 && st.lanes == (uint64_t)parts * pieces);
+    fprintf(stderr, "streamed + whole: %llu launches, %llu spanning >= 2 slots\n",
+            (unsigned long long)st.launches, (unsigned long long)st.multi_slot_launches);
+    CHECK(st.multi_slot_launches > 0 && st.launches * 2 <= (uint64_t)parts);
+    CHECK(st.inbox_free == st.inbox_blocks && st.pending == 0);
+    h.reset();
+    std::map<uint64_t, int> last;
+    bool ordered = log.seen.size() == (size_t)parts * 2;
+    for (auto& e : log.seen) {
+      if (e.second != last[e.first] + 1) ordered = false;
+      last[e.first] = e.second;
+    }
+    CHECK(ordered);
+  }
+  {
+    FakeDeviceKnobs k;
+    k.fail_launch_at = 1;
+    std::unique_ptr<FakeHasher> h(new FakeHasher(4 << 20, 256, 4 << 20, 4, 2, 2, 256, k, 3));
+    const GpuPartHashApi* api = h->api();
+    auto buf = rnd(1 << 20, 77);
+    uint64_t a = api->stage_open(api->ctx, 1 << 20, 1 << 16);
+    uint64_t tok = api->stage_push(api->ctx, a, 0, buf.data(), 1 << 19);
+    CHECK(a && tok && api->stage_wait(api->ctx, tok) == 0);
+    api->stage_abort(api->ctx, a);
+    CHECK(h->stats().inbox_free == 3);
+    CHECK(api->stage_push(api->ctx, a, 0, buf.data(), 16) == 0);
+    uint64_t held[3];
+    for (auto& x : held) CHECK((x = api->stage_open(api->ctx, 1 << 20, 1 << 16)) != 0);
+    CHECK(api->stage_open(api->ctx, 1 << 20, 1 << 16) == 0 && h->stats().stage_refused == 1);
+    api->stage_abort(api->ctx, held[1]);
+    api->stage_abort(api->ctx, held[2]);
+    tok = api->stage_push(api->ctx, held[0], 0, buf.data(), 1 << 19);
+    CHECK(tok && api->stage_wait(api->ctx, tok) == 0);
+    uint64_t t = api->submit(api->ctx, buf.data(), 1 << 20, 1 << 16);
+    uint8_t dig[16 * 20];
+    char err[256] = {0};
+    CHECK(t && api->wait(api->ctx, t, GPU_PART_DONE, dig, sizeof dig, err, sizeof err) != 0);
+    CHECK(h->stats().broken);
+    CHECK(api->stage_push(api->ctx, held[0], 1 << 19, buf.data(), 1 << 19) == 0);
+    CHECK(api->stage_submit(api->ctx, held[0]) == 0);
+    CHECK(api->stage_open(api->ctx, 1 << 20, 1 << 16) == 0);
+    CHECK(h->stats().inbox_free == 3 && h->stats().staged_parts == 0);
+  }
+  {
+    FakeDeviceKnobs k;
+    k.seed = 9;
+    std::unique_ptr<FakeHasher> h(new FakeHasher(8 << 20, 256, 8 << 20, 4, 2, 2, 256, k));
+    set_gpu_part_hasher(h->api(), 8);
+    set_part_stream(1);
+    auto body = rnd(3 << 20, 41);
+    const int64_t plen = 1 << 16, skip = 1000, n = (int64_t)body.size();
+    const int64_t full = ((n - skip - 4095) / plen) * plen - 7;
+    std::string want = hash_pieces("sha1", body.data() + skip, (size_t)full, (size_t)plen, 1);
+    auto relay = [&](int who, std::atomic<int>* good, std::atomic<int>* failed) {
+      Server origin([&](int fd) {
+        read_head(fd);
+        send_str(fd, "HTTP/1.1 206 Partial Content\r\nContent-Length: " + std::to_string(n) + "\r\n\r\n");
+        send_str(fd, std::string((const char*)body.data(), body.size()));
+      });
+      Server sink([&](int fd) {
+        read_head(fd);
+        drain_body(fd, n);
+        send_str(fd, "HTTP/1.1 200 OK\r\nContent-Length: 0\r\n\r\n");
+      });
+      HttpConn src("127.0.0.1", origin.port, 5, 5), dst("127.0.0.1", sink.port, 5, 5);
+      src.send_request("GET /g HTTP/1.1\r\nHost: x\r\n\r\n", nullptr, 0);
+      ResponseHead g = src.read_head();
+      dst.send_raw("PUT /g HTTP/1.1\r\nHost: x\r\nContent-Length: " + std::to_string(n) + "\r\n\r\n");
+      std::string digests, head, tail;
+      uint64_t ticket = 0;
+      uint32_t crc = 0;
+      try {
+        const int64_t moved = src.relay_body_hashed(dst, g.content_length, skip, full, plen,
+                                                    nullptr, &digests, &head, &tail, &crc, &ticket);
+        ResponseHead p = dst.read_head();
+        dst.read_body(p, 16);
+        const bool streamed = ticket && gpu_part_streamed(ticket);
+        if (who == 0) {
+          gpu_part_forget(ticket);
+          digests = want;
+        } else if (ticket) {
+          digests = gpu_part_wait(ticket);
+        }
+        if (moved == n && streamed && digests == want && crc == crc32c(body.data(), body.size()) &&
+            head == std::string((const char*)body.data(), (size_t)skip) &&
+            tail == std::string((const char*)body.data() + skip + full, (size_t)(n - skip - full)))
+          good->fetch_add(1);
+      } catch (const std::exception&) {
+        failed->fetch_add(1);
+      }
+    };
+    std::atomic<int> good{0}, failed{0};
+    const uint64_t nt0 = relay_counters().nt_bytes;
+    std::vector<std::thread> ths;
+    for (int t = 0; t < 4; ++t) ths.emplace_back(relay, t, &good, &failed);
+    for (auto& th : ths) th.join();
+    CHECK(good.load() == 4 && failed.load() == 0);
+    CHECK(relay_counters().nt_bytes == nt0 && relay_pool_stats().in_use == 0);
+    for (int i = 0; i < 400 && (gpu_part_stats().pending || h->stats().pending); ++i)
+      std::this_thread::sleep_for(std::chrono::milliseconds(5));
+    CHECK(gpu_part_stats().pending == 0);
+    CHECK(h->stats().staged_parts == 4 && h->stats().inbox_free == h->stats().inbox_blocks);
+    FakeDeviceKnobs kb;
+    kb.fail_push_at = 2;
+    std::unique_ptr<FakeHasher> bad(new FakeHasher(8 << 20, 256, 8 << 20, 4, 2, 2, 256, kb));
+    set_gpu_part_hasher(bad->api(), 8);
+    good = 0;
+    std::thread(relay, 1, &good, &failed).join();
+    CHECK(good.load() == 0 && failed.load() == 1);
+    CHECK(bad->stats().inbox_free == bad->stats().inbox_blocks);
+    set_part_stream(-1);
+    set_gpu_part_hasher(nullptr, 0);
+  }
+  fprintf(stderr, "streamed parts: ok\n");
+}
+
 static void stress_sections() {
+  stream_section();
   multislot_section();
   {
     Watchdog wd("part stress", 90);
diff --git a/downloader_amd/csrc/transfer.cpp b/downloader_amd/csrc/transfer.cpp
--- a/downloader_amd/csrc/transfer.cpp
+++ b/downloader_amd/csrc/transfer.cpp
@@ -1398,6 +1398,7 @@
 
 std::atomic<int> g_gpu_min_pieces{8};
 std::atomic<uint64_t> g_gpu_submitted{0}, g_gpu_fallbacks{0}, g_gpu_refused{0};
+std::atomic<uint64_t> g_gpu_streamed{0}, g_gpu_stream_failed{0};
 
 struct GpuPending {
   std::unique_ptr<PartBuffer> buf;
@@ -1407,6 +1408,7 @@
   bool copied = false, finished = false, failed = false;
   bool forgotten = false, copied_reported = false;
   bool waited = false;
+  bool streamed = false;
   std::string result;
 };
 std::mutex g_gpu_mu;
@@ -1454,21 +1456,24 @@
   const int rc = a->wait(a->ctx, ticket, GPU_PART_COPIED, nullptr, 0, err, sizeof err);
   std::unique_ptr<PartBuffer> buf;
   int64_t skip = 0, full = 0, plen = 0;
+  bool streamed = false;
   {
     std::lock_guard<std::mutex> g(g_gpu_mu);
     auto it = g_gpu_parts.find(id);
-    if (it == g_gpu_parts.end() || it->second.copied || !it->second.buf) return;
+    if (it == g_gpu_parts.end() || it->second.copied) return;
+    streamed = it->second.streamed;
+    if (!streamed && !it->second.buf) return;
     buf = std::move(it->second.buf);
     skip = it->second.skip;
     full = it->second.full_len;
     plen = it->second.piece_len;
   }
   std::string digests;
-  if (rc != 0) {
+  if (rc != 0 && !streamed) {
     host_digests(buf->data + skip, full, plen, &digests);
     g_gpu_fallbacks++;
   }
-  part_pool().release(std::move(buf));
+  if (buf) part_pool().release(std::move(buf));
   std::lock_guard<std::mutex> g(g_gpu_mu);
   auto it = g_gpu_parts.find(id);
   if (it == g_gpu_parts.end()) return;
@@ -1476,7 +1481,13 @@
   p.copied = true;
   if (rc != 0) {
     p.finished = true;
-    p.result.swap(digests);
+    if (streamed) {
+      p.failed = true;
+      p.result = std::string("GPU part stream failed: ") + err;
+      g_gpu_stream_failed++;
+    } else {
+      p.result.swap(digests);
+    }
     g_gpu_ids.erase({a, ticket});
   }
   if (p.forgotten && p.finished)
@@ -1702,7 +1713,13 @@
     pending = g_gpu_parts.size();
   }
   return GpuPartStats{g_gpu_submitted.load(), g_gpu_fallbacks.load(), g_gpu_refused.load(),
-                      pending};
+                      pending, g_gpu_streamed.load(), g_gpu_stream_failed.load()};
+}
+
+bool gpu_part_streamed(uint64_t id) {
+  std::lock_guard<std::mutex> g(g_gpu_mu);
+  auto it = g_gpu_parts.find(id);
+  return it != g_gpu_parts.end() && it->second.streamed;
 }
 
 std::string gpu_part_wait(uint64_t id) {
@@ -1835,11 +1852,184 @@
     memcpy(d, s, n);
 }
 
+static std::atomic<int> g_part_stream{-1};
+static bool part_stream_on() {
+  int v = g_part_stream.load(std::memory_order_relaxed);
+  if (v < 0) {
+    const char* e = getenv("STAGER_PART_STREAM");
+    v = e && e[0] == '1' ? 1 : 0;
+    g_part_stream.store(v);
+  }
+  return v != 0;
+}
+void set_part_stream(int on) { g_part_stream.store(on < 0 ? -1 : (on ? 1 : 0)); }
+bool part_stream_enabled() { return part_stream_on(); }
+
+static int part_stream_ring() {
+  static const int d = [] {
+    const char* e = getenv("STAGER_PART_STREAM_RING");
+    const int v = e ? atoi(e) : 4;
+    return std::max(2, std::min(16, v));
+  }();
+  return d;
+}
+
+static size_t part_stream_bytes() {
+  static const size_t b = [] {
+    const char* e = getenv("STAGER_PART_STREAM_KB");
+    const long kb = e ? atol(e) : 0;
+    return kb >= 64 && kb <= 16384 ? (size_t)kb * 1024 : peek_stage_bytes();
+  }();
+  return b;
+}
+
+namespace {
+struct StageRing {
+  uint8_t* base;
+  size_t chunk;
+  int depth;
+  const GpuPartHashApi* api;
+};
+thread_local StageRing t_ring{nullptr, 0, 0, nullptr};
+
+StageRing* stage_ring(const GpuPartHashApi* api) {
+  StageRing& r = t_ring;
+  if (!r.base) {
+    const size_t chunk = part_stream_bytes();
+    const int depth = part_stream_ring();
+    void* m = mmap(nullptr, chunk * (size_t)depth, PROT_READ | PROT_WRITE,
+                   MAP_PRIVATE | MAP_ANONYMOUS | MAP_POPULATE, -1, 0);
+    if (m == MAP_FAILED) return nullptr;
+    r.base = (uint8_t*)m;
+    r.chunk = chunk;
+    r.depth = depth;
+  }
+  if (r.api != api) {
+    if (r.api) r.api->unreg(r.api->ctx, r.base);
+    r.api = nullptr;
+    if (api->reg(api->ctx, r.base, r.chunk * (size_t)r.depth) != 0) return nullptr;
+    r.api = api;
+  }
+  return &r;
+}
+
+struct StageGuard {
+  const GpuPartHashApi* api;
+  uint64_t handle;
+  uint64_t tok[16] = {0};
+  StageGuard(const GpuPartHashApi* a, uint64_t h) : api(a), handle(h) {}
+  bool settle() {
+    bool ok = true;
+    for (uint64_t& t : tok)
+      if (t) {
+        ok = (api->stage_wait(api->ctx, t) == 0) && ok;
+        t = 0;
+      }
+    return ok;
+  }
+  ~StageGuard() {
+    settle();
+    if (handle) api->stage_abort(api->ctx, handle);
+  }
+};
+}
+
 int64_t HttpConn::relay_body_hashed_mb(HttpConn& dst, int64_t n, int64_t skip,
                                        int64_t full_len, int64_t piece_len, Progress* prog,
                                        std::string* digests, std::string* head,
                                        std::string* tail, uint32_t* crc,
                                        uint64_t* gpu_ticket) {
+  if (gpu_ticket && part_stream_on() && !ssl_ && !dst.ssl_ && relay_tee_on()) {
+    const GpuPartHashApi* sapi = g_gpu_api.load();
+    const int64_t snp = (full_len + piece_len - 1) / piece_len;
+    StageRing* ring = sapi && sapi->abi >= 3 && sapi->stage_open && full_len > 0 &&
+                              snp >= g_gpu_min_pieces.load()
+                          ? stage_ring(sapi)
+                          : nullptr;
+    const uint64_t h = ring ? sapi->stage_open(sapi->ctx, full_len, piece_len) : 0;
+    if (h) {
+      StageGuard sg(sapi, h);
+      const int64_t full_end = skip + full_len;
+      int64_t pos = 0;
+      int slot = 0;
+      size_t fill = 0;
+      const size_t peek = peek_stage_bytes();
+      std::string hd, tl;
+      uint32_t c = crc ? *crc : 0;
+      auto broke = [&](const char* what) {
+        reusable_ = false;
+        dst.reusable_ = false;
+        g_gpu_stream_failed++;
+        throw IoError(std::string("GPU part stream: ") + what + " failed");
+      };
+      const int64_t m = relay_dup(
+          dst, n, 0, prog,
+          [&](size_t& len) {
+            if (fill == 0 && sg.tok[slot]) {
+              const int rc = sapi->stage_wait(sapi->ctx, sg.tok[slot]);
+              sg.tok[slot] = 0;
+              if (rc != 0) broke("stage_wait");
+            }
+            len = std::min({len, peek, ring->chunk - fill, (size_t)(n - pos)});
+            return ring->base + (size_t)slot * ring->chunk + fill;
+          },
+          [&](const uint8_t* got, size_t got_len) {
+            if (crc) {
+              uint64_t t0 = mono_ns();
+              c = stager::crc32c(got, got_len, c);
+              t_tally.crc_ns += mono_ns() - t0;
+            }
+            fill += got_len;
+            pos += (int64_t)got_len;
+            if (fill < ring->chunk && pos < n) return;
+            const uint8_t* p = ring->base + (size_t)slot * ring->chunk;
+            const size_t k = fill;
+            const int64_t a = pos - (int64_t)k, e = pos;
+            if (a < skip) hd.append((const char*)p, (size_t)(std::min(e, skip) - a));
+            const int64_t lo = std::max(a, skip), hi = std::min(e, full_end);
+            if (lo < hi) {
+              sg.tok[slot] = sapi->stage_push(sapi->ctx, h, lo - skip, p + (lo - a), hi - lo);
+              if (!sg.tok[slot]) broke("stage_push");
+            }
+            if (e > full_end) {
+              const int64_t from = std::max(a, full_end);
+              tl.append((const char*)p + (from - a), (size_t)(e - from));
+            }
+            fill = 0;
+            slot = (slot + 1) % ring->depth;
+          });
+      if (m >= 0) {
+        if (!sg.settle()) broke("stage_wait");
+        uint64_t id = 0;
+        {
+          std::lock_guard<std::mutex> g(g_gpu_mu);
+          const uint64_t t = sapi->stage_submit(sapi->ctx, h);
+          sg.handle = 0;
+          if (t) {
+            id = ++g_gpu_next_id;
+            GpuPending& pend = g_gpu_parts[id];
+            pend.api = sapi;
+            pend.ticket = t;
+            pend.skip = skip;
+            pend.full_len = full_len;
+            pend.piece_len = piece_len;
+            pend.streamed = true;
+            const bool fresh = g_gpu_ids.emplace(std::make_pair(sapi, t), id).second;
+            if (!fresh) throw std::logic_error("gpu part hasher reused a pending ticket");
+            g_gpu_submitted++;
+            g_gpu_streamed++;
+          }
+        }
+        if (!id) broke("stage_submit");
+        if (crc) *crc = c;
+        head->swap(hd);
+        tail->swap(tl);
+        digests->clear();
+        *gpu_ticket = id;
+        return pos;
+      }
+    }
+  }
   PartLease lease((size_t)n);
   uint8_t* b = lease.b->data;
   int64_t pos = 0;
diff --git a/downloader_amd/net/http.py b/downloader_amd/net/http.py
--- a/downloader_amd/net/http.py
+++ b/downloader_amd/net/http.py
@@ -445,6 +445,8 @@
             put.sent_crc32c = d.get("crc32c", "")
         hashed = {k: d[k] for k in ("digests", "head", "tail", "gpu_ticket")} \
             if split is not None else None
+        if hashed is not None:
+            hashed["streamed"] = bool(d.get("streamed"))
         return get, put, d["moved"], hashed
 
     async def relay(self, src_url: str, src_headers: Headers, dst_url: str, dst_headers: Headers,
diff --git a/downloader_amd/ops/build.py b/downloader_amd/ops/build.py
--- a/downloader_amd/ops/build.py
+++ b/downloader_amd/ops/build.py
@@ -52,7 +52,8 @@
             CSRC / "tls.cpp", CSRC / "peerwire.cpp"]
     out = OPS / f"_native{EXT}"
     if force or _stale(out, srcs + [CSRC / "native.h", CSRC / "crc32c.h",
-                                    CSRC / "gpu_part_api.h"]):
+                                    CSRC / "gpu_part_api.h", CSRC / "part_dispatch.h",
+                                    CSRC / "part_fake_device.h"]):
         cxx = os.environ.get("CXX", "g++")
         cmd = [cxx, "-O3", "-std=c++17", "-shared", "-fPIC", "-fvisibility=hidden",
                "-march=x86-64-v3", "-Wall", "-Wno-unused-result",
@@ -118,7 +119,8 @@
     BIN.mkdir(exist_ok=True)
     out = BIN / f"selftest_{kind}"
     if force or _stale(out, srcs + [CSRC / "native.h", CSRC / "crc32c.h",
-                                    CSRC / "gpu_part_api.h", CSRC / "part_dispatch.h"]):
+                                    CSRC / "gpu_part_api.h", CSRC / "part_dispatch.h",
+                                    CSRC / "part_fake_device.h"]):
         cxx = os.environ.get("CXX", "g++")
         cmd = [cxx, "-O1", "-g", "-std=c++17", "-msse4.2", *SANITIZERS[kind],
                *[str(s) for s in srcs],
diff --git a/downloader_amd/ops/hashing.py b/downloader_amd/ops/hashing.py
--- a/downloader_amd/ops/hashing.py
+++ b/downloader_amd/ops/hashing.py
@@ -104,6 +104,14 @@
 
 PART_SLOT_BYTES = 1 << 30
 PART_SLOTS = 16
+PART_INBOX_BLOCKS = 32
+PART_INBOX_BLOCK_BYTES = 64 << 20
+
+
+def set_part_inbox(blocks: int, block_bytes: int) -> None:
+    global PART_INBOX_BLOCKS, PART_INBOX_BLOCK_BYTES
+    PART_INBOX_BLOCKS = max(0, int(blocks))
+    PART_INBOX_BLOCK_BYTES = max(4096, int(block_bytes))
 
 
 def gpu_relay_hashing(min_pieces: int = 8, slots: int = PART_SLOTS,
@@ -116,8 +124,10 @@
         if _part_hasher_failed or not gpu_available():
             return False
         try:
+            inbox = PART_INBOX_BLOCKS if native().part_stream_enabled() else 0
             ph = gpuhash().PartHasher(gpu_device(), int(slot_bytes), int(slots),
-                                      int(compute_streams), 16384, int(copy_streams))
+                                      int(compute_streams), 16384, int(copy_streams),
+                                      inbox, PART_INBOX_BLOCK_BYTES)
             native().set_gpu_part_hasher(ph.api(), min_pieces)
         except Exception:
             _part_hasher_failed = True
diff --git a/downloader_amd/service/worker.py b/downloader_amd/service/worker.py
--- a/downloader_amd/service/worker.py
+++ b/downloader_amd/service/worker.py
@@ -112,6 +112,7 @@
         try:
             if not await loop.run_in_executor(None, gpu_available):
                 return
+            hashing.set_part_inbox(d.stream_gpu_inbox_blocks, d.stream_gpu_inbox_block_mb << 20)
             ok = await loop.run_in_executor(
                 None, lambda: hashing.gpu_relay_hashing(
                     d.stream_gpu_min_pieces, d.stream_gpu_slots, d.stream_gpu_slot_mb << 20,
diff --git a/downloader_amd/torrent/stream.py b/downloader_amd/torrent/stream.py
--- a/downloader_amd/torrent/stream.py
+++ b/downloader_amd/torrent/stream.py
@@ -202,6 +202,10 @@
         self._gpu_copy_streams = int(getattr(d, "stream_gpu_copy_streams", 2) or 2)
         self._gpu_compute_streams = int(getattr(d, "stream_gpu_compute_streams", 0) or 0)
         self._gpu_slot_bytes = int(getattr(d, "stream_gpu_slot_mb", 1024) or 1024) << 20
+        if self.verify_mode != "cpu":
+            from ..ops import hashing
+            hashing.set_part_inbox(int(getattr(d, "stream_gpu_inbox_blocks", 32)),
+                                   int(getattr(d, "stream_gpu_inbox_block_mb", 64) or 64) << 20)
         self.gpu_tail = int(getattr(d, "stream_gpu_tail", 0) or 0)
         self._n_parts = sum(1 for u in self.units if u.target is not None)
         from ..ops import hashing
@@ -345,7 +349,13 @@
                         if not await self._unit_failed(u, e, queue):
                             return
                         continue
-                    part.copied.add_done_callback(lambda _f, nb=nb: self._budget.release(nb))
+                    if res[1].get("streamed"):
+                        self._budget.release(nb)
+                        self.stats["gpu_streamed_parts"] = \
+                            self.stats.get("gpu_streamed_parts", 0) + 1
+                    else:
+                        part.copied.add_done_callback(
+                            lambda _f, nb=nb: self._budget.release(nb))
                     t = asyncio.ensure_future(self._complete(u, res, part, queue))
                     self._continuations.add(t)
                     t.add_done_callback(self._continuations.discard)
diff --git a/downloader_amd/utils/config.py b/downloader_amd/utils/config.py
--- a/downloader_amd/utils/config.py
+++ b/downloader_amd/utils/config.py
@@ -104,6 +104,8 @@
     stream_gpu_slot_mb: int = 1024
     stream_gpu_copy_streams: int = 2
     stream_gpu_compute_streams: int = 0
+    stream_gpu_inbox_blocks: int = 32
+    stream_gpu_inbox_block_mb: int = 64
     stream_gpu_min_pieces: int = 8
     stream_gpu_tail: int = 32
     verify_threads: int = 0
```

Result: slower. 54450 (-1.3%).
